# assafmu/wav2letter_pytorch

Measured on AMD Instinct MI355X. Metric: audio-frames/sec/GPU (fwd+bwd+CTC), Wav2Letter 64-mel x 1000-frame bf16, higher is better.
Workload: dtype bf16

## Files before the change

### include/w2l_hip.h

```cpp
#ifndef W2L_HIP_H
#define W2L_HIP_H
#include <stdint.h>
#ifdef __cplusplus
extern "C" {
#endif

const char* w2l_last_error(void);
int w2l_abi_version(void);


int w2l_pack_weights(const float* w, int64_t s_co, int64_t s_ci, int64_t s_kw, int Cout, int Cin, int Kw,
                     int CoutP, int CinP, void* w_fwd_hi, void* w_fwd_lo, void* w_dgr_hi, void* w_dgr_lo,
                     void* stream);

int w2l_sgd_pack(float* p, float* g, float* m, int first_step, float lr, float momentum, float weight_decay,
                 int nesterov, int zero_grad, int Cout, int Cin, int Kw, void* w_fwd_hi, void* w_fwd_lo, void* w_dgr_hi,
                 void* w_dgr_lo, void* w_fwd_q, void* w_dgr_q, float q_scale, void* stream);

int w2l_nct_to_ntc(const float* x, int N, int C, int T, int CP, int pad_l, int pad_r, int pad_mode,
                   const int32_t* lens, void* out_hi, void* out_lo, void* stream);

int w2l_pad_cast(const float* g, int N, int T, int C, int CP, int halo, void* out_hi, void* out_lo, float* colsum,
                 void* stream);

int w2l_conv_stat_tiles(int N, int Tout);
int w2l_conv1d_igemm(const void* xp, int64_t x_bstride, int64_t x_rows_total, const void* w, void* y, int y_f32,
                     int accumulate, const float* bias, float* stats_partial, int N, int Cin, int Cout, int Tout,
                     int Kw, int stride, int dil, void* stream);

int w2l_conv1d_igemm_tune(const void* xp, int64_t x_bstride, int64_t x_rows_total, const void* w, void* y, int y_f32,
                          const float* bias, float* stats_partial, int N, int Cin, int Cout, int Tout, int Kw, int stride,
                          int dil, int reps, void* stream);

int w2l_conv1d_igemm_ws(const void* xp, int64_t x_bstride, int64_t x_rows_total, const void* w, void* y, int y_f32,
                        int accumulate, const float* bias, float* stats_partial, int N, int Cin, int Cout, int Tout, int Kw,
                        int stride, int dil, void* splitk_ws, int64_t splitk_ws_bytes, void* stream);
int w2l_conv1d_igemm_tune_ws(const void* xp, int64_t x_bstride, int64_t x_rows_total, const void* w, void* y, int y_f32,
                             const float* bias, float* stats_partial, int N, int Cin, int Cout, int Tout, int Kw, int stride,
                             int dil, int reps, void* splitk_ws, int64_t splitk_ws_bytes, void* stream);
int64_t w2l_conv_splitk_workspace_bytes(int N, int Cout, int Tout);
int w2l_conv_streamk_ranges(int idx, int N, int Cin, int Cout, int Tout, int Kw, int stride, int dil, int64_t ws_bytes);
int w2l_conv_streamk_pieces(int tiles, int steps, int G, int* out, int cap);

int w2l_conv1d_igemm_fp8(const void* xq, int64_t x_bstride, int64_t x_rows_total, const void* wq, void* y, int y_f32,
                         float descale, const float* descale_dev, const float* bias, float* stats_partial, int N, int Cin,
                         int Cout, int Tout, int Kw, int dil, void* stream);
int w2l_conv1d_igemm_fp8_tune(const void* xq, int64_t x_bstride, int64_t x_rows_total, const void* wq, void* y, int y_f32,
                              const float* bias, float* stats_partial, int N, int Cin, int Cout, int Tout, int Kw, int dil,
                              int reps, void* stream);

void w2l_conv_force_tile_config(int idx);
void w2l_conv_force_fp8_config(int idx);
int w2l_conv_plan(int N, int Cin, int Cout, int Tout, int Kw, int stride, int dil, int stats_flag, int64_t ws_bytes,
                  int forced_idx, int* out);
int w2l_conv_plan_fp8(int N, int Cin, int Cout, int Tout, int Kw, int dil, int stats_flag, int forced_idx, int* out);

int w2l_wgrad_needs_zero(int N, int Cin, int Cout, int Tout, int Kw);
int w2l_conv1d_wgrad(const void* dy, int64_t dy_bstride, const void* xp, int64_t x_bstride, int64_t x_rows_total,
                     float* dw, int N, int Cin, int Cout, int Tout, int Kw, int stride, int dil, int accumulate,
                     void* stream);

int w2l_conv1d_wgrad_ws(const void* dy, int64_t dy_bstride, const void* xp, int64_t x_bstride, int64_t x_rows_total, float* dw,
                        int N, int Cin, int Cout, int Tout, int Kw, int stride, int dil, int accumulate, void* ws,
                        int64_t ws_bytes, void* stream);
int w2l_conv1d_wgrad_tune_ws(const void* dy, int64_t dy_bstride, const void* xp, int64_t x_bstride, int64_t x_rows_total,
                             float* dw_scratch, int N, int Cin, int Cout, int Tout, int Kw, int stride, int dil, int reps,
                             void* ws, int64_t ws_bytes, void* stream);
int w2l_wgrad_needs_zero_ws(int N, int Cin, int Cout, int Tout, int Kw, int64_t ws_bytes);
int64_t w2l_wgrad_workspace_bytes(int Cin, int Cout, int Kw);

int64_t w2l_wgrad_dealt_workspace_bytes(int Cin, int Cout, int Kw);
int w2l_conv1d_wgrad_tune_x(const void* dy, int64_t dy_bstride, const void* xp, int64_t x_bstride, int64_t x_rows_total,
                            float* dw_scratch, int N, int Cin, int Cout, int Tout, int Kw, int stride, int dil, int reps,
                            void* ws, int64_t ws_bytes, int flags, void* stream);
int w2l_wgrad_needs_zero_x(int N, int Cin, int Cout, int Tout, int Kw, int stride, int dil, int64_t ws_bytes);
int w2l_wgrad_dealt_segments(int tiles, int steps, int ranges, int* out, int max_blocks);
int w2l_wgrad_plan(int N, int Cin, int Cout, int Tout, int Kw);

typedef struct {
    const void* dy;
    int64_t dy_bstride;
    const void* xp;
    int64_t x_bstride;
    int64_t x_rows_total;
    float* dw;
    int Cin, Cout, Kw, pad_;
} w2l_wgrad_item_t;
#define W2L_WGRAD_GROUP_MAX 8
int w2l_conv1d_wgrad_group(const w2l_wgrad_item_t* items, int nitems, int N, int Tout, int dil, int form, void* stream);
int w2l_wgrad_group_tiles(int Cin, int Cout, int Kw, int form);

void w2l_wgrad_force_plan(int splits, int order);
void w2l_wgrad_deterministic(int on);

int w2l_conv1d_wgrad_tune(const void* dy, int64_t dy_bstride, const void* xp, int64_t x_bstride, int64_t x_rows_total,
                          float* dw_scratch, int N, int Cin, int Cout, int Tout, int Kw, int stride, int dil, int reps,
                          void* stream);

int w2l_wgrad_fp8_needs_zero(int N, int Cin, int Cout, int Tout, int Kw);
int w2l_conv1d_wgrad_fp8(const void* dyq, int64_t dy_bstride, const void* xq, int64_t x_bstride, int64_t x_rows_total,
                         float* dw, int N, int Cin, int Cout, int Tout, int Kw, int dil, float descale,
                         const float* descale_dev, int accumulate, void* stream);
int w2l_conv1d_wgrad_fp8_tune(const void* dyq, int64_t dy_bstride, const void* xq, int64_t x_bstride, int64_t x_rows_total,
                              float* dw_scratch, int N, int Cin, int Cout, int Tout, int Kw, int dil, int reps, void* stream);

int w2l_tune_save(const char* path);
int w2l_tune_load(const char* path);

int w2l_dwconv_fwd(const void* x_hi, const void* x_lo, int x_rows, const float* w, void* y_hi, void* y_lo, int N, int Tout,
                   int C, int K, int stride, int dil, const int32_t* lens, void* stream);
int w2l_dwconv_dgrad(const void* dy, int dy_f32, int dy_rows, const float* w, void* dxp, int dxp_f32, int N, int Tp, int Tout,
                     int C, int K, int dil, const int32_t* lens, void* stream);
int w2l_dwconv_wgrad(const void* dy, int dy_f32, int dy_rows, const void* x_hi, const void* x_lo, int x_rows, float* dw, int N,
                     int Tout, int C, int K, int stride, int dil, const int32_t* lens, void* stream);


int w2l_bn_finalize(const float* partial, int ntiles, int C, int64_t count, const float* gamma, const float* beta,
                    float eps, float momentum, float* running_mean, float* running_var, float* mean, float* invstd,
                    float* scale, float* shift, void* stream);

typedef struct {
    int32_t N, T, C;
    const void* y;
    int32_t y_f32;
    const float* scale;
    const float* shift;
    const float* mean;
    const float* invstd;
    const void* y2;
    const float* scale2;
    const float* shift2;
    const float* mean2;
    const float* invstd2;
    int32_t act;
    float drop_p;
    uint64_t seed, offset;
    uint8_t* mask;
    const int32_t* lens;
    const uint64_t* offset_dev;
    uint64_t* q_clipped;
} w2l_bnact_t;

int w2l_bn_act_fwd(const w2l_bnact_t* d, void* out_hi, void* out_lo, int out_rows, int pad_l, int pad_r,
                   int pad_mode, void* stream);
int w2l_bn_act_fwd_q(const w2l_bnact_t* d, void* out_hi, void* out_lo, void* out_q, float q_scale, int out_rows,
                     int pad_l, int pad_r, int pad_mode, void* stream);
typedef struct {
    const float* partial;
    int32_t rows;
    int64_t count;
    const float* gamma;
    const float* beta;
    float eps, momentum;
    float* running_mean;
    float* running_var;
    float* mean;
    float* invstd;
    float* scale;
    float* shift;
} w2l_bnfin_t;
int w2l_bn_act_fwd_fin(const w2l_bnact_t* d, const w2l_bnfin_t* f1, const w2l_bnfin_t* f2, void* out_hi, void* out_q,
                       float q_scale, int out_rows, int pad_l, int pad_r, int pad_mode, void* stream);
void w2l_conv_stats_mode(int slots);

int w2l_quantize_e4m3(const void* src, int src_f32, int64_t n, float scale, void* dst, void* stream);

typedef struct {
    const void* dxp;
    int32_t f32;
    int32_t pad_l, pad_r, pad_mode;
    int32_t rows;
} w2l_gradsrc_t;

int w2l_bn_bwd_blocks(int N, int T, int C);
int w2l_bn_act_bwd_reduce(const w2l_bnact_t* d, const w2l_gradsrc_t* g1, const w2l_gradsrc_t* g2, float* partial,
                          void* stream);
int w2l_bn_bwd_finalize(const float* partial, int nblocks, int C, int ncomp, float* sums, void* stream);
int w2l_bn_act_bwd_apply(const w2l_bnact_t* d, const w2l_gradsrc_t* g1, const w2l_gradsrc_t* g2, const float* sums,
                         void* dy_hi, void* dy_lo, int halo, void* dy2_hi, void* dy2_lo, int halo2, void* stream);
int w2l_bn_act_bwd_apply_fin(const w2l_bnact_t* d, const w2l_gradsrc_t* g1, const w2l_gradsrc_t* g2, const float* partial,
                             int nblocks, float* sums, void* dy_hi, void* dy_lo, int halo, void* dy2_hi, void* dy2_lo,
                             int halo2, float* amax, void* stream);
int w2l_bn_bwd_fast_ok(const w2l_bnact_t* d, const w2l_gradsrc_t* g1, const w2l_gradsrc_t* g2);
int w2l_bn_act_bwd_reduce_slots(const w2l_bnact_t* d, const w2l_gradsrc_t* g1, float* partial, int slots, void* stream);
int w2l_bn_act_bwd_apply_slots(const w2l_bnact_t* d, const w2l_gradsrc_t* g1, const float* partial, int nrows, float* sums,
                               void* dy_hi, int halo, float* amax, void* stream);
#define W2L_AMAX_SLOTS 64
int w2l_bn_act_bwd_apply_amax(const w2l_bnact_t* d, const w2l_gradsrc_t* g1, const w2l_gradsrc_t* g2, const float* sums,
                              void* dy_hi, void* dy_lo, int halo, void* dy2_hi, void* dy2_lo, int halo2, float* amax,
                              void* stream);
int w2l_quantize_e4m3_dyn(const void* src_bf16, int64_t n, const float* amax, void* dst, float* inv_scale, void* stream);

int w2l_conv1d_dgrad_bnreduce_ws(const void* dy, int64_t dy_rows_total, const void* w_dgr, void* dxp, float* partial,
                                 const w2l_bnact_t* d, int pad_l, int pad_r, int pad_mode, int per, int Cconv_out,
                                 int flat_rows, int Kw, int dil, void* splitk_ws, int64_t splitk_ws_bytes, void* stream);
int w2l_conv1d_dgrad_bnreduce_tune_ws(const void* dy, int64_t dy_rows_total, const void* w_dgr, void* dxp, float* partial,
                                      const w2l_bnact_t* d, int pad_l, int pad_r, int pad_mode, int per, int Cconv_out,
                                      int flat_rows, int Kw, int dil, int reps, void* splitk_ws, int64_t splitk_ws_bytes,
                                      void* stream);

typedef struct {
    const float* scale;
    const float* shift;
    const void* res;
    const void* res_lo;
    int32_t act;
    const int32_t* lens;
    void* out_hi;
    void* out_lo;
    int32_t out_rows, pad_l, pad_r, pad_mode;
} w2l_bnact_epi_t;
int w2l_conv1d_igemm_bnact(const void* xp, int64_t x_bstride, int64_t x_rows_total, const void* w, const float* acc_in,
                           const float* bias, const w2l_bnact_epi_t* e, int N, int Cin, int Cout, int Tout, int Kw, int stride,
                           int dil, void* stream);
int w2l_conv1d_igemm_bnact_ws(const void* xp, int64_t x_bstride, int64_t x_rows_total, const void* w, const float* acc_in,
                              const float* bias, const w2l_bnact_epi_t* e, int N, int Cin, int Cout, int Tout, int Kw,
                              int stride, int dil, void* splitk_ws, int64_t splitk_ws_bytes, void* stream);
int w2l_conv1d_igemm_bnact_tune_ws(const void* xp, int64_t x_bstride, int64_t x_rows_total, const void* w, const float* bias,
                                   const w2l_bnact_epi_t* e, int N, int Cin, int Cout, int Tout, int Kw, int stride, int dil,
                                   int reps, void* splitk_ws, int64_t splitk_ws_bytes, void* stream);

int w2l_conv1d_igemm_bnact_fp8(const void* xq, int64_t x_bstride, int64_t x_rows_total, const void* wq, float descale,
                               const float* bias, const w2l_bnact_epi_t* e, void* out_q, float q_scale, int64_t* q_clipped,
                               int N, int Cin, int Cout, int Tout, int Kw, int dil, void* stream);
int w2l_conv1d_igemm_bnact_fp8_tune(const void* xq, int64_t x_bstride, int64_t x_rows_total, const void* wq, const float* bias,
                                    const w2l_bnact_epi_t* e, void* out_q, float q_scale, int N, int Cin, int Cout, int Tout,
                                    int Kw, int dil, int reps, void* stream);

int w2l_log_softmax_fwd(const float* logits, int N, int T, int C, int CP, int mode, float* out, void* stream);
int w2l_log_softmax_bwd(const float* gout, const float* out, int N, int T, int C, int mode, float* glogits,
                        void* stream);
int64_t w2l_ctc_workspace_bytes(int N, int T, int Smax);
int w2l_ctc_loss(const float* log_probs, const int32_t* targets, const int32_t* input_lengths,
                 const int32_t* target_lengths, int N, int T, int C, int Smax, int blank, int zero_infinity,
                 float* nll, float* loss, float* grad, void* workspace, void* stream);

int64_t w2l_ctc_align_workspace_bytes(int N, int T, int Smax);
int w2l_ctc_align(const float* x, const int32_t* input_lengths, const int32_t* targets, int64_t target_stride,
                  const int32_t* target_lengths, int64_t length_stride, int N, int T, int A, int Smax, int blank,
                  int log_probs, void* workspace, int64_t workspace_bytes, float* score, int32_t* status, int32_t* path,
                  int32_t* starts, int32_t* ends, void* stream);

int64_t w2l_asg_workspace_bytes(int N, int T, int A, int Smax);
int w2l_asg_loss(const float* x, const float* transitions, const int32_t* targets, const int32_t* input_lengths,
                 const int32_t* target_lengths, int N, int T, int A, int Smax, int repeat_index, int reduction, float* nll,
                 float* loss, float* grad_x, float* grad_trans, int32_t* status, void* workspace, int64_t workspace_bytes,
                 void* stream);
int64_t w2l_asg_viterbi_workspace_bytes(int N, int T, int A);
int w2l_asg_viterbi(const float* x, const float* transitions, const int32_t* input_lengths, int N, int T, int A,
                    void* workspace, int64_t workspace_bytes, int32_t* path, float* score, void* stream);

int w2l_argmax(const float* probs, int64_t rows, int C, int32_t* idx, void* stream);
typedef struct {
    const float* prob;
    const float* bo;
    const uint64_t* ngram_keys;
    const int32_t* ngram_vals;
    int64_t ngram_cap;
    const uint64_t* trie_keys;
    const int32_t* trie_vals;
    int64_t trie_cap;
    const int32_t* trie_word;
    int32_t n_entries;
    int32_t n_words;
    int32_t n_trie_nodes;
} w2l_ngram_lm_t;
int w2l_ngram_lm_build(const uint64_t* keys, const int32_t* vals, int64_t n, uint64_t* table_keys, int32_t* table_vals,
                       int64_t cap, int32_t* dups, void* stream);
typedef struct {
    const uint64_t* trie_keys;
    const int32_t* trie_vals;
    int64_t trie_cap;
    const int32_t* trie_word;
    int32_t n_trie_nodes;
} w2l_lexicon_t;
int64_t w2l_ctc_beam_search_workspace_bytes(int N, int T, int k, int order);
int w2l_ctc_beam_search(const float* probs, const int32_t* sizes, int N, int T, int A, const int32_t* label_info_host,
                        int blank, int end_index, int space_index, int k, double alpha, double beta, double prune,
                        int log_probs, const w2l_ngram_lm_t* lm, int order, const w2l_lexicon_t* lexicon,
                        int complete_only, const w2l_lexicon_t* hotwords, double hotword_weight, void* workspace,
                        int64_t workspace_bytes, void* out, void* stream);
int64_t w2l_asg_beam_search_workspace_bytes(int N, int T, int A, int k, int order);
int w2l_asg_beam_search(const float* x, const float* transitions, const int32_t* sizes, int N, int T, int A,
                        const int32_t* label_info_host, int repeat_index, int space_index, int k, double alpha, double beta,
                        double prune, const w2l_ngram_lm_t* lm, int order, void* workspace, int64_t workspace_bytes, void* out,
                        void* stream);
int w2l_asg_beam_search_tables(const float* x, const float* transitions, const int32_t* sizes, int N, int T, int A,
                               const int32_t* label_info_host, int repeat_index, int space_index, int k, double alpha,
                               double beta, double prune, const w2l_ngram_lm_t* lm, int order, const w2l_lexicon_t* lexicon,
                               int complete_only, const w2l_lexicon_t* hotwords, double hotword_weight, void* workspace,
                               int64_t workspace_bytes, void* out, void* stream);
int64_t w2l_asg_align_workspace_bytes(int N, int T, int A, int Smax);
int w2l_asg_align(const float* x, const float* transitions, const int32_t* input_lengths, const int32_t* targets,
                  int64_t target_stride, const int32_t* target_lengths, int64_t length_stride, int N, int T, int A, int Smax,
                  int repeat_index, int encoded, void* workspace, int64_t workspace_bytes, float* score, int32_t* status,
                  int32_t* path, int32_t* starts, int32_t* ends, void* stream);
int w2l_levenshtein_host(const int32_t* a_host, int na, const int32_t* b_host, int nb);
int w2l_greedy_score_host(const int32_t* idx_host, int N, int T, const int32_t* sizes_host, int blank, const int32_t* lut,
                          int n_labels, const int32_t* ref_cp, const int64_t* ref_off, int64_t* totals, int32_t* hyp_cp,
                          int64_t* hyp_off);

int w2l_novograd_pack(float* p, const float* g, float* exp_avg, float* exp_avg_sq, float* max_exp_avg_sq, float* scratch,
                      int scratch_floats, float lr, float beta1, float beta2, float eps, float weight_decay, int grad_averaging,
                      int Cout, int Cin, int Kw, void* w_fwd_hi, void* w_fwd_lo, void* w_dgr_hi, void* w_dgr_lo, void* stream);

int w2l_logmel(const float* audio, const int32_t* n_samples, const float* noise, float dither, float preemph, int N,
               int64_t audio_stride, const float* window, int win_length, int n_fft, int hop, const float* fbT,
               const int32_t* fb_range, int n_mels, int take_log, float log_guard, float* logmel, int Tmax, void* stream);
int w2l_feature_normalize(const float* logmel, const int32_t* n_samples, int hop, int N, int Tmax, int n_mels, float eps,
                          float* mean_ws, float* std_ws, float* out_nct, void* stream);
int w2l_zero_rects(float* x, int N, int C, int T, const int32_t* rects, int R, void* stream);

#define W2L_RESAMPLE_TILE 512
#define W2L_RESAMPLE_MAX_K 512
#define W2L_RESAMPLE_MAX_SPAN 8192
int w2l_resample(const float* x, int64_t in_stride, float* out, int64_t out_stride, int N, const int32_t* rows_host,
                 const int32_t* rows_dev, const int32_t* banks_host, const int32_t* banks_dev, int n_banks, const float* taps,
                 int64_t n_taps, void* stream);

#define W2L_REVERB_TILE 1024
#define W2L_REVERB_CHUNK 512
#define W2L_REVERB_MAX_TAPS 16384
int w2l_reverb(const float* x, int64_t in_stride, float* out, int64_t out_stride, int N, const int32_t* rows_host,
               const int32_t* rows_dev, const int32_t* banks_host, const int32_t* banks_dev, int n_banks, const float* taps,
               int64_t n_taps, void* stream);
#define W2L_MIX_TILE 2048
int64_t w2l_mix_noise_slab_doubles(int N, int64_t out_stride);
int w2l_mix_noise(const float* x, int64_t x_stride, const float* z, int64_t z_stride, float* out, int64_t out_stride, int N,
                  const int32_t* rows_host, const int32_t* rows_dev, const float* snr_db, double* slab, int64_t slab_doubles,
                  void* stream);

int w2l_stream_probe(void* stream_a, void* stream_b, void* stamps_dev, int rounds, int spin_us);

#define W2L_RCCL_ID_BYTES 128
int w2l_rccl_available(void);
const char* w2l_rccl_library(void);
int w2l_rccl_unique_id(void* id_host);
int w2l_rccl_init(const void* id_host, int rank, int world, void** comm_out);
int w2l_rccl_world(void* comm, int* world_out);
int w2l_rccl_all_reduce(void* comm, void* buf, int64_t count, int dtype, int average, void* stream);
int w2l_rccl_broadcast(void* comm, void* buf, int64_t bytes, int root, void* stream);
int w2l_rccl_destroy(void* comm);

typedef union { void* p; int64_t i; double d; } w2l_slot_t;
#define W2L_REPLAY_MAX_ARGS 24
typedef struct { int32_t op; int32_t nargs; w2l_slot_t a[W2L_REPLAY_MAX_ARGS]; } w2l_call_t;
int w2l_replay_op(const char* entry_point_name);
int w2l_replay_arity(int op);
int w2l_replay(const w2l_call_t* calls, int n, int* failed_at);

int w2l_event_create(void** event_out);
int w2l_event_destroy(void* event);
int w2l_event_record(void* event, void* stream);
int w2l_stream_wait_event(void* stream, void* event);
int w2l_event_query(void* event);
int w2l_event_synchronize(void* event);
int w2l_stream_wait_stream(void* waiter, void* signaler);

int w2l_fill_zero(void* p, int64_t bytes, void* stream);
int w2l_pad_vec_f32(const float* src, int n, float* dst, int cp, float fill, void* stream);
int w2l_counter_add(void* counter_i64, int64_t delta, void* stream);
int w2l_add_i64_multi(void* table_dev, int n, int64_t delta, void* stream);
typedef struct { float* p; const float* g; float* m; int32_t n; int32_t pad_; } w2l_sgd_small_t;
int w2l_sgd_small_multi(const w2l_sgd_small_t* items_dev, int nitems, int max_n , float lr,
                        float momentum, float weight_decay, int nesterov, void* stream);

#define W2L_CLIP_NORM 0
#define W2L_CLIP_COEF 1
#define W2L_CLIP_BOUND 2
#define W2L_GNORM_CHUNK 8192
#define W2L_GNORM_BLOCKS 2048
typedef struct { const float* g; int64_t n; int64_t chunk0; } w2l_gnorm_item_t;
int w2l_grad_sqnorm_multi(const w2l_gnorm_item_t* items_dev, int nitems, int64_t nchunks, int inf_norm, double* partials,
                          float max_norm, float* clip, float* norm_out, void* stream);
int w2l_grad_clip_value(float* clip, float clip_value, void* stream);
int w2l_sgd_pack_clip(float* p, float* g, float* m, int first_step, float lr, float momentum, float weight_decay,
                      int nesterov, int zero_grad, int Cout, int Cin, int Kw, void* w_fwd_hi, void* w_fwd_lo, void* w_dgr_hi,
                      void* w_dgr_lo, void* w_fwd_q, void* w_dgr_q, float q_scale, const float* clip, void* stream);
int w2l_sgd_small_multi_clip(const w2l_sgd_small_t* items_dev, int nitems, int max_n, float lr, float momentum,
                             float weight_decay, int nesterov, const float* clip, void* stream);

typedef struct { int64_t step; double pow1; double pow2; } w2l_adam_state_t;
typedef struct { float* p; const float* g; float* m; float* v; int32_t n; int32_t pad_; } w2l_adam_small_t;
int w2l_adam_tick(w2l_adam_state_t* state_dev, float* dyn_dev, double lr, double beta1, double beta2, void* stream);
int w2l_adam_pack(float* p, float* g, float* m, float* v, const float* dyn, float beta1, float beta2, float eps,
                  float weight_decay, int decoupled, int zero_grad, int Cout, int Cin, int Kw, void* w_fwd_hi, void* w_fwd_lo,
                  void* w_dgr_hi, void* w_dgr_lo, void* w_fwd_q, void* w_dgr_q, float q_scale, const float* clip ,
                  void* stream);
// ... 9 lines not shown
```

### wav2letter_pytorch_amd/_lib.py

```python
from __future__ import annotations

import ctypes as C
import os

os.environ.setdefault('GPU_MAX_HW_QUEUES', '8')

import torch

_HERE = os.path.dirname(os.path.abspath(__file__))
LIB_PATH = os.environ.get('W2L_LIB') or os.path.join(_HERE, 'libw2l_hip.so')

c_p = C.c_void_p
c_i = C.c_int
c_i64 = C.c_int64
c_u64 = C.c_uint64
c_f = C.c_float


class BnActDesc(C.Structure):
    _fields_ = [
        ('N', C.c_int32), ('T', C.c_int32), ('C', C.c_int32),
        ('y', c_p), ('y_f32', C.c_int32),
        ('scale', c_p), ('shift', c_p), ('mean', c_p), ('invstd', c_p),
        ('y2', c_p), ('scale2', c_p), ('shift2', c_p), ('mean2', c_p), ('invstd2', c_p),
        ('act', C.c_int32), ('drop_p', c_f), ('seed', c_u64), ('offset', c_u64),
        ('mask', c_p), ('lens', c_p), ('offset_dev', c_p), ('q_clipped', c_p),
    ]


class WgradItem(C.Structure):
    _fields_ = [('dy', c_p), ('dy_bstride', C.c_int64), ('xp', c_p), ('x_bstride', C.c_int64), ('x_rows_total', C.c_int64),
                ('dw', c_p), ('Cin', C.c_int32), ('Cout', C.c_int32), ('Kw', C.c_int32), ('pad_', C.c_int32)]


class BnFin(C.Structure):
    _fields_ = [('partial', c_p), ('rows', C.c_int32), ('count', C.c_int64), ('gamma', c_p), ('beta', c_p), ('eps', c_f),
                ('momentum', c_f), ('running_mean', c_p), ('running_var', c_p), ('mean', c_p), ('invstd', c_p), ('scale', c_p),
                ('shift', c_p)]


class LmTables(C.Structure):
    _fields_ = [('prob', c_p), ('bo', c_p), ('ngram_keys', c_p), ('ngram_vals', c_p), ('ngram_cap', C.c_int64),
                ('trie_keys', c_p), ('trie_vals', c_p), ('trie_cap', C.c_int64), ('trie_word', c_p), ('n_entries', C.c_int32),
                ('n_words', C.c_int32), ('n_trie_nodes', C.c_int32)]


class LexTables(C.Structure):
    _fields_ = [('trie_keys', c_p), ('trie_vals', c_p), ('trie_cap', C.c_int64), ('trie_word', c_p),
                ('n_trie_nodes', C.c_int32)]


class BnActEpi(C.Structure):
    _fields_ = [('scale', c_p), ('shift', c_p), ('res', c_p), ('res_lo', c_p), ('act', C.c_int32), ('lens', c_p),
                ('out_hi', c_p), ('out_lo', c_p), ('out_rows', C.c_int32), ('pad_l', C.c_int32), ('pad_r', C.c_int32),
                ('pad_mode', C.c_int32)]


class GradSrc(C.Structure):
    _fields_ = [('dxp', c_p), ('f32', C.c_int32), ('pad_l', C.c_int32), ('pad_r', C.c_int32),
                ('pad_mode', C.c_int32), ('rows', C.c_int32)]


_SIGNATURES = {
    'w2l_last_error': (C.c_char_p, []),
    'w2l_abi_version': (c_i, []),
    'w2l_tune_save': (c_i, [C.c_char_p]),
    'w2l_tune_load': (c_i, [C.c_char_p]),
    'w2l_pack_weights': (c_i, [c_p, c_i64, c_i64, c_i64, c_i, c_i, c_i, c_i, c_i, c_p, c_p, c_p, c_p, c_p]),
    'w2l_sgd_pack': (c_i, [c_p, c_p, c_p, c_i, c_f, c_f, c_f, c_i, c_i, c_i, c_i, c_i, c_p, c_p, c_p, c_p, c_p, c_p, c_f, c_p]),
    'w2l_novograd_pack': (c_i, [c_p, c_p, c_p, c_p, c_p, c_p, c_i, c_f, c_f, c_f, c_f, c_f, c_i, c_i, c_i, c_i, c_p, c_p, c_p, c_p,
                                c_p]),
    'w2l_nct_to_ntc': (c_i, [c_p, c_i, c_i, c_i, c_i, c_i, c_i, c_i, c_p, c_p, c_p, c_p]),
    'w2l_pad_cast': (c_i, [c_p, c_i, c_i, c_i, c_i, c_i, c_p, c_p, c_p, c_p]),
    'w2l_conv_stat_tiles': (c_i, [c_i, c_i]),
    'w2l_conv1d_igemm': (c_i, [c_p, c_i64, c_i64, c_p, c_p, c_i, c_i, c_p, c_p, c_i, c_i, c_i, c_i, c_i, c_i, c_i, c_p]),
    'w2l_conv1d_igemm_tune': (c_i, [c_p, c_i64, c_i64, c_p, c_p, c_i, c_p, c_p, c_i, c_i, c_i, c_i, c_i, c_i, c_i, c_i, c_p]),
    'w2l_conv1d_igemm_ws': (c_i, [c_p, c_i64, c_i64, c_p, c_p, c_i, c_i, c_p, c_p, c_i, c_i, c_i, c_i, c_i, c_i, c_i, c_p, c_i64, c_p]),
    'w2l_conv1d_igemm_tune_ws': (c_i, [c_p, c_i64, c_i64, c_p, c_p, c_i, c_p, c_p, c_i, c_i, c_i, c_i, c_i, c_i, c_i, c_i, c_p,
                                       c_i64, c_p]),
    'w2l_conv1d_igemm_bnact': (c_i, [c_p, c_i64, c_i64, c_p, c_p, c_p, C.POINTER(BnActEpi), c_i, c_i, c_i, c_i, c_i, c_i, c_i, c_p]),
    'w2l_conv1d_igemm_bnact_ws': (c_i, [c_p, c_i64, c_i64, c_p, c_p, c_p, C.POINTER(BnActEpi), c_i, c_i, c_i, c_i, c_i, c_i, c_i,
                                        c_p, c_i64, c_p]),
    'w2l_conv1d_igemm_bnact_tune_ws': (c_i, [c_p, c_i64, c_i64, c_p, c_p, C.POINTER(BnActEpi), c_i, c_i, c_i, c_i, c_i, c_i, c_i,
                                             c_i, c_p, c_i64, c_p]),
    'w2l_conv_splitk_workspace_bytes': (c_i64, [c_i, c_i, c_i]),
    'w2l_conv_streamk_ranges': (c_i, [c_i] * 8 + [c_i64]),
    'w2l_conv_streamk_pieces': (c_i, [c_i, c_i, c_i, c_p, c_i]),
    'w2l_conv_force_tile_config': (None, [c_i]),
    'w2l_conv_force_fp8_config': (None, [c_i]),
    'w2l_conv_plan': (c_i, [c_i] * 8 + [c_i64, c_i, c_p]),
    'w2l_conv_plan_fp8': (c_i, [c_i] * 8 + [c_p]),
    'w2l_wgrad_force_plan': (None, [c_i, c_i]),
    'w2l_wgrad_deterministic': (None, [c_i]),
    'w2l_wgrad_needs_zero': (c_i, [c_i, c_i, c_i, c_i, c_i]),
    'w2l_conv1d_wgrad': (c_i, [c_p, c_i64, c_p, c_i64, c_i64, c_p, c_i, c_i, c_i, c_i, c_i, c_i, c_i, c_i, c_p]),
    'w2l_conv1d_wgrad_ws': (c_i, [c_p, c_i64, c_p, c_i64, c_i64, c_p, c_i, c_i, c_i, c_i, c_i, c_i, c_i, c_i, c_p, c_i64, c_p]),
    'w2l_conv1d_wgrad_tune_ws': (c_i, [c_p, c_i64, c_p, c_i64, c_i64, c_p, c_i, c_i, c_i, c_i, c_i, c_i, c_i, c_i, c_p, c_i64, c_p]),
    'w2l_wgrad_needs_zero_ws': (c_i, [c_i, c_i, c_i, c_i, c_i, c_i64]),
    'w2l_wgrad_workspace_bytes': (c_i64, [c_i, c_i, c_i]),
    'w2l_wgrad_dealt_workspace_bytes': (c_i64, [c_i, c_i, c_i]),
    'w2l_conv1d_wgrad_tune_x': (c_i, [c_p, c_i64, c_p, c_i64, c_i64, c_p, c_i, c_i, c_i, c_i, c_i, c_i, c_i, c_i, c_p, c_i64, c_i, c_p]),
    'w2l_wgrad_needs_zero_x': (c_i, [c_i, c_i, c_i, c_i, c_i, c_i, c_i, c_i64]),
    'w2l_wgrad_dealt_segments': (c_i, [c_i, c_i, c_i, c_p, c_i]),
    'w2l_wgrad_plan': (c_i, [c_i, c_i, c_i, c_i, c_i]),
    'w2l_conv1d_wgrad_group': (c_i, [c_p, c_i, c_i, c_i, c_i, c_i, c_p]),
    'w2l_wgrad_group_tiles': (c_i, [c_i, c_i, c_i, c_i]),
    'w2l_conv1d_wgrad_tune': (c_i, [c_p, c_i64, c_p, c_i64, c_i64, c_p, c_i, c_i, c_i, c_i, c_i, c_i, c_i, c_i, c_p]),
    'w2l_dwconv_fwd': (c_i, [c_p, c_p, c_i, c_p, c_p, c_p, c_i, c_i, c_i, c_i, c_i, c_i, c_p, c_p]),
    'w2l_dwconv_dgrad': (c_i, [c_p, c_i, c_i, c_p, c_p, c_i, c_i, c_i, c_i, c_i, c_i, c_i, c_p, c_p]),
    'w2l_dwconv_wgrad': (c_i, [c_p, c_i, c_i, c_p, c_p, c_i, c_p, c_i, c_i, c_i, c_i, c_i, c_i, c_p, c_p]),
    'w2l_bn_finalize': (c_i, [c_p, c_i, c_i, c_i64, c_p, c_p, c_f, c_f, c_p, c_p, c_p, c_p, c_p, c_p, c_p]),
    'w2l_bn_act_fwd': (c_i, [C.POINTER(BnActDesc), c_p, c_p, c_i, c_i, c_i, c_i, c_p]),
    'w2l_bn_act_fwd_q': (c_i, [C.POINTER(BnActDesc), c_p, c_p, c_p, c_f, c_i, c_i, c_i, c_i, c_p]),
    'w2l_bn_bwd_fast_ok': (c_i, [C.POINTER(BnActDesc), C.POINTER(GradSrc), C.POINTER(GradSrc)]),
    'w2l_bn_act_bwd_reduce_slots': (c_i, [C.POINTER(BnActDesc), C.POINTER(GradSrc), c_p, c_i, c_p]),
    'w2l_bn_act_bwd_apply_slots': (c_i, [C.POINTER(BnActDesc), C.POINTER(GradSrc), c_p, c_i, c_p, c_p, c_i, c_p, c_p]),
    'w2l_bn_act_fwd_fin': (c_i, [C.POINTER(BnActDesc), C.POINTER(BnFin), C.POINTER(BnFin), c_p, c_p, c_f, c_i, c_i, c_i, c_i, c_p]),
    'w2l_conv_stats_mode': (None, [c_i]),
    'w2l_quantize_e4m3': (c_i, [c_p, c_i, c_i64, c_f, c_p, c_p]),
    'w2l_quantize_e4m3_dyn': (c_i, [c_p, c_i64, c_p, c_p, c_p, c_p]),
    'w2l_bn_act_bwd_apply_amax': (c_i, [C.POINTER(BnActDesc), C.POINTER(GradSrc), C.POINTER(GradSrc), c_p, c_p, c_p, c_i,
                                        c_p, c_p, c_i, c_p, c_p]),
    'w2l_conv1d_igemm_fp8': (c_i, [c_p, c_i64, c_i64, c_p, c_p, c_i, c_f, c_p, c_p, c_p, c_i, c_i, c_i, c_i, c_i, c_i, c_p]),
    'w2l_conv1d_igemm_bnact_fp8': (c_i, [c_p, c_i64, c_i64, c_p, c_f, c_p, C.POINTER(BnActEpi), c_p, c_f, c_p, c_i, c_i, c_i, c_i,
                                         c_i, c_i, c_p]),
    'w2l_conv1d_igemm_bnact_fp8_tune': (c_i, [c_p, c_i64, c_i64, c_p, c_p, C.POINTER(BnActEpi), c_p, c_f, c_i, c_i, c_i, c_i, c_i,
                                              c_i, c_i, c_p]),
    'w2l_conv1d_igemm_fp8_tune': (c_i, [c_p, c_i64, c_i64, c_p, c_p, c_i, c_p, c_p, c_i, c_i, c_i, c_i, c_i, c_i, c_i, c_p]),
    'w2l_bn_bwd_blocks': (c_i, [c_i, c_i, c_i]),
    'w2l_bn_act_bwd_reduce': (c_i, [C.POINTER(BnActDesc), C.POINTER(GradSrc), C.POINTER(GradSrc), c_p, c_p]),
    'w2l_bn_bwd_finalize': (c_i, [c_p, c_i, c_i, c_i, c_p, c_p]),
    'w2l_bn_act_bwd_apply': (c_i, [C.POINTER(BnActDesc), C.POINTER(GradSrc), C.POINTER(GradSrc), c_p, c_p, c_p, c_i,
                                   c_p, c_p, c_i, c_p]),
    'w2l_conv1d_dgrad_bnreduce_ws': (c_i, [c_p, c_i64, c_p, c_p, c_p, C.POINTER(BnActDesc), c_i, c_i, c_i, c_i, c_i, c_i, c_i, c_i,
                                           c_p, c_i64, c_p]),
    'w2l_conv1d_dgrad_bnreduce_tune_ws': (c_i, [c_p, c_i64, c_p, c_p, c_p, C.POINTER(BnActDesc), c_i, c_i, c_i, c_i, c_i, c_i, c_i,
                                                c_i, c_i, c_p, c_i64, c_p]),
    'w2l_bn_act_bwd_apply_fin': (c_i, [C.POINTER(BnActDesc), C.POINTER(GradSrc), C.POINTER(GradSrc), c_p, c_i, c_p, c_p, c_p, c_i,
                                       c_p, c_p, c_i, c_p, c_p]),
    'w2l_log_softmax_fwd': (c_i, [c_p, c_i, c_i, c_i, c_i, c_i, c_p, c_p]),
    'w2l_log_softmax_bwd': (c_i, [c_p, c_p, c_i, c_i, c_i, c_i, c_p, c_p]),
    'w2l_ctc_workspace_bytes': (c_i64, [c_i, c_i, c_i]),
    'w2l_ctc_loss': (c_i, [c_p, c_p, c_p, c_p, c_i, c_i, c_i, c_i, c_i, c_i, c_p, c_p, c_p, c_p, c_p]),
    'w2l_asg_workspace_bytes': (c_i64, [c_i, c_i, c_i, c_i]),
    'w2l_asg_loss': (c_i, [c_p, c_p, c_p, c_p, c_p, c_i, c_i, c_i, c_i, c_i, c_i, c_p, c_p, c_p, c_p, c_p, c_p, c_i64, c_p]),
    'w2l_asg_viterbi_workspace_bytes': (c_i64, [c_i, c_i, c_i]),
    'w2l_asg_viterbi': (c_i, [c_p, c_p, c_p, c_i, c_i, c_i, c_p, c_i64, c_p, c_p, c_p]),
    'w2l_argmax': (c_i, [c_p, c_i64, c_i, c_p, c_p]),
    'w2l_ctc_align_workspace_bytes': (c_i64, [c_i, c_i, c_i]),
    'w2l_ctc_align': (c_i, [c_p, c_p, c_p, c_i64, c_p, c_i64, c_i, c_i, c_i, c_i, c_i, c_i, c_p, c_i64, c_p, c_p, c_p, c_p, c_p,
                            c_p]),
    'w2l_ctc_beam_search_workspace_bytes': (c_i64, [c_i, c_i, c_i, c_i]),
    'w2l_ctc_beam_search': (c_i, [c_p, c_p, c_i, c_i, c_i, c_p, c_i, c_i, c_i, c_i, C.c_double, C.c_double, C.c_double, c_i,
                                  C.POINTER(LmTables), c_i, C.POINTER(LexTables), c_i, C.POINTER(LexTables), C.c_double,
                                  c_p, c_i64, c_p, c_p]),
    'w2l_ngram_lm_build': (c_i, [c_p, c_p, c_i64, c_p, c_p, c_i64, c_p, c_p]),
    'w2l_asg_beam_search_workspace_bytes': (c_i64, [c_i, c_i, c_i, c_i, c_i]),
    'w2l_asg_beam_search': (c_i, [c_p, c_p, c_p, c_i, c_i, c_i, c_p, c_i, c_i, c_i, C.c_double, C.c_double, C.c_double,
                                  C.POINTER(LmTables), c_i, c_p, c_i64, c_p, c_p]),
    'w2l_asg_beam_search_tables': (c_i, [c_p, c_p, c_p, c_i, c_i, c_i, c_p, c_i, c_i, c_i, C.c_double, C.c_double, C.c_double,
                                         C.POINTER(LmTables), c_i, C.POINTER(LexTables), c_i, C.POINTER(LexTables), C.c_double,
                                         c_p, c_i64, c_p, c_p]),
    'w2l_asg_align_workspace_bytes': (c_i64, [c_i, c_i, c_i, c_i]),
    'w2l_asg_align': (c_i, [c_p, c_p, c_p, c_p, c_i64, c_p, c_i64, c_i, c_i, c_i, c_i, c_i, c_i, c_p, c_i64, c_p, c_p, c_p, c_p,
                            c_p, c_p]),
    'w2l_logmel': (c_i, [c_p, c_p, c_p, c_f, c_f, c_i, c_i64, c_p, c_i, c_i, c_i, c_p, c_p, c_i, c_i, c_f, c_p, c_i, c_p]),
    'w2l_feature_normalize': (c_i, [c_p, c_p, c_i, c_i, c_i, c_i, c_f, c_p, c_p, c_p, c_p]),
    'w2l_zero_rects': (c_i, [c_p, c_i, c_i, c_i, c_p, c_i, c_p]),
    'w2l_resample': (c_i, [c_p, c_i64, c_p, c_i64, c_i, c_p, c_p, c_p, c_p, c_i, c_p, c_i64, c_p]),
    'w2l_reverb': (c_i, [c_p, c_i64, c_p, c_i64, c_i, c_p, c_p, c_p, c_p, c_i, c_p, c_i64, c_p]),
    'w2l_mix_noise_slab_doubles': (c_i64, [c_i, c_i64]),
    'w2l_mix_noise': (c_i, [c_p, c_i64, c_p, c_i64, c_p, c_i64, c_i, c_p, c_p, c_p, c_p, c_i64, c_p]),
    'w2l_levenshtein_host': (c_i, [c_p, c_i, c_p, c_i]),
    'w2l_greedy_score_host': (c_i, [c_p, c_i, c_i, c_p, c_i, c_p, c_i, c_p, c_p, c_p, c_p, c_p]),
    'w2l_wgrad_fp8_needs_zero': (c_i, [c_i, c_i, c_i, c_i, c_i]),
    'w2l_conv1d_wgrad_fp8': (c_i, [c_p, c_i64, c_p, c_i64, c_i64, c_p, c_i, c_i, c_i, c_i, c_i, c_i, c_f, c_p, c_i, c_p]),
    'w2l_conv1d_wgrad_fp8_tune': (c_i, [c_p, c_i64, c_p, c_i64, c_i64, c_p, c_i, c_i, c_i, c_i, c_i, c_i, c_i, c_p]),
    'w2l_stream_probe': (c_i, [c_p, c_p, c_p, c_i, c_i]),
    'w2l_rccl_available': (c_i, []),
    'w2l_rccl_library': (C.c_char_p, []),
    'w2l_rccl_unique_id': (c_i, [c_p]),
    'w2l_rccl_init': (c_i, [c_p, c_i, c_i, c_p]),
    'w2l_rccl_world': (c_i, [c_p, c_p]),
    'w2l_rccl_all_reduce': (c_i, [c_p, c_p, c_i64, c_i, c_i, c_p]),
    'w2l_rccl_broadcast': (c_i, [c_p, c_p, c_i64, c_i, c_p]),
    'w2l_rccl_destroy': (c_i, [c_p]),
    'w2l_replay_op': (c_i, [C.c_char_p]),
    'w2l_replay_arity': (c_i, [c_i]),
    'w2l_replay': (c_i, [c_p, c_i, c_p]),
    'w2l_event_create': (c_i, [c_p]),
    'w2l_event_destroy': (c_i, [c_p]),
    'w2l_event_record': (c_i, [c_p, c_p]),
    'w2l_stream_wait_event': (c_i, [c_p, c_p]),
    'w2l_event_query': (c_i, [c_p]),
    'w2l_event_synchronize': (c_i, [c_p]),
    'w2l_stream_wait_stream': (c_i, [c_p, c_p]),
    'w2l_fill_zero': (c_i, [c_p, c_i64, c_p]),
    'w2l_pad_vec_f32': (c_i, [c_p, c_i, c_p, c_i, c_f, c_p]),
    'w2l_counter_add': (c_i, [c_p, c_i64, c_p]),
    'w2l_add_i64_multi': (c_i, [c_p, c_i, c_i64, c_p]),
    'w2l_sgd_small_multi': (c_i, [c_p, c_i, c_i, c_f, c_f, c_f, c_i, c_p]),
    'w2l_sgd_small_multi_clip': (c_i, [c_p, c_i, c_i, c_f, c_f, c_f, c_i, c_p, c_p]),
    'w2l_sgd_pack_clip': (c_i, [c_p, c_p, c_p, c_i, c_f, c_f, c_f, c_i, c_i, c_i, c_i, c_i, c_p, c_p, c_p, c_p, c_p, c_p, c_f, c_p,
                                c_p]),
    'w2l_grad_sqnorm_multi': (c_i, [c_p, c_i, c_i64, c_i, c_p, c_f, c_p, c_p, c_p]),
    'w2l_grad_clip_value': (c_i, [c_p, c_f, c_p]),
    'w2l_adam_tick': (c_i, [c_p, c_p, C.c_double, C.c_double, C.c_double, c_p]),
    'w2l_adam_pack': (c_i, [c_p, c_p, c_p, c_p, c_p, c_f, c_f, c_f, c_f, c_i, c_i, c_i, c_i, c_i, c_p, c_p, c_p, c_p, c_p, c_p, c_f,
                            c_p, c_p]),
    'w2l_adam_small_multi': (c_i, [c_p, c_i, c_i, c_p, c_f, c_f, c_f, c_f, c_i, c_p, c_p]),
}

EXPORTED_SYMBOLS = tuple(_SIGNATURES)
GNORM_CHUNK = 8192
GNORM_BLOCKS = 2048
CLIP_NORM, CLIP_COEF, CLIP_BOUND = 0, 1, 2


class W2LError(RuntimeError):
    pass


def _load():
    if not os.path.exists(LIB_PATH):
        raise ImportError(
            f'{LIB_PATH} not found: build the HIP extension first '
            f'(python -c "import __graft_entry__ as g; g.build()" or make -C wav2letter_pytorch_amd/csrc). '
            f'There is no CPU fallback.')
    lib = C.CDLL(LIB_PATH)
    for name, (res, args) in _SIGNATURES.items():
        fn = getattr(lib, name)
        fn.restype = res
        fn.argtypes = args
    return lib


lib = _load()


def check(rc: int, what: str = ''):
    if rc != 0:
        msg = lib.w2l_last_error()
        raise W2LError(f'{what} failed (code {rc}): {msg.decode() if msg else "?"}')


def ptr(t):
    return None if t is None else C.c_void_p(t.data_ptr())


def stream_ptr():
    return C.c_void_p(torch._C._cuda_getCurrentRawStream(torch._C._cuda_getDevice()))


def require_device(*tensors):
    for t in tensors:
        if t is not None and not t.is_cuda:
            raise W2LError('wav2letter_pytorch_amd runs on MI355X only: got a CPU tensor '
                           '(there is no CPU fallback; move the model and batch to cuda)')


TRACE_NAMES = {
    'w2l_conv1d_igemm': 'conv_igemm_kernel', 'w2l_conv1d_igemm_ws': 'conv_igemm_kernel',
    'w2l_conv1d_dgrad_bnreduce_ws': 'conv_igemm_kernel/dgrad+bnreduce',
    'w2l_conv1d_igemm_bnact': 'conv_igemm_kernel/bnact', 'w2l_conv1d_igemm_bnact_ws': 'conv_igemm_kernel/bnact',
    'w2l_conv1d_igemm_fp8': 'conv_igemm_fp8_kernel', 'w2l_conv1d_igemm_bnact_fp8': 'conv_igemm_fp8_kernel/bnact',
    'w2l_conv1d_wgrad': 'conv_wgrad_kernel', 'w2l_conv1d_wgrad_ws': 'conv_wgrad_kernel', 'w2l_conv1d_wgrad_group': 'conv_wgrad_kernel', 'w2l_conv1d_wgrad_fp8': 'conv_wgrad_fp8_kernel',
    'w2l_bn_finalize': 'bn_finalize_kernel', 'w2l_bn_act_fwd': 'bn_act_fwd_kernel', 'w2l_bn_act_fwd_q': 'bn_act_fwd_kernel',
    'w2l_bn_act_fwd_fin': 'bn_act_fwd_kernel', 'w2l_bn_act_bwd_reduce': 'bn_act_bwd_reduce_kernel',
    'w2l_bn_act_bwd_reduce_slots': 'bn_act_bwd_reduce_kernel', 'w2l_bn_act_bwd_apply_slots': 'bn_act_bwd_apply_kernel', 'w2l_bn_bwd_finalize': 'bn_bwd_finalize_kernel',
    'w2l_bn_act_bwd_apply': 'bn_act_bwd_apply_kernel', 'w2l_bn_act_bwd_apply_amax': 'bn_act_bwd_apply_kernel',
    'w2l_bn_act_bwd_apply_fin': 'bn_act_bwd_apply_kernel', 'w2l_sgd_pack': 'sgd_pack_kernel', 'w2l_pack_weights': 'pack_weights_kernel',
    'w2l_sgd_pack_clip': 'sgd_pack_kernel', 'w2l_adam_pack': 'adam_pack_kernel', 'w2l_grad_sqnorm_multi': 'grad_norm_kernels',
    'w2l_asg_loss': 'asg_kernels', 'w2l_asg_viterbi': 'asg_viterbi_kernel',
    'w2l_ctc_loss': 'ctc_kernels', 'w2l_log_softmax_fwd': 'log_softmax_fwd', 'w2l_log_softmax_bwd': 'log_softmax_bwd',
    'w2l_nct_to_ntc': 'nct_to_ntc_kernel', 'w2l_pad_cast': 'pad_cast_kernel', 'w2l_quantize_e4m3': 'quantize_e4m3',
    'w2l_quantize_e4m3_dyn': 'quantize_e4m3_dyn', 'w2l_dwconv_fwd': 'dw_fwd_kernel', 'w2l_dwconv_dgrad': 'dw_dgrad_kernel',
    'w2l_dwconv_wgrad': 'dw_wgrad_kernel', 'w2l_argmax': 'argmax_kernel', 'w2l_novograd_pack': 'novograd_pack_kernel',
    'w2l_ctc_beam_search': 'ctc_beam_search_kernel', 'w2l_ngram_lm_build': 'ngram_insert_kernel', 'w2l_ctc_align': 'ctc_align_kernel',
    'w2l_asg_beam_search': 'asg_beam_search_kernel', 'w2l_asg_beam_search_tables': 'asg_beam_search_kernel',
    'w2l_asg_align': 'asg_align_kernel',
}
_trace = {'rows': None, 'saved': {}, 'pool': []}


def trace_launches(enable: bool, capacity: int = 4096):
    if enable and _trace['rows'] is None:
        _trace['rows'] = []
    if enable and not _trace['saved']:
        _trace['pool'] = [torch.cuda.Event(enable_timing=True) for _ in range(2 * capacity)]
        for name, label in TRACE_NAMES.items():
            fn = getattr(lib, name)
            _trace['saved'][name] = fn

            def wrapper(*args, _fn=fn, _label=label):
                pool = _trace['pool']
                s = pool.pop() if pool else torch.cuda.Event(enable_timing=True)
                e = pool.pop() if pool else torch.cuda.Event(enable_timing=True)
                s.record()
                rc = _fn(*args)
                e.record()
                _trace['rows'].append((_label, torch._C._cuda_getCurrentRawStream(torch._C._cuda_getDevice()), s, e))
                return rc

            setattr(lib, name, wrapper)
    elif not enable:
        for name, fn in _trace['saved'].items():
            setattr(lib, name, fn)
        _trace['saved'] = {}


def trace_dump(path: str) -> int:
    rows, _trace['rows'] = _trace['rows'] or [], None
    _trace['pool'] = []
    if not rows:
        return 0
    origin = rows[0][2]
    with open(path, 'w') as f:
        f.write('Kernel_Name,Queue_Id,Start_Timestamp,End_Timestamp\n')
        for label, stream, s, e in rows:
            t0 = origin.elapsed_time(s)
            f.write('%s,%d,%d,%d\n' % (label, stream, int(t0 * 1e6), int((t0 + s.elapsed_time(e)) * 1e6)))
    return len(rows)


def raw_stream(stream=None) -> int:
    if stream is None:
        return torch._C._cuda_getCurrentRawStream(torch._C._cuda_getDevice())
    return stream.cuda_stream


class Event:
    __slots__ = ('h', '__weakref__')
    _free: list = []

    def __init__(self):
        if Event._free:
            self.h = Event._free.pop()
        else:
            out = C.c_void_p()
            check(lib.w2l_event_create(C.byref(out)), 'w2l_event_create')
            self.h = out.value
        rec = _recorder[0]
        if rec is not None:
            rec.keep.append(self)

    def record(self, stream=None):
        check(lib.w2l_event_record(self.h, raw_stream(stream)), 'w2l_event_record')

    def wait(self, stream=None):
        check(lib.w2l_stream_wait_event(raw_stream(stream), self.h), 'w2l_stream_wait_event')

    def query(self) -> bool:
        rc = lib.w2l_event_query(self.h)
        if rc not in (0, 1):
            check(rc, 'w2l_event_query')
        return rc == 0

    def synchronize(self):
        check(lib.w2l_event_synchronize(self.h), 'w2l_event_synchronize')

    def __del__(self):
        try:
            Event._free.append(self.h)
        except Exception:
            pass


def stream_wait_stream(waiter, signaler):
    a = waiter if isinstance(waiter, int) else waiter.cuda_stream
    b = signaler if isinstance(signaler, int) else signaler.cuda_stream
    check(lib.w2l_stream_wait_stream(a, b), 'w2l_stream_wait_stream')


class Slot(C.Union):
    _fields_ = [('p', c_p), ('i', c_i64), ('d', C.c_double)]


REPLAY_MAX_ARGS = 24


class Call(C.Structure):
    _fields_ = [('op', C.c_int32), ('nargs', C.c_int32), ('a', Slot * REPLAY_MAX_ARGS)]


_recorder = [None]
AUDIT = False
_REPLAY_OPS = {}


def _replay_ops():
    if not _REPLAY_OPS:
        for name, (_, args) in _SIGNATURES.items():
            op = lib.w2l_replay_op(name.encode())
            if op < 0:
                continue
            kinds = []
            for a in args:
                if a in (c_i, c_i64, c_u64, C.c_int32):
                    kinds.append('i')
                elif a in (c_f, C.c_double):
                    kinds.append('d')
                else:
                    kinds.append('p')
            assert lib.w2l_replay_arity(op) == len(kinds) <= REPLAY_MAX_ARGS, name
            _REPLAY_OPS[name] = (op, tuple(kinds))
    return _REPLAY_OPS


class Phase:
    __slots__ = ('items', 'keep', 'n_calls', 'dev_ptrs')

    def __init__(self, items, keep, n_calls, dev_ptrs=None):
        self.items, self.keep, self.n_calls = items, keep, n_calls
        self.dev_ptrs = dev_ptrs

    def replay(self):
        failed = C.c_int(-1)
        for it in self.items:
            if it[0] == 'c':
                rc = lib.w2l_replay(it[1], it[2], C.byref(failed))
                if rc != 0:
                    msg = lib.w2l_last_error()
                    raise W2LError(f'w2l_replay failed at record {failed.value} of {it[2]} (code {rc}): {msg.decode() if msg else "?"}')
            else:
                _, fn, args, stream = it
                if stream is None:
                    fn(*args)
# ... 155 lines not shown
```

### wav2letter_pytorch_amd/csrc/ctc.hip

```cpp
#include "common.h"
#include <math.h>
#include <stdlib.h>

namespace {

constexpr float NEG_INF = -INFINITY;

__device__ __forceinline__ float lse2(float a, float b) {
    const float m = fmaxf(a, b);
    if (m == NEG_INF) return NEG_INF;
    return m + __logf(__expf(a - m) + __expf(b - m));
}
__device__ __forceinline__ float lse3(float a, float b, float c) {
    const float m = __builtin_fmaxf(__builtin_fmaxf(a, b), c);
    if (m == NEG_INF) return NEG_INF;
    const float lo = __builtin_fminf(__builtin_fminf(a, b), c);
    const float md = __builtin_amdgcn_fmed3f(a, b, c);
    return m + __logf(1.f + __expf(md - m) + __expf(lo - m));
}

__global__ __launch_bounds__(256) void log_softmax_fwd_kernel(const float* logits, int64_t rows, int C, int CP, int mode,
                                                               float* out) {
    const int lane = threadIdx.x & 63;
    const int64_t row = (int64_t)blockIdx.x * 4 + (threadIdx.x >> 6);
// ... 40 lines not shown
    float* nll;
};

template <int NT, int SPT, bool LP_LDS>
__global__ __launch_bounds__(NT) void ctc_alpha_beta_kernel(CtcParams p) {
    extern __shared__ float sh[];
    const int n = blockIdx.x;
    const bool is_beta = blockIdx.y == 1;
    const int tid = threadIdx.x;
    const int S = min(max(p.tg_len[n], 0), p.Smax);
    const int Tn = min(max(p.in_len[n], 0), p.T);
    const int L = 2 * S + 1;
    const int Lp = SPT * NT + 4;
    float* buf0 = sh + 2;
    float* buf1 = sh + Lp + 2;
    const float* lp = p.lp + (int64_t)n * p.T * p.C;
    if (LP_LDS) {
        float* lds_lp = sh + 2 * Lp;
        const int total = Tn * p.C;
        for (int i = tid; i < total; i += NT) lds_lp[i] = lp[i];
        lp = lds_lp;
        __syncthreads();
    }
    float* dst = (is_beta ? p.beta : p.alpha) + (int64_t)n * p.T * p.L;
    const int32_t* tg = p.targets + (int64_t)n * p.Smax;

    int lab[SPT];
    bool skip[SPT];
#pragma unroll
    for (int k = 0; k < SPT; ++k) {
        const int s = tid + k * NT;
        lab[k] = p.blank;
        skip[k] = false;
        if (s < L && (s & 1)) {
            lab[k] = tg[s >> 1];
            if (!is_beta) skip[k] = s >= 3 && tg[(s >> 1) - 1] != lab[k];
            else skip[k] = s + 2 < L && tg[(s >> 1) + 1] != lab[k];
        }
    }
    if (tid < 2) { buf0[-2 + tid] = NEG_INF; buf1[-2 + tid] = NEG_INF; }
    if (tid < 2) { buf0[Lp - 4 + tid] = NEG_INF; buf1[Lp - 4 + tid] = NEG_INF; }

    if (Tn == 0) {
        if (!is_beta && tid == 0) p.nll[n] = S == 0 ? 0.f : (p.zero_inf ? 0.f : INFINITY);
        return;
    }
    const int t_first = is_beta ? Tn - 1 : 0;
    float cur[SPT], nxt_lp[SPT];
#pragma unroll
    for (int k = 0; k < SPT; ++k) {
        const int s = tid + k * NT;
        float v = NEG_INF;
        if (s < L) {
            const bool init = is_beta ? (s >= L - 2) : (s <= 1);
            if (init) v = lp[(int64_t)t_first * p.C + lab[k]];
            dst[(int64_t)t_first * p.L + s] = v;
        }
        cur[k] = v;
        buf0[s] = v;
        nxt_lp[k] = 0.f;
    }
    const int dir = is_beta ? -1 : 1;
    if (Tn > 1) {
#pragma unroll
        for (int k = 0; k < SPT; ++k)
            if (tid + k * NT < L) nxt_lp[k] = lp[(int64_t)(t_first + dir) * p.C + lab[k]];
    }
    __syncthreads();
    float* prev = buf0;
    float* next = buf1;
    for (int i = 1; i < Tn; ++i) {
        const int t = t_first + dir * i;
        float e[SPT];
#pragma unroll
        for (int k = 0; k < SPT; ++k) e[k] = nxt_lp[k];
        if (i + 1 < Tn) {
#pragma unroll
            for (int k = 0; k < SPT; ++k)
                if (tid + k * NT < L) nxt_lp[k] = lp[(int64_t)(t + dir) * p.C + lab[k]];
        }
#pragma unroll
        for (int k = 0; k < SPT; ++k) {
            const int s = tid + k * NT;
            const float a0 = cur[k];
            const float a1 = prev[s - dir];
            const float a2 = skip[k] ? prev[s - 2 * dir] : NEG_INF;
            float v = lse3(a0, a1, a2) + e[k];
            if (s >= L) v = NEG_INF;
            cur[k] = v;
            next[s] = v;
            if (s < L) dst[(int64_t)t * p.L + s] = v;
        }
        asm volatile("s_waitcnt lgkmcnt(0)" ::: "memory");
        __builtin_amdgcn_s_barrier();
        asm volatile("" ::: "memory");
        float* tmp = prev; prev = next; next = tmp;
    }
    if (!is_beta && tid == 0) {
        const float a = prev[L - 1];
        const float b = L > 1 ? prev[L - 2] : NEG_INF;
        float nll = -lse2(a, b);
        p.nll[n] = nll;
    }
}

__global__ __launch_bounds__(256) void ctc_grad_kernel(CtcParams p, float* grad, float* nll_out) {
    __shared__ float acc_all[4][64];
    const int lane = threadIdx.x & 63, w = threadIdx.x >> 6;
    const int n = blockIdx.y;
    const int t = blockIdx.x * 4 + w;
    if (t >= p.T) return;
    float* acc = acc_all[w];
    const int S = min(max(p.tg_len[n], 0), p.Smax);
    const int Tn = min(max(p.in_len[n], 0), p.T);
    const int L = 2 * S + 1;
    const float nll = p.nll[n];
    const bool inf = !(nll < INFINITY);
    float* g = grad + ((int64_t)n * p.T + t) * p.C;
    if (t >= Tn || (inf && p.zero_inf)) {
        for (int c = lane; c < p.C; c += 64) g[c] = 0.f;
        return;
    }
    const float* lp = p.lp + ((int64_t)n * p.T + t) * p.C;
    const float* al = p.alpha + ((int64_t)n * p.T + t) * p.L;
    const float* be = p.beta + ((int64_t)n * p.T + t) * p.L;
    const int32_t* tg = p.targets + (int64_t)n * p.Smax;
    for (int c = lane; c < 64; c += 64) acc[c] = 0.f;
    float m = NEG_INF;
    for (int s = lane; s < L; s += 64) {
        const int c = (s & 1) ? tg[s >> 1] : p.blank;
        const float v = al[s] + be[s];
        if (v > NEG_INF) m = fmaxf(m, v - lp[c]);
    }
#pragma unroll
    for (int k = 32; k > 0; k >>= 1) m = fmaxf(m, __shfl_xor(m, k, 64));
    __builtin_amdgcn_wave_barrier();
    if (m > NEG_INF) {
        for (int s = lane; s < L; s += 64) {
            const int c = (s & 1) ? tg[s >> 1] : p.blank;
            const float v = al[s] + be[s];
            if (v > NEG_INF) atomicAdd(&acc[c], expf(v - lp[c] - m));
        }
    }
    __builtin_amdgcn_wave_barrier();
    const float gs = 1.f / ((float)p.N * (float)max(S, 1));
    const float post_scale = m > NEG_INF ? expf(m + nll) : 0.f;
    for (int c = lane; c < p.C; c += 64) {
        const float post = acc[c] * post_scale;
        g[c] = (expf(lp[c]) - post) * gs;
    }
    (void)nll_out;
}

__global__ void ctc_loss_reduce_kernel(float* nll, const int32_t* tg_len, int N, int Smax, int zero_inf, float* loss) {
    __shared__ float red[256];
    float s = 0.f;
    for (int n = threadIdx.x; n < N; n += 256) {
        float v = nll[n];
        if (zero_inf && !(v < INFINITY)) { v = 0.f; nll[n] = 0.f; }
        const int S = min(max(tg_len[n], 0), Smax);
        s += v / (float)max(S, 1);
    }
    red[threadIdx.x] = s;
    __syncthreads();
    for (int k = 128; k > 0; k >>= 1) {
        if (threadIdx.x < k) red[threadIdx.x] += red[threadIdx.x + k];
        __syncthreads();
    }
    if (threadIdx.x == 0) loss[0] = red[0] / (float)N;
}

__global__ __launch_bounds__(256) void argmax_kernel(const float* probs, int64_t rows, int C, int32_t* idx) {
    const int64_t row = (int64_t)blockIdx.x * 256 + threadIdx.x;
    if (row >= rows) return;
    const float* p = probs + row * C;
    float best = p[0];
    int bi = 0;
    bool nan_found = best != best;
    for (int c = 1; c < C && !nan_found; ++c) {
        const float v = p[c];
        if (v != v) { bi = c; nan_found = true; }
        else if (v > best) { best = v; bi = c; }
    }
    idx[row] = bi;
}

}

extern "C" int w2l_log_softmax_fwd(const float* logits, int N, int T, int C, int CP, int mode, float* out, void* stream) {
    W2L_CHECK_ARG(logits && out && N > 0 && T > 0 && C > 0 && CP >= C, "log_softmax_fwd: bad arguments");
    const int64_t rows = (int64_t)N * T;
    hipLaunchKernelGGL(log_softmax_fwd_kernel, dim3((unsigned)((rows + 3) / 4)), dim3(256), 0, (hipStream_t)stream,
                       logits, rows, C, CP, mode, out);
    W2L_CHECK_LAUNCH();
    return 0;
}

extern "C" int w2l_log_softmax_bwd(const float* gout, const float* out, int N, int T, int C, int mode, float* glogits,
                                   void* stream) {
    W2L_CHECK_ARG(gout && out && glogits && N > 0 && T > 0 && C > 0, "log_softmax_bwd: bad arguments");
    const int64_t rows = (int64_t)N * T;
    hipLaunchKernelGGL(log_softmax_bwd_kernel, dim3((unsigned)((rows + 3) / 4)), dim3(256), 0, (hipStream_t)stream, gout,
                       out, rows, C, mode, glogits);
    W2L_CHECK_LAUNCH();
    return 0;
}

extern "C" int64_t w2l_ctc_workspace_bytes(int N, int T, int Smax) {
    if (N <= 0 || T <= 0 || Smax < 0) return 0;
    return 2 * (int64_t)N * T * (2 * Smax + 1) * (int64_t)sizeof(float);
}

extern "C" int w2l_ctc_loss(const float* log_probs, const int32_t* targets, const int32_t* input_lengths,
                            const int32_t* target_lengths, int N, int T, int C, int Smax, int blank, int zero_infinity,
                            float* nll, float* loss, float* grad, void* workspace, void* stream) {
    W2L_CHECK_ARG(log_probs && input_lengths && target_lengths && nll && loss && workspace, "ctc_loss: null pointer");
    W2L_CHECK_ARG(targets || Smax == 0, "ctc_loss: null targets");
    W2L_CHECK_ARG(N > 0 && T > 0 && C > 0 && C <= 64 && Smax >= 0 && blank >= 0 && blank < C, "ctc_loss: bad sizes");
    const int L = 2 * Smax + 1;
    W2L_CHECK_ARG(L <= 8 * 1024, "ctc_loss: target length %d too long (max 4095)", Smax);
    CtcParams p;
    p.lp = log_probs; p.targets = targets; p.in_len = input_lengths; p.tg_len = target_lengths;
    p.N = N; p.T = T; p.C = C; p.Smax = Smax; p.L = L; p.blank = blank; p.zero_inf = zero_infinity;
    p.alpha = (float*)workspace;
    p.beta = p.alpha + (int64_t)N * T * L;
    p.nll = nll;
    static const int kWide[] = {64, 128, 192, 256, 320, 384, 448, 512, 640, 768, 896, 1024};
    int nt = 1024;
    for (int w : kWide)
        if (L <= w) { nt = w; break; }
    int spt = (L + nt - 1) / nt;
    if (spt > 1) spt = spt <= 4 ? spt : (spt <= 6 ? 6 : 8);
    dim3 grid(N, 2), block(nt);
    size_t lds = 2 * (size_t)(spt * nt + 4) * sizeof(float);
    const size_t lp_bytes = (size_t)T * C * sizeof(float);
    const bool lp_lds = lds + lp_bytes <= 150 * 1024;
    if (lp_lds) lds += lp_bytes;
#define W2L_CTC_LAUNCH(NT, SPT)                                                                              \
    do {                                                                                                     \
        if (lp_lds) {                                                                                        \
            W2L_CHECK_HIP(w2l_allow_big_lds((const void*)ctc_alpha_beta_kernel<NT, SPT, true>));             \
            hipLaunchKernelGGL((ctc_alpha_beta_kernel<NT, SPT, true>), grid, block, lds, (hipStream_t)stream, p);  \
        } else {                                                                                             \
            hipLaunchKernelGGL((ctc_alpha_beta_kernel<NT, SPT, false>), grid, block, lds, (hipStream_t)stream, p); \
        }                                                                                                    \
    } while (0)
    if (spt == 1) {
        switch (nt) {
            case 64: W2L_CTC_LAUNCH(64, 1); break;
            case 128: W2L_CTC_LAUNCH(128, 1); break;
            case 192: W2L_CTC_LAUNCH(192, 1); break;
            case 256: W2L_CTC_LAUNCH(256, 1); break;
            case 320: W2L_CTC_LAUNCH(320, 1); break;
            case 384: W2L_CTC_LAUNCH(384, 1); break;
            case 448: W2L_CTC_LAUNCH(448, 1); break;
            case 512: W2L_CTC_LAUNCH(512, 1); break;
            case 640: W2L_CTC_LAUNCH(640, 1); break;
            case 768: W2L_CTC_LAUNCH(768, 1); break;
            case 896: W2L_CTC_LAUNCH(896, 1); break;
            default: W2L_CTC_LAUNCH(1024, 1); break;
        }
    } else {
        switch (spt) {
            case 2: W2L_CTC_LAUNCH(1024, 2); break;
            case 3: W2L_CTC_LAUNCH(1024, 3); break;
            case 4: W2L_CTC_LAUNCH(1024, 4); break;
            case 6: W2L_CTC_LAUNCH(1024, 6); break;
            default: W2L_CTC_LAUNCH(1024, 8); break;
        }
    }
#undef W2L_CTC_LAUNCH
    W2L_CHECK_LAUNCH();
    if (grad) {
        hipLaunchKernelGGL(ctc_grad_kernel, dim3((T + 3) / 4, N), dim3(256), 0, (hipStream_t)stream, p, grad, nll);
        W2L_CHECK_LAUNCH();
    }
    hipLaunchKernelGGL(ctc_loss_reduce_kernel, dim3(1), dim3(256), 0, (hipStream_t)stream, nll, target_lengths, N,
                       p.Smax, zero_infinity, loss);
    W2L_CHECK_LAUNCH();
    return 0;
}

extern "C" int w2l_argmax(const float* probs, int64_t rows, int C, int32_t* idx, void* stream) {
    W2L_CHECK_ARG(probs && idx && rows > 0 && C > 0, "argmax: bad arguments");
    hipLaunchKernelGGL(argmax_kernel, dim3((unsigned)((rows + 255) / 256)), dim3(256), 0, (hipStream_t)stream, probs, rows,
                       C, idx);
    W2L_CHECK_LAUNCH();
    return 0;
}
```

### wav2letter_pytorch_amd/csrc/pack.hip

```cpp
#include "common.h"

namespace {

__device__ __forceinline__ void put_split(bf16_raw* hi, bf16_raw* lo, int64_t off, float v) {
    bf16_raw h, l;
    f32_split_bf16(v, h, l);
    hi[off] = h;
    if (lo) lo[off] = l;
}

__global__ void pack_weights_kernel(const float* w, int64_t s_co, int64_t s_ci, int64_t s_kw, int Cout, int Cin,
                                    int Kw, int CoutP, int CinP, bf16_raw* fwd_hi, bf16_raw* fwd_lo,
                                    bf16_raw* dgr_hi, bf16_raw* dgr_lo) {
    __shared__ float tile[32][33];
    const int tx = threadIdx.x, ty = threadIdx.y;
    const int ci0 = blockIdx.x * 32, co0 = blockIdx.y * 32, kw = blockIdx.z;
    const bool ci_fast = s_ci <= s_co;
    for (int j = ty; j < 32; j += 8) {
        const int co = ci_fast ? co0 + j : co0 + tx;
        const int ci = ci_fast ? ci0 + tx : ci0 + j;
        float v = 0.f;
        if (co < Cout && ci < Cin) v = w[co * s_co + ci * s_ci + kw * s_kw];
        if (ci_fast) tile[j][tx] = v; else tile[tx][j] = v;
    }
// ... 221 lines not shown
    for (int64_t i = (int64_t)blockIdx.x * blockDim.x + threadIdx.x; i < total; i += (int64_t)gridDim.x * blockDim.x) {
        const int c = (int)(i % CP);
        const int64_t q = i / CP - halo;
        float v = 0.f;
        if (q >= 0) {
            const int64_t n = q / P;
            const int t = (int)(q - n * P);
            if (t < T && c < C) v = g[(n * T + t) * C + c];
        }
        put_split(out_hi, out_lo, i, v);
    }
}

__global__ void colsum_kernel(const float* g, int64_t rows, int C, int CP, float* colsum) {
    const int c = blockIdx.x;
    float s = 0.f;
    if (c < C)
        for (int64_t r = threadIdx.x; r < rows; r += blockDim.x) s += g[r * C + c];
    __shared__ float red[256];
    red[threadIdx.x] = s;
    __syncthreads();
    for (int k = 128; k > 0; k >>= 1) {
        if (threadIdx.x < k) red[threadIdx.x] += red[threadIdx.x + k];
        __syncthreads();
    }
    if (threadIdx.x == 0) colsum[c] = red[0];
}

}

extern "C" int w2l_pack_weights(const float* w, int64_t s_co, int64_t s_ci, int64_t s_kw, int Cout, int Cin, int Kw,
                                int CoutP, int CinP, void* w_fwd_hi, void* w_fwd_lo, void* w_dgr_hi, void* w_dgr_lo,
                                void* stream) {
    W2L_CHECK_ARG(w && (w_fwd_hi || w_dgr_hi), "pack_weights: null pointer");
    W2L_CHECK_ARG(Cout > 0 && Cin > 0 && Kw > 0 && CoutP >= Cout && CinP >= Cin, "pack_weights: bad sizes");
    W2L_CHECK_ARG(!(w_fwd_lo && !w_fwd_hi) && !(w_dgr_lo && !w_dgr_hi), "pack_weights: lo without hi");
    dim3 grid((CinP + 31) / 32, (CoutP + 31) / 32, Kw), block(32, 8);
    hipLaunchKernelGGL(pack_weights_kernel, grid, block, 0, (hipStream_t)stream, w, s_co, s_ci, s_kw, Cout, Cin, Kw,
                       CoutP, CinP, (bf16_raw*)w_fwd_hi, (bf16_raw*)w_fwd_lo, (bf16_raw*)w_dgr_hi, (bf16_raw*)w_dgr_lo);
    W2L_CHECK_LAUNCH();
    return 0;
}

extern "C" int w2l_sgd_pack(float* p, float* g, float* m, int first_step, float lr, float momentum,
                            float weight_decay, int nesterov, int zero_grad, int Cout, int Cin, int Kw, void* w_fwd_hi,
                            void* w_fwd_lo, void* w_dgr_hi, void* w_dgr_lo, void* w_fwd_q, void* w_dgr_q, float q_scale,
                            void* stream) {
    W2L_CHECK_ARG((!w_fwd_q && !w_dgr_q) || (q_scale > 0.f && w_fwd_hi && w_dgr_hi), "sgd_pack: e4m3 operands need a scale");
    W2L_CHECK_ARG(p && g && m, "sgd_pack: null pointer");
    W2L_CHECK_ARG(Cout > 0 && Cin > 0 && Kw > 0, "sgd_pack: bad sizes");
    W2L_CHECK_ARG(!(w_fwd_lo && !w_fwd_hi) && !(w_dgr_lo && !w_dgr_hi), "sgd_pack: lo without hi");
    dim3 grid((Cin + 31) / 32, (Cout + 31) / 32, Kw), block(32, 8);
    hipLaunchKernelGGL(sgd_pack_kernel<false>, grid, block, 0, (hipStream_t)stream, p, g, m, first_step, lr, momentum,
                       weight_decay, nesterov, zero_grad, Cout, Cin, Kw, (bf16_raw*)w_fwd_hi, (bf16_raw*)w_fwd_lo,
                       (bf16_raw*)w_dgr_hi, (bf16_raw*)w_dgr_lo, (uint8_t*)w_fwd_q, (uint8_t*)w_dgr_q, q_scale, nullptr);
    W2L_CHECK_LAUNCH();
    return 0;
}

extern "C" int w2l_sgd_pack_clip(float* p, float* g, float* m, int first_step, float lr, float momentum,
                                 float weight_decay, int nesterov, int zero_grad, int Cout, int Cin, int Kw, void* w_fwd_hi,
                                 void* w_fwd_lo, void* w_dgr_hi, void* w_dgr_lo, void* w_fwd_q, void* w_dgr_q, float q_scale,
                                 const float* clip, void* stream) {
    W2L_CHECK_ARG((!w_fwd_q && !w_dgr_q) || (q_scale > 0.f && w_fwd_hi && w_dgr_hi), "sgd_pack_clip: e4m3 operands need a scale");
    W2L_CHECK_ARG(p && g && m && clip, "sgd_pack_clip: null pointer");
    W2L_CHECK_ARG(Cout > 0 && Cin > 0 && Kw > 0, "sgd_pack_clip: bad sizes");
    W2L_CHECK_ARG(!(w_fwd_lo && !w_fwd_hi) && !(w_dgr_lo && !w_dgr_hi), "sgd_pack_clip: lo without hi");
    dim3 grid((Cin + 31) / 32, (Cout + 31) / 32, Kw), block(32, 8);
    hipLaunchKernelGGL(sgd_pack_kernel<true>, grid, block, 0, (hipStream_t)stream, p, g, m, first_step, lr, momentum,
                       weight_decay, nesterov, zero_grad, Cout, Cin, Kw, (bf16_raw*)w_fwd_hi, (bf16_raw*)w_fwd_lo,
                       (bf16_raw*)w_dgr_hi, (bf16_raw*)w_dgr_lo, (uint8_t*)w_fwd_q, (uint8_t*)w_dgr_q, q_scale, clip);
    W2L_CHECK_LAUNCH();
    return 0;
}

extern "C" int w2l_adam_pack(float* p, float* g, float* m, float* v, const float* dyn, float beta1, float beta2, float eps,
                             float weight_decay, int decoupled, int zero_grad, int Cout, int Cin, int Kw, void* w_fwd_hi,
                             void* w_fwd_lo, void* w_dgr_hi, void* w_dgr_lo, void* w_fwd_q, void* w_dgr_q, float q_scale,
                             const float* clip, void* stream) {
    W2L_CHECK_ARG((!w_fwd_q && !w_dgr_q) || (q_scale > 0.f && w_fwd_hi && w_dgr_hi), "adam_pack: e4m3 operands need a scale");
    W2L_CHECK_ARG(p && g && m && v && dyn, "adam_pack: null pointer");
    W2L_CHECK_ARG(Cout > 0 && Cin > 0 && Kw > 0, "adam_pack: bad sizes");
    W2L_CHECK_ARG(!(w_fwd_lo && !w_fwd_hi) && !(w_dgr_lo && !w_dgr_hi), "adam_pack: lo without hi");
    W2L_CHECK_ARG(beta1 >= 0.f && beta1 < 1.f && beta2 >= 0.f && beta2 < 1.f && eps >= 0.f, "adam_pack: betas in [0, 1), eps >= 0");
    dim3 grid((Cin + 31) / 32, (Cout + 31) / 32, Kw), block(32, 8);
    if (clip == nullptr)
        hipLaunchKernelGGL(adam_pack_kernel<false>, grid, block, 0, (hipStream_t)stream, p, g, m, v, dyn, beta1, beta2, eps,
                           weight_decay, decoupled, zero_grad, Cout, Cin, Kw, (bf16_raw*)w_fwd_hi, (bf16_raw*)w_fwd_lo,
                           (bf16_raw*)w_dgr_hi, (bf16_raw*)w_dgr_lo, (uint8_t*)w_fwd_q, (uint8_t*)w_dgr_q, q_scale, nullptr);
    else
        hipLaunchKernelGGL(adam_pack_kernel<true>, grid, block, 0, (hipStream_t)stream, p, g, m, v, dyn, beta1, beta2, eps,
                           weight_decay, decoupled, zero_grad, Cout, Cin, Kw, (bf16_raw*)w_fwd_hi, (bf16_raw*)w_fwd_lo,
                           (bf16_raw*)w_dgr_hi, (bf16_raw*)w_dgr_lo, (uint8_t*)w_fwd_q, (uint8_t*)w_dgr_q, q_scale, clip);
    W2L_CHECK_LAUNCH();
    return 0;
}

extern "C" int w2l_novograd_pack(float* p, const float* g, float* exp_avg, float* exp_avg_sq, float* max_exp_avg_sq,
                                 float* scratch, int scratch_floats, float lr, float beta1, float beta2, float eps,
                                 float weight_decay, int grad_averaging, int Cout, int Cin, int Kw, void* w_fwd_hi,
                                 void* w_fwd_lo, void* w_dgr_hi, void* w_dgr_lo, void* stream) {
    W2L_CHECK_ARG(p && g && exp_avg && exp_avg_sq && scratch, "novograd_pack: null pointer");
    W2L_CHECK_ARG(Cout > 0 && Cin > 0 && Kw > 0 && scratch_floats >= 2, "novograd_pack: bad sizes");
    W2L_CHECK_ARG(!(w_fwd_lo && !w_fwd_hi) && !(w_dgr_lo && !w_dgr_hi), "novograd_pack: lo without hi");
    const int64_t n = (int64_t)Cout * Cin * Kw;
    int nblocks = (int)((n + 256 * 16 - 1) / (256 * 16));
    if (nblocks > scratch_floats - 1) nblocks = scratch_floats - 1;
    if (nblocks > 1024) nblocks = 1024;
    if (nblocks < 1) nblocks = 1;
    hipStream_t st = (hipStream_t)stream;
    float* denom = scratch;
    float* partial = scratch + 1;
    hipLaunchKernelGGL(sqnorm_partial_kernel, dim3(nblocks), dim3(256), 0, st, g, n, partial);
    W2L_CHECK_LAUNCH();
    hipLaunchKernelGGL(novograd_finalize_kernel, dim3(1), dim3(256), 0, st, partial, nblocks, beta2, eps, exp_avg_sq,
                       max_exp_avg_sq, denom);
    W2L_CHECK_LAUNCH();
    dim3 grid((Cin + 31) / 32, (Cout + 31) / 32, Kw), block(32, 8);
    hipLaunchKernelGGL(novograd_pack_kernel, grid, block, 0, st, p, g, exp_avg, denom, lr, beta1, weight_decay, grad_averaging,
                       Cout, Cin, Kw, (bf16_raw*)w_fwd_hi, (bf16_raw*)w_fwd_lo, (bf16_raw*)w_dgr_hi, (bf16_raw*)w_dgr_lo);
    W2L_CHECK_LAUNCH();
    return 0;
}

extern "C" int w2l_nct_to_ntc(const float* x, int N, int C, int T, int CP, int pad_l, int pad_r, int pad_mode,
                              const int32_t* lens, void* out_hi, void* out_lo, void* stream) {
    W2L_CHECK_ARG(x && out_hi, "nct_to_ntc: null pointer");
    W2L_CHECK_ARG(N > 0 && C > 0 && T > 0 && CP >= C && pad_l >= 0 && pad_r >= 0, "nct_to_ntc: bad sizes");
    W2L_CHECK_ARG(pad_mode != 1 || (pad_l < T && pad_r < T), "nct_to_ntc: reflect padding (%d,%d) needs pad < T=%d",
                  pad_l, pad_r, T);
    const int R = pad_l + T + pad_r;
    dim3 grid((R + 31) / 32, (CP + 31) / 32, N), block(32, 8);
    hipLaunchKernelGGL(nct_to_ntc_kernel, grid, block, 0, (hipStream_t)stream, x, C, T, CP, R, pad_l, pad_r, pad_mode,
                       lens, (bf16_raw*)out_hi, (bf16_raw*)out_lo);
    W2L_CHECK_LAUNCH();
    return 0;
}

extern "C" int w2l_pad_cast(const float* g, int N, int T, int C, int CP, int halo, void* out_hi, void* out_lo,
                            float* colsum, void* stream) {
    W2L_CHECK_ARG(g && out_hi, "pad_cast: null pointer");
    W2L_CHECK_ARG(N > 0 && T > 0 && C > 0 && CP >= C && halo >= 0, "pad_cast: bad sizes");
    const int64_t total = ((int64_t)halo + (int64_t)N * (T + halo)) * CP;
    const int blocks = (int)((total + 255) / 256 < 4096 ? (total + 255) / 256 : 4096);
    hipLaunchKernelGGL(pad_cast_kernel, dim3(blocks), dim3(256), 0, (hipStream_t)stream, g, T, C, CP, halo,
                       (bf16_raw*)out_hi, (bf16_raw*)out_lo, total);
    W2L_CHECK_LAUNCH();
    if (colsum) {
        hipLaunchKernelGGL(colsum_kernel, dim3(CP), dim3(256), 0, (hipStream_t)stream, g, (int64_t)N * T, C, CP, colsum);
        W2L_CHECK_LAUNCH();
    }
    return 0;
}
```

### wav2letter_pytorch_amd/csrc/replay.hip

```cpp
#include "common.h"
#include "../../include/w2l_hip.h"
#include <string.h>
#include <mutex>
#include <type_traits>
#include <utility>
#include <vector>

extern "C" int w2l_event_create(void** ev) {
    W2L_CHECK_ARG(ev != nullptr, "event_create: null pointer");
    hipEvent_t e;
    W2L_CHECK_HIP(hipEventCreateWithFlags(&e, hipEventDisableTiming));
    *ev = (void*)e;
    return 0;
}
extern "C" int w2l_event_destroy(void* ev) {
    if (ev != nullptr) W2L_CHECK_HIP(hipEventDestroy((hipEvent_t)ev));
    return 0;
}
extern "C" int w2l_event_record(void* ev, void* stream) {
    W2L_CHECK_ARG(ev != nullptr, "event_record: null event");
    W2L_CHECK_HIP(hipEventRecord((hipEvent_t)ev, (hipStream_t)stream));
    return 0;
}
extern "C" int w2l_stream_wait_event(void* stream, void* ev) {
// ... 74 lines not shown
    }
}
template <bool CLIP>
__global__ __launch_bounds__(256) void adam_small_multi_kernel(const w2l_adam_small_t* items, const float* dyn, float beta1, float beta2,
                                                               float eps, float wd, int decoupled, const float* clip) {
    const w2l_adam_small_t it = items[blockIdx.x];
    const int lo = blockIdx.y * SGD_SMALL_CHUNK, hi = min(it.n, lo + SGD_SMALL_CHUNK);
    const adam_scalars s = adam_load_scalars(dyn, beta1, beta2, eps, wd, decoupled);
    float coef = 1.f, bound = 0.f;
    if constexpr (CLIP) {
        coef = clip[W2L_CLIP_COEF];
        bound = clip[W2L_CLIP_BOUND];
    }
    for (int i = lo + threadIdx.x; i < hi; i += 256) {
        float gv = it.g[i];
        if constexpr (CLIP) gv = clip_grad_read(gv, coef, bound);
        float mv = it.m[i], vv = it.v[i];
        const float pv = adam_update(s, it.p[i], gv, mv, vv);
        it.m[i] = mv;
        it.v[i] = vv;
        it.p[i] = pv;
    }
}
__global__ void adam_tick_kernel(w2l_adam_state_t* st, float* dyn, double lr, double beta1, double beta2) {
    if (threadIdx.x != 0 || blockIdx.x != 0) return;
    const double p1 = st->pow1 * beta1, p2 = st->pow2 * beta2;
    st->step += 1;
    st->pow1 = p1;
    st->pow2 = p2;
    dyn[W2L_ADAM_LR] = (float)lr;
    dyn[W2L_ADAM_STEP_SIZE] = (float)(lr / (1.0 - p1));
    dyn[W2L_ADAM_BC2_SQRT] = (float)sqrt(1.0 - p2);
    dyn[3] = 0.f;
}
}

extern "C" int w2l_pad_vec_f32(const float* src, int n, float* dst, int cp, float fill, void* stream) {
    W2L_CHECK_ARG(src != nullptr && dst != nullptr && n >= 0 && cp >= n, "pad_vec_f32: bad arguments");
    if (cp == 0) return 0;
    hipLaunchKernelGGL(pad_vec_kernel, dim3((cp + 255) / 256), dim3(256), 0, (hipStream_t)stream, src, n, dst, cp, fill);
    W2L_CHECK_LAUNCH();
    return 0;
}
extern "C" int w2l_counter_add(void* counter_i64, int64_t delta, void* stream) {
    W2L_CHECK_ARG(counter_i64 != nullptr, "counter_add: null pointer");
    hipLaunchKernelGGL(counter_add_kernel, dim3(1), dim3(64), 0, (hipStream_t)stream, (long long*)counter_i64, (long long)delta);
    W2L_CHECK_LAUNCH();
    return 0;
}
extern "C" int w2l_add_i64_multi(void* table_dev, int n, int64_t delta, void* stream) {
    W2L_CHECK_ARG(table_dev != nullptr || n == 0, "add_i64_multi: null table");
    if (n <= 0) return 0;
    hipLaunchKernelGGL(add_i64_multi_kernel, dim3((n + 63) / 64), dim3(64), 0, (hipStream_t)stream, (long long* const*)table_dev, n,
                       (long long)delta);
    W2L_CHECK_LAUNCH();
    return 0;
}
extern "C" int w2l_sgd_small_multi(const w2l_sgd_small_t* items_dev, int nitems, int max_n, float lr, float momentum,
                                   float weight_decay, int nesterov, void* stream) {
    W2L_CHECK_ARG(items_dev != nullptr || nitems == 0, "sgd_small_multi: null table");
    W2L_CHECK_ARG(max_n >= 0 && max_n <= (1 << 26), "sgd_small_multi: max_n (the largest item's element count) out of range");
    if (nitems <= 0 || max_n == 0) return 0;
    const int chunks = (max_n + SGD_SMALL_CHUNK - 1) / SGD_SMALL_CHUNK;
    hipLaunchKernelGGL(sgd_small_multi_kernel<false>, dim3(nitems, chunks), dim3(256), 0, (hipStream_t)stream, items_dev, lr,
                       momentum, weight_decay, nesterov, nullptr);
    W2L_CHECK_LAUNCH();
    return 0;
}
extern "C" int w2l_sgd_small_multi_clip(const w2l_sgd_small_t* items_dev, int nitems, int max_n, float lr, float momentum,
                                        float weight_decay, int nesterov, const float* clip, void* stream) {
    W2L_CHECK_ARG(items_dev != nullptr || nitems == 0, "sgd_small_multi_clip: null table");
    W2L_CHECK_ARG(clip != nullptr, "sgd_small_multi_clip: null clip buffer");
    W2L_CHECK_ARG(max_n >= 0 && max_n <= (1 << 26), "sgd_small_multi_clip: max_n (the largest item's element count) out of range");
    if (nitems <= 0 || max_n == 0) return 0;
    const int chunks = (max_n + SGD_SMALL_CHUNK - 1) / SGD_SMALL_CHUNK;
    hipLaunchKernelGGL(sgd_small_multi_kernel<true>, dim3(nitems, chunks), dim3(256), 0, (hipStream_t)stream, items_dev, lr,
                       momentum, weight_decay, nesterov, clip);
    W2L_CHECK_LAUNCH();
    return 0;
}

extern "C" int w2l_adam_small_multi(const w2l_adam_small_t* items_dev, int nitems, int max_n, const float* dyn, float beta1,
                                    float beta2, float eps, float weight_decay, int decoupled, const float* clip, void* stream) {
    W2L_CHECK_ARG(items_dev != nullptr || nitems == 0, "adam_small_multi: null table");
    W2L_CHECK_ARG(dyn != nullptr, "adam_small_multi: null dyn buffer");
    W2L_CHECK_ARG(max_n >= 0 && max_n <= (1 << 26), "adam_small_multi: max_n (the largest item's element count) out of range");
    W2L_CHECK_ARG(beta1 >= 0.f && beta1 < 1.f && beta2 >= 0.f && beta2 < 1.f && eps >= 0.f, "adam_small_multi: betas in [0, 1), eps >= 0");
    if (nitems <= 0 || max_n == 0) return 0;
    const int chunks = (max_n + SGD_SMALL_CHUNK - 1) / SGD_SMALL_CHUNK;
    if (clip == nullptr)
        hipLaunchKernelGGL(adam_small_multi_kernel<false>, dim3(nitems, chunks), dim3(256), 0, (hipStream_t)stream, items_dev, dyn,
                           beta1, beta2, eps, weight_decay, decoupled, nullptr);
    else
        hipLaunchKernelGGL(adam_small_multi_kernel<true>, dim3(nitems, chunks), dim3(256), 0, (hipStream_t)stream, items_dev, dyn,
                           beta1, beta2, eps, weight_decay, decoupled, clip);
    W2L_CHECK_LAUNCH();
    return 0;
}
extern "C" int w2l_adam_tick(w2l_adam_state_t* state_dev, float* dyn_dev, double lr, double beta1, double beta2, void* stream) {
    W2L_CHECK_ARG(state_dev != nullptr && dyn_dev != nullptr, "adam_tick: null pointer");
    W2L_CHECK_ARG(beta1 >= 0.0 && beta1 < 1.0 && beta2 >= 0.0 && beta2 < 1.0, "adam_tick: betas in [0, 1)");
    hipLaunchKernelGGL(adam_tick_kernel, dim3(1), dim3(64), 0, (hipStream_t)stream, state_dev, dyn_dev, lr, beta1, beta2);
    W2L_CHECK_LAUNCH();
    return 0;
}

namespace {
template <class T>
inline T slot_get(const w2l_slot_t& s) {
    if constexpr (std::is_pointer_v<T>) return (T)s.p;
    else if constexpr (std::is_floating_point_v<T>) return (T)s.d;
    else return (T)s.i;
}
template <class F>
struct Sig;
template <class R, class... A>
struct Sig<R (*)(A...)> {
    static constexpr int arity = (int)sizeof...(A);
    template <R (*Fn)(A...), size_t... I>
    static int call(const w2l_slot_t* a, std::index_sequence<I...>) {
        if constexpr (std::is_void_v<R>) {
            Fn(slot_get<A>(a[I])...);
            return 0;
        } else {
            return (int)Fn(slot_get<A>(a[I])...);
        }
    }
};
template <auto Fn>
int thunk(const w2l_slot_t* a) {
    using S = Sig<decltype(Fn)>;
    return S::template call<Fn>(a, std::make_index_sequence<(size_t)S::arity>{});
}
struct Entry {
    const char* name;
    int (*fn)(const w2l_slot_t*);
    int arity;
};
#define W2L_E(f) {#f, &thunk<&f>, Sig<decltype(&f)>::arity}
const Entry kEntries[] = {
    W2L_E(w2l_event_record), W2L_E(w2l_stream_wait_event), W2L_E(w2l_stream_wait_stream), W2L_E(w2l_fill_zero),
    W2L_E(w2l_pad_vec_f32), W2L_E(w2l_counter_add), W2L_E(w2l_add_i64_multi), W2L_E(w2l_sgd_small_multi),
    W2L_E(w2l_sgd_small_multi_clip), W2L_E(w2l_sgd_pack_clip), W2L_E(w2l_grad_sqnorm_multi), W2L_E(w2l_grad_clip_value),
    W2L_E(w2l_conv_stats_mode), W2L_E(w2l_wgrad_deterministic),
    W2L_E(w2l_pack_weights), W2L_E(w2l_sgd_pack), W2L_E(w2l_novograd_pack), W2L_E(w2l_adam_pack), W2L_E(w2l_adam_small_multi), W2L_E(w2l_nct_to_ntc), W2L_E(w2l_pad_cast),
    W2L_E(w2l_conv1d_igemm), W2L_E(w2l_conv1d_igemm_ws), W2L_E(w2l_conv1d_igemm_fp8), W2L_E(w2l_conv1d_dgrad_bnreduce_ws),
    W2L_E(w2l_conv1d_wgrad), W2L_E(w2l_conv1d_wgrad_ws), W2L_E(w2l_conv1d_wgrad_group), W2L_E(w2l_conv1d_wgrad_fp8),
    W2L_E(w2l_dwconv_fwd), W2L_E(w2l_dwconv_dgrad), W2L_E(w2l_dwconv_wgrad),
    W2L_E(w2l_bn_finalize), W2L_E(w2l_bn_act_fwd), W2L_E(w2l_bn_act_fwd_q), W2L_E(w2l_bn_act_fwd_fin),
    W2L_E(w2l_bn_act_bwd_reduce), W2L_E(w2l_bn_act_bwd_reduce_slots), W2L_E(w2l_bn_bwd_finalize), W2L_E(w2l_bn_act_bwd_apply),
    W2L_E(w2l_bn_act_bwd_apply_amax), W2L_E(w2l_bn_act_bwd_apply_fin), W2L_E(w2l_bn_act_bwd_apply_slots),
    W2L_E(w2l_quantize_e4m3), W2L_E(w2l_quantize_e4m3_dyn),
    W2L_E(w2l_log_softmax_fwd), W2L_E(w2l_log_softmax_bwd), W2L_E(w2l_ctc_loss), W2L_E(w2l_asg_loss), W2L_E(w2l_argmax),
    W2L_E(w2l_rccl_all_reduce),
};
constexpr int kNumEntries = (int)(sizeof(kEntries) / sizeof(kEntries[0]));
}

extern "C" int w2l_replay_op(const char* name) {
    if (name == nullptr) return -1;
    for (int i = 0; i < kNumEntries; ++i)
        if (strcmp(kEntries[i].name, name) == 0) return i;
    return -1;
}
extern "C" int w2l_replay_arity(int op) { return op >= 0 && op < kNumEntries ? kEntries[op].arity : -1; }

extern "C" int w2l_replay(const w2l_call_t* calls, int n, int* failed_at) {
    W2L_CHECK_ARG(calls != nullptr || n == 0, "replay: null list");
    for (int i = 0; i < n; ++i) {
        const w2l_call_t& c = calls[i];
        if (c.op < 0 || c.op >= kNumEntries || c.nargs != kEntries[c.op].arity) {
            if (failed_at) *failed_at = i;
            w2l_set_error("replay: record %d names entry point %d with %d arguments", i, c.op, c.nargs);
            return 1;
        }
        const int rc = kEntries[c.op].fn(c.a);
        if (rc != 0) {
            if (failed_at) *failed_at = i;
            return rc;
        }
    }
    return 0;
}
```

### wav2letter_pytorch_amd/ctc_loss.py

```python
from __future__ import annotations

import torch
import torch.nn as nn

from . import _lib
from ._lib import check, lib, ptr, stream_ptr


class _CTCFn(torch.autograd.Function):
    @staticmethod
    def forward(ctx, log_probs, targets, input_lengths, target_lengths, blank, zero_infinity):
        _lib.require_device(log_probs)
        lp = log_probs.detach().transpose(0, 1)
        if not lp.is_contiguous() or lp.dtype != torch.float32:
            lp = lp.contiguous().float()
        n, t, c = lp.shape
        dev = lp.device
        if targets.dim() != 2:
            raise NotImplementedError('CTCLoss: targets must be 2-D [N, S_max] (padded), as the collator produces')
        tg = targets.to(device=dev, dtype=torch.int32).contiguous()
        il = torch.as_tensor(input_lengths).to(device=dev, dtype=torch.int32).contiguous()
        tl = torch.as_tensor(target_lengths).to(device=dev, dtype=torch.int32).contiguous()
        smax = tg.shape[1]
        ws = torch.empty(max(int(lib.w2l_ctc_workspace_bytes(n, t, smax)), 4), dtype=torch.uint8, device=dev)
        nll = torch.empty(n, dtype=torch.float32, device=dev)
        loss = torch.empty(1, dtype=torch.float32, device=dev)
        grad = torch.empty(n, t, c, dtype=torch.float32, device=dev)
        check(lib.w2l_ctc_loss(ptr(lp), ptr(tg), ptr(il), ptr(tl), n, t, c, smax, int(blank), int(zero_infinity),
                               ptr(nll), ptr(loss), ptr(grad), ptr(ws), stream_ptr()), 'w2l_ctc_loss')
        ctx.grad = grad
        ctx.nll = nll
        return loss[0]

    @staticmethod
    def backward(ctx, g):
        grad = ctx.grad * g
        return grad.transpose(0, 1), None, None, None, None, None


class CTCLoss(nn.Module):

    def __init__(self, blank=0, reduction='mean', zero_infinity=False):
        super().__init__()
        if reduction != 'mean':
            raise NotImplementedError("only reduction='mean' is implemented (base_asr_models.py:23)")
        self.blank = blank
        self.reduction = reduction
        self.zero_infinity = zero_infinity

    def forward(self, log_probs, targets, input_lengths, target_lengths):
        return _CTCFn.apply(log_probs, targets, input_lengths, target_lengths, self.blank, self.zero_infinity)
```

### wav2letter_pytorch_amd/engine.py

```python
from __future__ import annotations

import atexit
import ctypes as C
import math
import os
from dataclasses import dataclass, field
from typing import Callable, List, NamedTuple, Optional, Sequence, Tuple

import torch

from . import _lib
from . import wgrad_groups as WG
from ._lib import BnActDesc, BnActEpi, GradSrc, check, lib, ptr, stream_ptr

ACT_NONE, ACT_CLAMP20, ACT_RELU = 0, 1, 2
PAD_ZERO, PAD_REFLECT = 0, 1


def _none():
    return None


class _Volatile(dict):

# ... 322 lines not shown
                fused.wait()
            if not recording or fused is not None:
                return hit
        cout, cin, kw = w.shape
        s_co, s_ci, s_kw = _phys_strides(w)
        check(lib.w2l_pack_weights(ptr(w), s_co, s_ci, s_kw, cout, cin, kw, hit.coutp, hit.cinp, ptr(hit.fwd_hi), ptr(hit.fwd_lo),
                                   ptr(hit.dgr_hi), ptr(hit.dgr_lo), stream_ptr()), 'w2l_pack_weights')
        hit.version, hit.ready = w._version, None
        return hit
    cout, cin, kw = w.shape
    coutp, cinp = padded_channels(cout), padded_channels(cin)
    dev = w.device
    if recording:
        _lib.poison('operand pack buffers created')
    fwd_hi = torch.empty(kw, coutp, cinp, dtype=torch.bfloat16, device=dev)
    dgr_hi = torch.empty(kw, cinp, coutp, dtype=torch.bfloat16, device=dev)
    fwd_lo = torch.empty_like(fwd_hi) if precise else None
    dgr_lo = torch.empty_like(dgr_hi) if precise else None
    s_co, s_ci, s_kw = _phys_strides(w)
    check(lib.w2l_pack_weights(ptr(w), s_co, s_ci, s_kw, cout, cin, kw, coutp, cinp, ptr(fwd_hi), ptr(fwd_lo),
                               ptr(dgr_hi), ptr(dgr_lo), stream_ptr()), 'w2l_pack_weights')
    pk = _PackedW(w._version, fwd_hi, fwd_lo, dgr_hi, dgr_lo, cinp, coutp, w.data_ptr())
    cache[precise] = pk
    return pk


def weight_event(w) -> '_lib.Event':
    ev = w.__dict__.get('_w2l_ready_ev')
    if ev is None:
        ev = w.__dict__['_w2l_ready_ev'] = _lib.Event()
        _wev_epoch[0] += 1
    return ev


_wev_epoch = [0]
_in_forward = [False]


FUSED_INFER = os.environ.get('W2L_FUSED_INFER', '1') != '0'
_infer_epoch = [0]


def infer_copies(units: Sequence['UnitSpec'], has_head: bool, fp8: bool, cp0: int) -> List[Tuple[bool, bool]]:
    out = []
    for ai in range(len(units) + 1):
        cp = cp0 if ai == 0 else padded_channels(units[ai - 1].main.cout)
        dense1 = [u.dw is None and u.main.stride == 1 for u in units if u.src == ai]
        dense1 += [u.res.stride == 1 for u in units if u.res is not None and u.res_src == ai]
        q = bool(fp8 and ai > 0 and cp % 128 == 0 and any(dense1))
        hi = (has_head and ai == len(units)) or any(not (q and d) for d in dense1)
        out.append((bool(hi or not q), q))
    return out


def bnact_rows(t: int, T: int, pad_l: int, pad_r: int, reflect: bool) -> List[int]:
    rows = [pad_l + t]
    if reflect:
        if 1 <= t <= pad_l:
            rows.append(pad_l - t)
        j = T - 1 - t
        if 1 <= j <= pad_r:
            rows.append(pad_l + T - 1 + j)
    return rows


def bnact_zero_rows(T: int, pad_l: int, pad_r: int) -> List[int]:
    return list(range(pad_l)) + [pad_l + T + j for j in range(pad_r)]


def fold_bn(gamma, beta, running_mean, running_var, eps: float):
    istd = 1.0 / torch.sqrt(running_var.float() + eps)
    scale = gamma.float() * istd
    return scale, beta.float() - running_mean.float() * gamma.float() * istd


def drop_infer_state():
    _infer_epoch[0] += 1


def invalidate_packed(params) -> int:
    if isinstance(params, torch.nn.Module):
        params = params.parameters()
    drop_infer_state()
    n = 0
    for p in params:
        cache = getattr(p, '_w2l_pack', None)
        if cache:
            for pk in cache.values():
                pk.version = -1
            n += 1
    return n


def _padded_vec(v: Optional[torch.Tensor], cp: int, fill: float) -> Optional[torch.Tensor]:
    if v is None:
        return None
    v = v.detach()
    if v.dtype != torch.float32:
        _lib.poison('a per-channel vector that is not fp32')
        v = v.float()
    if v.numel() == cp and v.is_contiguous():
        return v
    if v.is_cuda and v.is_contiguous():
        out = torch.empty(cp, dtype=torch.float32, device=v.device)
        check(lib.w2l_pad_vec_f32(ptr(v), v.numel(), ptr(out), cp, float(fill), stream_ptr()), 'w2l_pad_vec_f32')
        return out
    out = torch.full((cp,), fill, dtype=torch.float32, device=v.device)
    out[: v.numel()] = v
    return out


SPLITK_WS_CAP = 1 << 30
_splitk_ws = {}


def _splitk_workspace(dev, n, cout, tout):
    need = min(int(lib.w2l_conv_splitk_workspace_bytes(n, cout, tout)), SPLITK_WS_CAP)
    ws = _splitk_ws.get(dev.index)
    if ws is None or ws.numel() < need:
        if ws is not None:
            _retired_ws.append(ws)
        _lib.poison('split-K workspace grown')
        ws = torch.zeros(need, dtype=torch.uint8, device=dev)
        _splitk_ws[dev.index] = ws
    return ws


_side_streams = {}


def _side_stream(dev, main=None) -> 'torch.cuda.Stream':
    st = _side_streams.get(dev.index)
    if st is None:
        from .streams import concurrent_stream
        _lib.poison('side stream created')
        st = concurrent_stream(dev, 'wgrad', main=main)
        _side_streams[dev.index] = st
    return st


WGROUP_MAX = int(os.environ.get('W2L_WGRAD_GROUP_MAX', '3'))
_wgrad_ws = {}
_retired_ws = []
DETERMINISTIC_WGRAD = os.environ.get('W2L_DETERMINISTIC', '0') == '1'
lib.w2l_wgrad_deterministic(int(DETERMINISTIC_WGRAD))
DEALT_WGRAD = os.environ.get('W2L_DEALT_WGRAD', '1') == '1'
DEFER_SPREAD = os.environ.get('W2L_DEFER_SPREAD', 'start')
WGRAD_AFTER_DGRAD = os.environ.get('W2L_WGRAD_AFTER_DGRAD', '0') == '1'
FUSED_BN_REDUCE = os.environ.get('W2L_FUSED_BN_REDUCE', '0')
FUSED_BN_REDUCE_MAX_ROWS = 12288
FOLD_BN_FINALIZE = os.environ.get('W2L_FOLD_BN_FINALIZE', '0') == '1'
FOLD_BN_FWD = os.environ.get('W2L_FOLD_BN_FWD', 'auto')
FOLD_BN_FWD_MAX_ROWS = 12288
FAST_BN_BWD = os.environ.get('W2L_FAST_BN_BWD', '1') == '1'
STAT_SLOTS = int(os.environ.get('W2L_STAT_SLOTS', '8'))


def _wgrad_workspace(dev, cin, cout, kw):
    if DETERMINISTIC_WGRAD:
        need = min(int(lib.w2l_wgrad_workspace_bytes(cin, cout, kw)), SPLITK_WS_CAP)
    else:
        need = min(int(lib.w2l_wgrad_dealt_workspace_bytes(cin, cout, kw)), SPLITK_WS_CAP)
        if need == 0:
            return None
    ws = _wgrad_ws.get(dev.index)
    if ws is None or ws.numel() < need:
        if ws is not None:
            _retired_ws.append(ws)
        _lib.poison('weight-gradient workspace grown')
        ws = torch.zeros(need, dtype=torch.uint8, device=dev)
        _wgrad_ws[dev.index] = ws
    return ws


def _igemm(x: Act, row_off: int, w_hi, w_lo, y, bias, stats, Cin, Cout, Tout, Kw, stride, dil, precise, alg_flops=0.0):
    n = x.N
    bstride = x.rows * x.CP
    rows_total = n * x.rows - row_off
    esz = 2

    def xptr(t):
        return C.c_void_p(t.data_ptr() + row_off * x.CP * esz)

    st = stream_ptr()
    if not precise:
        ws = _splitk_workspace(x.hi.device, n, Cout, Tout)
        if AUTOTUNE:
            key = (n, Cin, Cout, Tout, Kw, stride, dil, stats is not None, x.hi.device.index)
            if _tune_once(key, 'measuring launches'):
                check(lib.w2l_conv1d_igemm_tune_ws(xptr(x.hi), bstride, rows_total, ptr(w_hi), ptr(y),
                                                   int(y.dtype == torch.float32), ptr(bias), ptr(stats), n, Cin, Cout, Tout,
                                                   Kw, stride, dil, TUNE_REPS, ptr(ws), ws.numel(), st), 'w2l_conv1d_igemm_tune_ws')
                if stats is not None and stats.shape[0] <= 64:
                    stats.zero_()
        with _timed('conv_igemm_kernel', alg_flops):
            check(lib.w2l_conv1d_igemm_ws(xptr(x.hi), bstride, rows_total, ptr(w_hi), ptr(y), int(y.dtype == torch.float32),
                                          0, ptr(bias), ptr(stats), n, Cin, Cout, Tout, Kw, stride, dil, ptr(ws), ws.numel(),
                                          st), 'w2l_conv1d_igemm_ws')
        return
    assert y.dtype == torch.float32
    check(lib.w2l_conv1d_igemm(xptr(x.hi), bstride, rows_total, ptr(w_hi), ptr(y), 1, 0, ptr(bias), None, n, Cin, Cout,
                               Tout, Kw, stride, dil, st), 'w2l_conv1d_igemm')
    check(lib.w2l_conv1d_igemm(xptr(x.hi), bstride, rows_total, ptr(w_lo), ptr(y), 1, 1, None, None, n, Cin, Cout, Tout,
                               Kw, stride, dil, st), 'w2l_conv1d_igemm')
    check(lib.w2l_conv1d_igemm(xptr(x.lo), bstride, rows_total, ptr(w_hi), ptr(y), 1, 1, None, ptr(stats), n, Cin, Cout,
                               Tout, Kw, stride, dil, st), 'w2l_conv1d_igemm')


FP8_ACT_SCALE = {ACT_CLAMP20: 16.0, ACT_RELU: 8.0, ACT_NONE: 8.0}
FP8_WEIGHT_RESCALE = 256
FP8_RESCALE_LAG = 8
AMAX_SLOTS = 64
FP8_DGRAD = os.environ.get('W2L_FP8_DGRAD', 'auto')
FP8_DGRAD_MIN_ROWS = 3072
FP8_WGRAD = os.environ.get('W2L_FP8_WGRAD', 'auto')
JOIN_EVENTS = None


_fp8_epoch = [0]


def _pow2_scale(amax: float) -> float:
    return 2.0 ** math.floor(math.log2(448.0 / max(float(amax), 1e-30)))


def _fp8_weights(conv: ConvSpec, pk: '_PackedW', dgrad: bool = False):
    w = conv.weight
    st = w.__dict__.get('_w2l_fp8')
    if st is None or st['q'].shape != pk.fwd_hi.shape or st['q'].device != pk.fwd_hi.device:
        _lib.poison('fp8 weight scale: first use')
        mn, mx = torch.aminmax(pk.fwd_hi)
        scale = _pow2_scale(max(-float(mn), float(mx)))
        dev = pk.fwd_hi.device
        st = _Volatile({'q': torch.empty(pk.fwd_hi.shape, dtype=torch.uint8, device=dev),
                        'qd': torch.empty(pk.dgr_hi.shape, dtype=torch.uint8, device=dev), 'scale': scale, 'age': 0,
                        'version': None, 'version_d': None, 'req': None})
        w.__dict__['_w2l_fp8'] = st
    elif not dgrad and not torch.cuda.is_current_stream_capturing():
        req = st.get('req')
        if req is not None and st['age'] >= FP8_RESCALE_LAG:
            ev, host = req
            ev.synchronize()
            _lib.poison('fp8 weight scale: adoption point')
            st['req'] = None
            scale = _pow2_scale(max(-float(host[0]), float(host[1])))
            if scale != st['scale']:
                st['scale'] = scale
                _fp8_epoch[0] += 1
                st['version'] = st['version_d'] = None
        elif req is None and st['age'] >= FP8_WEIGHT_RESCALE:
            _lib.poison('fp8 weight scale: amax request')
            host = torch.empty(2, dtype=torch.float32, pin_memory=True)
            host.copy_(torch.stack(torch.aminmax(pk.fwd_hi)).float(), non_blocking=True)
            ev = torch.cuda.Event()
            ev.record()
            st['req'] = (ev, host)
            st['age'] = 0
    key, vkey, src = ('qd', 'version_d', pk.dgr_hi) if dgrad else ('q', 'version', pk.fwd_hi)
    if st[vkey] != pk.version:
        check(lib.w2l_quantize_e4m3(ptr(src), 0, src.numel(), st['scale'], ptr(st[key]), stream_ptr()), 'w2l_quantize_e4m3')
        st[vkey] = pk.version
        if not dgrad:
            st['age'] += 1
    return st[key], st['scale']


class StackEngine:

    def __init__(self, units: Sequence[UnitSpec], head: Optional[ConvSpec], n_labels: int, precise: bool = False,
                 fp8: bool = False):
        if fp8 and precise:
            raise ValueError('fp8 operands and the fp32 parity mode exclude each other')
        self.fp8 = fp8
        """``head`` = the classifier conv followed by (log_)softmax; ``None`` runs an OPEN stack whose result is the last
        unit's activation as fp32 [N, C, T'] (stand-alone Conv1dBlock / MaskedConv1d / JasperBlock modules)."""
        self.units = list(units)
        self.head = head
        self.n_labels = n_labels
        self.precise = precise
        self.grad_ready: Optional[Callable] = None
        self.flat_ready: Optional[Callable] = None
        self.backward_done: Optional[Callable[[], None]] = None
        self.overlap_wgrad = True
        self._side = None
        self._main_stream = None
        self._side_used = False
        self._held: list = []
        self._dyq: dict = {}
        self._nbt_pending: list = []
        self._zero_pool = None
        self.dropout_counter: Optional[torch.Tensor] = None
        self._q_clipped: Optional[torch.Tensor] = None
        self.defer_wgrad = 0
        self.deferred = None
        self.grad_reduce_start: Optional[Callable] = None
        self._deferred: list = []
        self._wg_of: dict = {}
        self._wg_pending: dict = {}

    def parameters(self) -> List[torch.Tensor]:
        out = []
        for u in self.units:
            if u.dw is not None:
                out += u.dw.params()
            out += u.main.params()
            if u.res is not None:
                out += u.res.params()
        if self.head is not None:
            out += self.head.params()
        return out

    def _in_pad_for(self, act_index: int):
        pl = pr = 0
        mode = PAD_ZERO
        convs = []
        for u in self.units:
            if u.src == act_index:
                convs.append(u.dw if u.dw is not None else u.main)
            if u.res is not None and u.res_src == act_index:
                convs.append(u.res)
        if act_index == len(self.units) and self.head is not None:
            convs.append(self.head)
        for c in convs:
            if c.pad_l > pl or c.pad_r > pr:
                pl, pr = max(pl, c.pad_l), max(pr, c.pad_r)
            if c.pad_l or c.pad_r:
                mode = c.pad_mode
        return pl, pr, mode

    def forward(self, x: torch.Tensor, lens: Optional[torch.Tensor], training: bool, softmax_mode: int = 0,
                want_input_grad: bool = False):
        _in_forward[0] = True
        try:
            return self._forward(x, lens, training, softmax_mode, want_input_grad)
        finally:
            _in_forward[0] = False
            lib.w2l_conv_stats_mode(0)
            self._stat_pool = None

    def _forward(self, x, lens, training, softmax_mode, want_input_grad):
        _lib.require_device(x)
        global _dropout_calls
        if training:
            _infer_epoch[0] += 1
        if self._deferred:
            self.flush_deferred(pos=0)
        precise = self.precise
        N, C0, T0 = x.shape
        fold = training and not precise and x.is_cuda and not DETERMINISTIC_WGRAD and (
            FOLD_BN_FWD in ('1', True) or (FOLD_BN_FWD == 'auto' and self.units and
                                           N * T0 // max(1, self.units[0].main.stride) < FOLD_BN_FWD_MAX_ROWS))
        self._stat_pool = None
        self._after_apply = []
        if fold:
            need = 0
            for u in self.units:
                for c in (u.main, u.res):
                    if c is not None and c.has_bn:
                        need += STAT_SLOTS * 2 * padded_channels(c.cout)
            fold = need > 0
            if fold:
                self._stat_pool = [zeros(need, torch.float32, x.device), 0]
        lib.w2l_conv_stats_mode(STAT_SLOTS if fold else 0)
        x = x.contiguous().float()
        dev = x.device
        st = stream_ptr
        ctx = {'units': [], 'acts': [], 'training': training, 'x_shape': (N, C0, T0), 'want_dx': bool(want_input_grad)}
        lens_dev, mid_lens, out_lens, lens_final = self._plan_lens(lens, dev)
        pl, pr, mode = self._in_pad_for(0)
        cp0 = padded_channels(C0)
        a_hi = torch.empty(N, pl + T0 + pr, cp0, dtype=torch.bfloat16, device=dev)
        a_lo = torch.empty_like(a_hi) if precise else None
        if lens_dev is not None and not any((u.src == 0 and u.update_lens) for u in self.units):
            in_mask = None
        else:
            in_mask = lens_dev
        check(lib.w2l_nct_to_ntc(ptr(x), N, C0, T0, cp0, pl, pr, mode, ptr(in_mask), ptr(a_hi), ptr(a_lo), st()),
              'w2l_nct_to_ntc')
        acts: List[Act] = [Act(a_hi, a_lo, N, T0, C0, cp0, pl, pr, mode, in_mask)]
        if self.fp8 and self.head is None and self.units and cp0 % 128 == 0 and self._fp8_consumers(0):
            a0 = acts[0]
            a0.q = torch.empty(a_hi.shape, dtype=torch.uint8, device=dev)
            a0.q_scale = FP8_ACT_SCALE[self.units[0].act]
            check(lib.w2l_quantize_e4m3(ptr(a_hi), 0, a_hi.numel(), a0.q_scale, ptr(a0.q), st()), 'w2l_quantize_e4m3')

        for ui, u in enumerate(self.units):
            if ui and self._deferred:
                self.flush_deferred(pos=ui)
            uc = _UnitCtx(unit=u)
            src = acts[u.src]
            conv = u.main
            if u.dw is not None:
                dwc = u.dw
                src = self._dw_forward(dwc, src, mid_lens[ui])
                uc.mid = src
            y, stats, Tout = self._conv_forward(conv, src, need_stats=conv.has_bn and training)
            uc.y, uc.Tout = y, Tout
            coutp = y.shape[2]
            fins = [None, None]
            if conv.has_bn:
                if fold:
                    fins[0], (uc.scale, uc.shift, uc.mean, uc.invstd) = self._bn_fin_record(conv, stats, N * Tout, coutp)
                else:
                    uc.scale, uc.shift, uc.mean, uc.invstd = self._bn_finalize(conv, stats, N * Tout, coutp, training)
            if u.res is not None:
                rsrc = acts[u.res_src]
                y2, stats2, Tout2 = self._conv_forward(u.res, rsrc, need_stats=u.res.has_bn and training)
                if Tout2 != Tout or y2.shape != y.shape:
                    raise ValueError('residual branch shape mismatch')
                uc.y2 = y2
                if u.res.has_bn:
                    if fold:
                        fins[1], (uc.scale2, uc.shift2, uc.mean2, uc.invstd2) = self._bn_fin_record(u.res, stats2, N * Tout, coutp)
                    else:
                        uc.scale2, uc.shift2, uc.mean2, uc.invstd2 = self._bn_finalize(u.res, stats2, N * Tout, coutp, training)
            uc.lens_out = out_lens[ui]
            opl, opr, omode = self._in_pad_for(ui + 1)
            out_hi = torch.empty(N, opl + Tout + opr, coutp, dtype=torch.bfloat16, device=dev)
            out_lo = torch.empty_like(out_hi) if precise else None
            p = u.drop_p if training else 0.0
            if p > 0.0:
                uc.mask = torch.empty(N * Tout * (coutp // 8), dtype=torch.uint8, device=dev)
                uc.seed = torch.initial_seed() & 0xFFFFFFFFFFFFFFFF
                if self.dropout_counter is not None:
                    uc.offset = ui + 1
                else:
                    _dropout_calls += 1
                    uc.offset = _dropout_calls
            d = self._desc(uc, N, Tout, coutp, p, uc.lens_out)
            out_q, q_scale = None, 1.0
            if self.fp8 and coutp % 128 == 0 and self._fp8_consumers(ui + 1):
                out_q = torch.empty(N, opl + Tout + opr, coutp, dtype=torch.uint8, device=dev)
                q_scale = FP8_ACT_SCALE[u.act]
                if self._q_clipped is None or self._q_clipped.device != dev:
                    _lib.poison('fp8 saturation counter created')
                    self._q_clipped = torch.zeros(1, dtype=torch.int64, device=dev)
                d.q_clipped = self._q_clipped.data_ptr()
# ... 358 lines not shown
        xq = C.c_void_p(src.q.data_ptr() + row_off * src.CP)
        bstride, rows_total = src.rows * src.CP, N * src.rows - row_off
        y_f32 = int(y.dtype == torch.float32)
        st = stream_ptr()
        if AUTOTUNE:
            key = ('fp8', N, cin, cout, Tout, conv.kernel, conv.dilation, stats is not None, src.q.device.index)
            if _tune_once(key):
                check(lib.w2l_conv1d_igemm_fp8_tune(xq, bstride, rows_total, ptr(wq), ptr(y), y_f32, ptr(bias), ptr(stats), N,
                                                    cin, cout, Tout, conv.kernel, conv.dilation, TUNE_REPS, st),
                      'w2l_conv1d_igemm_fp8_tune')
                if stats is not None and getattr(self, '_stat_pool', None) is not None:
                    stats.zero_()
        with _timed('conv_igemm_fp8_kernel', flops):
            check(lib.w2l_conv1d_igemm_fp8(xq, bstride, rows_total, ptr(wq), ptr(y), y_f32, 1.0 / (src.q_scale * w_scale), None,
                                           ptr(bias), ptr(stats), N, cin, cout, Tout, conv.kernel, conv.dilation, st),
                  'w2l_conv1d_igemm_fp8')

    @staticmethod
    def _dw_weight(dwc: ConvSpec, cp: int) -> torch.Tensor:
        w = dwc.weight.detach()
        c, _, k = w.shape
        km = w.permute(2, 0, 1).reshape(k, c)
        if cp == c and km.is_contiguous():
            return km
        _lib.poison('depthwise weight of a padded channel count')
        out = torch.zeros(k, cp, dtype=torch.float32, device=w.device)
        out[:, :c] = km
        return out

    def _dw_forward(self, dwc: ConvSpec, src: Act, lens_mid, out=None) -> Act:
        if src.pad_l < dwc.pad_l or src.pad_r < dwc.pad_r:
            raise ValueError('activation buffer is not padded enough for its depthwise consumer')
        N, cp = src.N, src.CP
        Tmid = dwc.out_len(src.T)
        dev = src.hi.device
        if out is not None:
            mid_hi, mid_lo = out
        else:
            mid_hi = torch.empty(N, Tmid, cp, dtype=torch.bfloat16, device=dev)
            mid_lo = torch.empty_like(mid_hi) if self.precise else None
        row_off = src.pad_l - dwc.pad_l
        off = row_off * cp * 2
        w = self._dw_weight(dwc, cp)
        check(lib.w2l_dwconv_fwd(C.c_void_p(src.hi.data_ptr() + off),
                                 C.c_void_p(src.lo.data_ptr() + off) if src.lo is not None else None, src.rows, ptr(w),
                                 ptr(mid_hi), ptr(mid_lo), N, Tmid, cp, dwc.kernel, dwc.stride, dwc.dilation, ptr(lens_mid),
                                 stream_ptr()), 'w2l_dwconv_fwd')
        return Act(mid_hi, mid_lo, N, Tmid, dwc.cout, cp, 0, 0, PAD_ZERO, lens_mid)

    def _dw_backward(self, dwc: ConvSpec, dmid, src: Act, mid: Act, need_dx: bool, grads):
        g, per = dmid.buf, dmid.per
        N, cp = src.N, src.CP
        dev = g.device
        row_off = src.pad_l - dwc.pad_l
        k = dwc.kernel
        dwg = zeros((k, cp), torch.float32, dev)
        check(lib.w2l_dwconv_wgrad(ptr(g), int(g.dtype == torch.float32), per, _row_ptr(src.hi, row_off, cp, 2),
                                   _row_ptr(src.lo, row_off, cp, 2) if src.lo is not None else None, src.rows, ptr(dwg), N,
                                   mid.T, cp, k, dwc.stride, dwc.dilation, ptr(mid.lens), stream_ptr()), 'w2l_dwconv_wgrad')
        c = dwc.cout
        gw = dwg.view(k, cp, 1).permute(1, 2, 0)
        self._set(grads, dwc.weight, gw if cp == c else gw[:c], storage=dwg)
        if not need_dx:
            return None
        Tp = src.T + dwc.pad_l + dwc.pad_r
        tmid, lens_mid = mid.T, mid.lens
        if dwc.stride != 1:
            _lib.poison('strided depthwise data gradient')
            s_ = dwc.stride
            tup = (mid.T - 1) * s_ + 1
            up = torch.zeros(N, tup, cp, dtype=g.dtype, device=dev)
            up[:, 0:tup:s_] = g.view(N, per, cp)[:, :mid.T]
            g, per, tmid = up, tup, tup
            if lens_mid is not None:
                lens_mid = ((lens_mid - 1) * s_ + 1).clamp(min=0).to(torch.int32)
        dxp = torch.empty(N, Tp, cp, dtype=torch.float32 if self.precise else torch.bfloat16, device=dev)
        w = self._dw_weight(dwc, cp)
        check(lib.w2l_dwconv_dgrad(ptr(g), int(g.dtype == torch.float32), per, ptr(w), ptr(dxp),
                                   int(dxp.dtype == torch.float32), N, Tp, tmid, cp, k, dwc.dilation, ptr(lens_mid),
                                   stream_ptr()), 'w2l_dwconv_dgrad')
        return _GradSource(dxp, dwc.pad_l, dwc.pad_r, dwc.pad_mode, Tp)

    def _bn_finalize(self, conv: ConvSpec, stats, count, cp, training):
        dev = conv.weight.device
        scale, shift, mean, invstd = torch.empty(4, cp, dtype=torch.float32, device=dev).unbind(0)
        gamma = _padded_vec(conv.bn_weight, cp, 1.0)
        beta = _padded_vec(conv.bn_bias, cp, 0.0)
        rm, rv = conv.running_mean, conv.running_var
        padded_running = rm is not None and rm.numel() != cp
        if padded_running:
            rm_p, rv_p = _padded_vec(rm, cp, 0.0).clone(), _padded_vec(rv, cp, 1.0).clone()
        else:
            rm_p, rv_p = rm, rv
        if training:
            ntiles = stats.shape[0]
            check(lib.w2l_bn_finalize(ptr(stats), ntiles, cp, count, ptr(gamma), ptr(beta), conv.eps, conv.momentum,
                                      ptr(rm_p), ptr(rv_p), ptr(mean), ptr(invstd), ptr(scale), ptr(shift),
                                      stream_ptr()), 'w2l_bn_finalize')
            if padded_running:
                _lib.poison('running statistics of a padded channel count')
                rm.copy_(rm_p[: rm.numel()])
                rv.copy_(rv_p[: rv.numel()])
            if conv.num_batches_tracked is not None:
                self._nbt_pending.append(conv.num_batches_tracked)
        else:
            check(lib.w2l_bn_finalize(None, 0, cp, 1, ptr(gamma), ptr(beta), conv.eps, conv.momentum, ptr(rm_p),
                                      ptr(rv_p), ptr(mean), ptr(invstd), ptr(scale), ptr(shift), stream_ptr()),
                  'w2l_bn_finalize')
        return scale, shift, mean, invstd

    def _bn_fin_record(self, conv: ConvSpec, stats, count, cp):
        dev = conv.weight.device
        scale, shift, mean, invstd = torch.empty(4, cp, dtype=torch.float32, device=dev).unbind(0)
        gamma = _padded_vec(conv.bn_weight, cp, 1.0)
        beta = _padded_vec(conv.bn_bias, cp, 0.0)
        rm, rv = conv.running_mean, conv.running_var
        if rm is not None and rm.numel() != cp:
            rm_p, rv_p = _padded_vec(rm, cp, 0.0).clone(), _padded_vec(rv, cp, 1.0).clone()
            self._after_apply.append((rm, rv, rm_p, rv_p))
        else:
            rm_p, rv_p = rm, rv
        f = _lib.BnFin()
        f.partial, f.rows, f.count = stats.data_ptr(), stats.shape[0], count
        f.gamma, f.beta = gamma.data_ptr(), beta.data_ptr()
        f.eps, f.momentum = conv.eps, conv.momentum
        f.running_mean = rm_p.data_ptr() if rm_p is not None else None
        f.running_var = rv_p.data_ptr() if rv_p is not None else None
        f.mean, f.invstd, f.scale, f.shift = mean.data_ptr(), invstd.data_ptr(), scale.data_ptr(), shift.data_ptr()
        f._keep = (gamma, beta, rm_p, rv_p, stats)
        if conv.num_batches_tracked is not None:
            self._nbt_pending.append(conv.num_batches_tracked)
        return f, (scale, shift, mean, invstd)

    def _desc(self, uc: _UnitCtx, N, T, cp, p, lens, constant_stats: bool = False) -> BnActDesc:
        d = BnActDesc()
        d.N, d.T, d.C = N, T, cp
        d.y = uc.y.data_ptr()
        d.y_f32 = int(uc.y.dtype == torch.float32)
        for name in ('scale', 'shift', 'mean', 'invstd', 'scale2', 'shift2', 'mean2', 'invstd2'):
            t = getattr(uc, name)
            if constant_stats and name in ('mean', 'invstd', 'mean2', 'invstd2'):
                t = None
            setattr(d, name, t.data_ptr() if t is not None else None)
        d.y2 = uc.y2.data_ptr() if uc.y2 is not None else None
        d.act = uc.unit.act
        d.drop_p = float(p)
        d.seed, d.offset = uc.seed, uc.offset
        d.mask = uc.mask.data_ptr() if uc.mask is not None else None
        d.lens = lens.data_ptr() if lens is not None else None
        d.offset_dev = self.dropout_counter.data_ptr() if (self.dropout_counter is not None and p > 0.0) else None
        uc.keep.append(lens)
        return d

    def backward(self, ctx, g_out: torch.Tensor):
        try:
            return self._backward(ctx, g_out)
        finally:
            lib.w2l_conv_stats_mode(0)
            self._slot_pool = None

    def _backward(self, ctx, g_out: torch.Tensor):
        acts: List[Act] = ctx['acts']
        out = ctx['out']
        N = out.shape[0]
        dev = out.device
        grads = {}
        batch_stats = bool(ctx['training'])
        self._main_stream = torch.cuda.current_stream(dev) if dev.type == 'cuda' else None
        pool_elems = roundup(self.head.cout, 64) if self.head is not None else 0
        for uc in ctx['units']:
            if uc.unit.main.has_bn or (uc.unit.res is not None and uc.unit.res.has_bn):
                pool_elems += 4 * acts[uc.out_index].CP
        slot_need = 0
        if FAST_BN_BWD and not DETERMINISTIC_WGRAD and batch_stats and not self.precise and dev.type == 'cuda':
            slot_need = sum(STAT_SLOTS * 2 * acts[uc.out_index].CP for uc in ctx['units'] if uc.unit.main.has_bn and uc.unit.res is None)
        bias_need = 0
        if batch_stats:
            for u in self.units:
                for c in (u.main, u.res):
                    if c is not None and c.bias is not None and c.has_bn:
                        bias_need += roundup(c.cout, 64)
        zbuf = zeros(pool_elems + slot_need + bias_need, torch.float32, dev)
        small_pool = zbuf[:pool_elems]
        pool_off = 0
        self._slot_pool = [zbuf[pool_elems: pool_elems + slot_need], 0, {}] if slot_need else None
        self._zero_pool = [zbuf[pool_elems + slot_need:], 0] if bias_need else None
        lib.w2l_conv_stats_mode(STAT_SLOTS if self._slot_pool is not None else 0)
        lib.w2l_wgrad_deterministic(int(DETERMINISTIC_WGRAD))
        act_grads: List[List[_GradSource]] = [[] for _ in acts]
        if self.head is None:
            last = acts[-1]
            _lib.poison('open stack')
            gp = torch.zeros(N, last.T, last.CP, dtype=torch.float32, device=dev)
            gp[:, :, :last.C] = g_out.float().transpose(1, 2)
            act_grads[len(acts) - 1].append(_GradSource(gp, 0, 0, PAD_ZERO, last.T))
        else:
            self._plan_wgrad_groups(ctx)
            pool_off = self._head_backward(ctx, g_out, small_pool, grads, act_grads)
        self._units_backward(ctx, act_grads, small_pool, pool_off, grads, batch_stats)
        for recs in list(self._wg_pending.values()):
            for r in recs:
                self._wgrad_single(r, grads)
        self._wg_pending.clear()
        self._wg_of = {}
        ctx['input_grad'] = self.input_grad(ctx, act_grads[0]) if ctx.get('want_dx') and act_grads[0] else None
        if self.flat_ready is not None:
            _py(self.flat_ready, small_pool)
        elif self.grad_ready is not None:
            _py(self.grad_ready, None, small_pool, small_pool)
        if self._side_used:
            if JOIN_EVENTS is not None:
                em, es = torch.cuda.Event(enable_timing=True), torch.cuda.Event(enable_timing=True)
                em.record(self._main_stream)
                es.record(self._side)
                JOIN_EVENTS.append((em, es))
            _lib.stream_wait_stream(self._main_stream, self._side)
            self._side_used = False
        self._main_stream = None
        self._held.clear()
        self._dyq.clear()
        self._zero_pool = None
        self._slot_pool = None
        lib.w2l_conv_stats_mode(0)
        _flush_tune_cache()
        if self.backward_done is not None:
            _py(self.backward_done)
        return [grads.get(id(p)) for p in self.parameters()]

    def _head_backward(self, ctx, g_out, small_pool, grads, act_grads) -> int:
        precise = self.precise
        acts: List[Act] = ctx['acts']
        out = ctx['out']
        N, Th, L = out.shape
        dev = out.device
        st = stream_ptr
        pool_off = 0
        g_out = g_out.contiguous().float()
        glog = torch.empty_like(out)
        check(lib.w2l_log_softmax_bwd(ptr(g_out), ptr(out), N, Th, L, ctx['softmax_mode'], ptr(glog), st()),
              'w2l_log_softmax_bwd')
        head = self.head
        pk = pack_weights(head, precise)
        hh = roundup(Th, 64) - Th
        dy_hi = torch.empty(hh + N * (Th + hh), pk.coutp, dtype=torch.bfloat16, device=dev)
        dy_lo = torch.empty_like(dy_hi) if precise else None
        colsum = small_pool[pool_off: pool_off + pk.coutp]
        pool_off += roundup(head.cout, 64)
        check(lib.w2l_pad_cast(ptr(glog), N, Th, L, pk.coutp, hh, ptr(dy_hi), ptr(dy_lo), ptr(colsum), st()),
              'w2l_pad_cast')
        last = acts[-1]
        self._wgrad(head, pk, dy_hi, dy_lo, hh, Th, last, grads)
        if head.bias is not None:
            grads[id(head.bias)] = colsum[: head.cout]
        act_grads[len(acts) - 1].append(self._dgrad(head, pk, dy_hi, dy_lo, hh, Th, last, self._producer(ctx, len(acts) - 1)))
        return pool_off

    def _producer(self, ctx, act_index: int):
        mode = FUSED_BN_REDUCE
        if mode in (False, '0') or self.precise or act_index < 1:
            return None
        uc = ctx['units'][act_index - 1]
        u = uc.unit
        if u.res is not None or not u.main.has_bn or uc.y is None or uc.y.dtype != torch.bfloat16:
            return None
        if mode == 'auto' and uc.y.shape[0] * uc.y.shape[1] >= FUSED_BN_REDUCE_MAX_ROWS:
            return None
        return (uc, ctx['training'])

    def _units_backward(self, ctx, act_grads, small_pool, pool_off, grads, batch_stats: bool):
        precise = self.precise
        acts: List[Act] = ctx['acts']
        N = ctx['out'].shape[0]
        dev = ctx['out'].device
        amax_pool = (zeros((len(acts) + 1, 2, AMAX_SLOTS), torch.float32, dev)
                     if self.fp8 else None)
        for uc in reversed(ctx['units']):
            u = uc.unit
            oi = uc.out_index
            srcs = act_grads[oi]
            if not srcs:
                raise RuntimeError('activation without a gradient source')
            if len(srcs) > 2:
                raise NotImplementedError('more than two consumers of one activation')
            a_out = acts[oi]
            Tout, coutp = uc.Tout, a_out.CP
            p = u.drop_p if (ctx['training'] and uc.mask is not None) else 0.0
            d = self._desc(uc, N, Tout, coutp, p, uc.lens_out)
            g1 = self._gsrc(srcs[0])
            g2 = self._gsrc(srcs[1]) if len(srcs) > 1 else None
            chain, partial, nb, sums, pool_off = self._bn_bwd_reduce(uc, d, g1, g2, srcs, N, coutp, small_pool, pool_off, batch_stats)
            main, res = u.main, u.res
            need_dx_main = self._needs_grad(u.src, ctx)
            tail = roundup(Tout, 128 if self.fp8 else 64) - Tout
            h1 = max((main.kernel - 1) * main.dilation, tail)
            dy_hi = torch.empty(h1 + N * (Tout + h1), coutp, dtype=torch.bfloat16, device=dev)
            dy_lo = torch.empty_like(dy_hi) if precise else None
            dy2_hi = dy2_lo = None
            h2 = 0
            if res is not None:
                h2 = max((res.kernel - 1) * res.dilation, tail)
                dy2_hi = torch.empty(h2 + N * (Tout + h2), coutp, dtype=torch.bfloat16, device=dev)
                dy2_lo = torch.empty_like(dy2_hi) if precise else None
            if not batch_stats:
                d = self._desc(uc, N, Tout, coutp, p, uc.lens_out, constant_stats=True)
            fp8_dgrad = self.fp8 and coutp % 128 == 0 and (FP8_DGRAD == '1' or (FP8_DGRAD == 'auto' and
                                                                                  N * Tout >= FP8_DGRAD_MIN_ROWS))
            fp8_wgrad = self.fp8 and coutp % 128 == 0 and (FP8_WGRAD == '1' or (FP8_WGRAD == 'auto' and
                                                                                  N * Tout >= FP8_DGRAD_MIN_ROWS))
            amax = amax_pool[oi] if fp8_dgrad or fp8_wgrad else None
            amax_w = amax if fp8_wgrad else None
            amax_d = amax if fp8_dgrad else None
            self._bn_bwd_apply(chain, d, g1, g2, partial, nb, sums, dy_hi, dy_lo, h1, dy2_hi, dy2_lo, h2, amax)
            act_grads[oi] = []
            if main.has_bn:
                grads[id(main.bn_bias)] = sums[0, : main.cout]
                grads[id(main.bn_weight)] = sums[1, : main.cout]
            if res is not None and res.has_bn:
                grads[id(res.bn_bias)] = sums[2, : res.cout]
                grads[id(res.bn_weight)] = sums[3, : res.cout]
            pkm = pack_weights(main, precise)
            src = acts[u.src] if u.dw is None else uc.mid
            late = WGRAD_AFTER_DGRAD and u.dw is None and need_dx_main
            if not late:
                self._wgrad(main, pkm, dy_hi, dy_lo, h1, Tout, src, grads, amax=None if amax_w is None else amax_w[0],
                            defer=self._defer_ok(ctx, uc, main))
            if main.bias is not None:
                if main.has_bn and batch_stats:
                    grads[id(main.bias)] = self._zeros(main.cout, dev)
                else:
                    self._set(grads, main.bias, self._dy_colsum(dy_hi, dy_lo, h1, N, Tout, coutp, main.cout))
            if u.dw is not None:
                dmid = self._dgrad(main, pkm, dy_hi, dy_lo, h1, Tout, src,
                                   amax=None if amax_d is None else amax_d[0])
                gsrc = self._dw_backward(u.dw, dmid, acts[u.src], uc.mid, need_dx_main, grads)
                if gsrc is not None:
                    act_grads[u.src].append(gsrc)
            elif need_dx_main:
                act_grads[u.src].append(self._dgrad(main, pkm, dy_hi, dy_lo, h1, Tout, src, self._producer(ctx, u.src),
                                                    amax=None if amax_d is None else amax_d[0]))
            if late:
                self._wgrad(main, pkm, dy_hi, dy_lo, h1, Tout, src, grads, amax=None if amax_w is None else amax_w[0],
                            defer=self._defer_ok(ctx, uc, main))
            if res is not None:
                pkr = pack_weights(res, precise)
                rsrc = acts[u.res_src]
                self._wgrad(res, pkr, dy2_hi, dy2_lo, h2, Tout, rsrc, grads, amax=None if amax_w is None else amax_w[1],
                            defer=self._defer_ok(ctx, uc, res))
                if res.bias is not None:
                    if res.has_bn and batch_stats:
                        grads[id(res.bias)] = self._zeros(res.cout, dev)
                    else:
                        self._set(grads, res.bias, self._dy_colsum(dy2_hi, dy2_lo, h2, N, Tout, coutp, res.cout))
                if self._needs_grad(u.res_src, ctx):
                    act_grads[u.res_src].append(self._dgrad(res, pkr, dy2_hi, dy2_lo, h2, Tout, rsrc,
                                                            self._producer(ctx, u.res_src),
                                                            amax=None if amax_d is None else amax_d[1]))

    def _bn_bwd_reduce(self, uc, d, g1, g2, srcs, N, coutp, small_pool, pool_off, batch_stats):
        u, slot_pool = uc.unit, self._slot_pool
        if not (u.main.has_bn or (u.res is not None and u.res.has_bn)):
            return 'plain', None, 0, None, pool_off
        pd, pg1, pg2, st = C.byref(d), C.byref(g1), None if g2 is None else C.byref(g2), stream_ptr()
        ncomp = 4 if u.res is not None else 2
        def slots_ok():
            return bool(g2 is None and slot_pool is not None and lib.w2l_bn_bwd_fast_ok(pd, pg1, None))
        chain = 'fold' if FOLD_BN_FINALIZE and batch_stats else 'three'
        fused = [s_.partial for s_ in srcs if s_.partial is not None]
        if len(fused) == len(srcs) and ncomp == 2:
            fused = list({id(t): t for t in fused}.values())
            partial = fused[0] if len(fused) == 1 else torch.cat(fused, 0)
            if slot_pool is not None and len(fused) == 1 and slot_pool[2].get(id(uc)) is not None and slots_ok():
                chain = 'slots'
        elif FAST_BN_BWD and batch_stats and not self.precise and ncomp == 2 and slots_ok():
            chain, partial = 'slots', slot_pool[0][slot_pool[1]: slot_pool[1] + STAT_SLOTS * 2 * coutp].view(STAT_SLOTS, 2, coutp)
            slot_pool[1] += partial.numel()
            check(lib.w2l_bn_act_bwd_reduce_slots(pd, pg1, ptr(partial), STAT_SLOTS, st), 'w2l_bn_act_bwd_reduce_slots')
        else:
            partial = torch.empty(lib.w2l_bn_bwd_blocks(N, uc.Tout, coutp), ncomp, coutp, dtype=torch.float32, device=small_pool.device)
            check(lib.w2l_bn_act_bwd_reduce(pd, pg1, pg2, ptr(partial), st), 'w2l_bn_act_bwd_reduce')
        nb, sums = partial.shape[0], small_pool[pool_off: pool_off + 4 * coutp].view(4, coutp)
        if chain == 'three':
            check(lib.w2l_bn_bwd_finalize(ptr(partial), nb, coutp, ncomp, ptr(sums), st), 'w2l_bn_bwd_finalize')
        uc.keep.append((partial, sums))
        return chain, partial, nb, sums, pool_off + 4 * coutp

    def _bn_bwd_apply(self, chain, d, g1, g2, partial, nb, sums, dy_hi, dy_lo, h1, dy2_hi, dy2_lo, h2, amax):
        pd, pg1, pg2, st = C.byref(d), C.byref(g1), None if g2 is None else C.byref(g2), stream_ptr()
        if chain == 'slots':
            check(lib.w2l_bn_act_bwd_apply_slots(pd, pg1, ptr(partial), nb, ptr(sums), ptr(dy_hi), h1, ptr(amax), st), 'w2l_bn_act_bwd_apply_slots')
        elif chain == 'fold':
            check(lib.w2l_bn_act_bwd_apply_fin(pd, pg1, pg2, ptr(partial), nb, ptr(sums), ptr(dy_hi), ptr(dy_lo), h1, ptr(dy2_hi),
                                               ptr(dy2_lo), h2, ptr(amax), st), 'w2l_bn_act_bwd_apply_fin')
        else:
            check(lib.w2l_bn_act_bwd_apply_amax(pd, pg1, pg2, ptr(sums), ptr(dy_hi), ptr(dy_lo), h1, ptr(dy2_hi), ptr(dy2_lo), h2,
                                                ptr(amax), st), 'w2l_bn_act_bwd_apply')

    def _needs_grad(self, act_index: int, ctx=None) -> bool:
        return act_index != 0 or bool(ctx and ctx.get('want_dx'))

    def input_grad(self, ctx, srcs) -> torch.Tensor:
        N, C0, T0 = ctx['x_shape']
        a0 = ctx['acts'][0]
# ... 476 lines not shown
```

### wav2letter_pytorch_amd/layers.py

```python
from __future__ import annotations

import math
import os
from itertools import chain
from typing import Callable, Optional

import torch
import torch.nn as nn

from .engine import ACT_NONE, PAD_ZERO, ConvSpec, StackEngine, UnitSpec, _GradSource


def default_precision(cfg=None) -> str:
    p = None
    if cfg is not None:
        try:
            p = cfg.get('precision', None)
        except Exception:
            p = None
    p = p or os.environ.get('W2L_PRECISION', 'bf16')
    if p not in ('bf16', 'fp32', 'fp8'):
        raise ValueError(f"precision must be 'bf16', 'fp32' or 'fp8', got {p!r}")
    return p


class Conv1d(nn.Module):

    def __init__(self, in_channels, out_channels, kernel_size, stride=1, padding=0, dilation=1, groups=1, bias=True,
                 init='torch_default'):
        super().__init__()
        k = kernel_size[0] if isinstance(kernel_size, (tuple, list)) else kernel_size
        self.in_channels, self.out_channels = in_channels, out_channels
        self.kernel_size = (k,)
        self.stride = (stride,)
        self.padding = (padding,)
        self.dilation = (dilation,)
        self.groups = groups
        phys = torch.empty(k, out_channels, in_channels // groups)
        self.weight = nn.Parameter(phys.permute(1, 2, 0))
        self.bias = nn.Parameter(torch.empty(out_channels)) if bias else None
        self.reset_parameters(init)

    def reset_parameters(self, init='torch_default'):
        tmp = torch.empty(self.weight.shape)
        if init == 'xavier_uniform':
            nn.init.xavier_uniform_(tmp, gain=1.0)
        else:
            nn.init.kaiming_uniform_(tmp, a=math.sqrt(5))
        with torch.no_grad():
            self.weight.copy_(tmp)
            if self.bias is not None:
                fan_in = self.weight.shape[1] * self.weight.shape[2]
                bound = 1 / math.sqrt(fan_in) if fan_in > 0 else 0
                self.bias.copy_(torch.empty(self.bias.shape).uniform_(-bound, bound))

    def extra_repr(self):
        return (f'{self.in_channels}, {self.out_channels}, kernel_size={self.kernel_size}, stride={self.stride}, '
                f'padding={self.padding}, dilation={self.dilation}, bias={self.bias is not None}')

    def forward(self, x):
        if self.groups != 1:
            return depthwise_forward(self, x, None)
        pad = self.padding[0]
        eng = solo_engine(self, lambda: [UnitSpec(main=conv_spec(self, None, pad, pad, PAD_ZERO, 'conv'), src=0, act=ACT_NONE)])
        out, _ = run_stack(eng, x, None, self.training)
        return out


class BatchNorm1d(nn.Module):

    def __init__(self, num_features, eps=1e-5, momentum=0.1):
        super().__init__()
        self.num_features, self.eps, self.momentum = num_features, eps, momentum
        self.affine = True
        self.track_running_stats = True
        self.weight = nn.Parameter(torch.ones(num_features))
        self.bias = nn.Parameter(torch.zeros(num_features))
        self.register_buffer('running_mean', torch.zeros(num_features))
        self.register_buffer('running_var', torch.ones(num_features))
        self.register_buffer('num_batches_tracked', torch.tensor(0, dtype=torch.long))

    def extra_repr(self):
        return f'{self.num_features}, eps={self.eps}, momentum={self.momentum}'

    def forward(self, x):
        raise RuntimeError('BatchNorm1d holds parameters and running statistics only: the kernels normalise the output of '
                           'the convolution in front of it (Conv1dBlock / JasperBlock), there is no conv-less BatchNorm pass')


class _DepthwiseFn(torch.autograd.Function):

    @staticmethod
    def forward(ctx, x, conv, lens, weight, bias):
        import ctypes as C
        from . import _lib
        from ._lib import check, lib, ptr, stream_ptr
        from .engine import Act, padded_channels
        _lib.require_device(x)
        prec = getattr(conv, 'precision', None) or default_precision()
        eng = StackEngine([], None, 0, precise=prec == 'fp32')
        pad = conv.padding[0]
        spec = conv_spec(conv, None, pad, pad, PAD_ZERO, 'depthwise', depthwise=True)
        x = x.contiguous().float()
        n, c, t = x.shape
        cp = padded_channels(c)
        dev = x.device
        lens_dev = None if lens is None else lens.to(device=dev, dtype=torch.int32)
        a_hi = torch.empty(n, t + 2 * pad, cp, dtype=torch.bfloat16, device=dev)
        a_lo = torch.empty_like(a_hi) if eng.precise else None
        check(lib.w2l_nct_to_ntc(ptr(x), n, c, t, cp, pad, pad, PAD_ZERO, ptr(lens_dev), ptr(a_hi), ptr(a_lo), stream_ptr()),
              'w2l_nct_to_ntc')
        src = Act(a_hi, a_lo, n, t, c, cp, pad, pad, PAD_ZERO, lens_dev)
        mid = eng._dw_forward(spec, src, None)
        out = mid.hi[:, :, :c].float()
        if mid.lo is not None:
            out = out + mid.lo[:, :, :c].float()
        out = out.transpose(1, 2).contiguous()
        if bias is not None:
            out = out + bias.detach()[None, :, None]
        ctx.state = (eng, spec, src, mid, bias is not None)
        return out

    @staticmethod
    def backward(ctx, g):
        eng, spec, src, mid, has_bias = ctx.state
        n, c, t, cp = src.N, src.C, src.T, src.CP
        gp = torch.zeros(n, mid.T, cp, dtype=torch.float32, device=g.device)
        gp[:, :, :c] = g.float().transpose(1, 2)
        grads = {}
        gsrc = eng._dw_backward(spec, _GradSource(gp, 0, 0, PAD_ZERO, mid.T), src, mid, True, grads)
        dxp, pl, per = gsrc.buf, gsrc.pad_l, gsrc.per
        dx = dxp.view(n, per, cp)[:, pl:pl + t, :c].float()
        if src.lens is not None:
            dx = dx * (torch.arange(t, device=dx.device)[None, :, None] < src.lens.long()[:, None, None])
        ctx.state = None
        return dx.transpose(1, 2).contiguous(), None, None, grads[id(spec.weight)], (g.sum((0, 2)) if has_bias else None)


def depthwise_forward(conv: 'Conv1d', x, lens):
    if conv.groups != conv.in_channels or conv.in_channels != conv.out_channels:
        raise NotImplementedError('grouped convolution with 1 < groups < channels is not built (not reachable from the '
                                  'config: jasper.py:440-449 never passes groups)')
    return _DepthwiseFn.apply(x, conv, lens, conv.weight, conv.bias)


def conv_spec(conv: Conv1d, bn: Optional[BatchNorm1d], pad_l: int, pad_r: int, pad_mode: int, name: str = '',
              depthwise: bool = False) -> ConvSpec:
    if depthwise:
        if conv.groups != conv.in_channels or conv.in_channels != conv.out_channels:
            raise NotImplementedError('only depthwise (groups == channels) grouped convolutions are built')
    elif conv.groups != 1:
        raise NotImplementedError('grouped convolution (1 < groups < channels) is not reachable from the config')
    spec = ConvSpec(weight=conv.weight, bias=conv.bias, kernel=conv.kernel_size[0], stride=conv.stride[0],
                    dilation=conv.dilation[0], pad_l=pad_l, pad_r=pad_r, pad_mode=pad_mode, name=name)
    if bn is not None:
        spec.bn_weight, spec.bn_bias = bn.weight, bn.bias
        spec.running_mean, spec.running_var = bn.running_mean, bn.running_var
        spec.num_batches_tracked = bn.num_batches_tracked
        spec.eps, spec.momentum = bn.eps, bn.momentum
    return spec


class _StackFn(torch.autograd.Function):

    @staticmethod
    def forward(ctx, x, engine: StackEngine, lens, training: bool, softmax_mode: int, holder: dict, *params):
        want_dx = bool(x.requires_grad)
        out, ectx = engine.forward(x, lens, training, softmax_mode, want_input_grad=want_dx)
        ctx.engine, ctx.ectx = engine, ectx
        if holder.get('keep_ctx'):
            holder['ctx'] = ectx
        holder['lens_out'] = ectx['lens_out']
        return out

    @staticmethod
    def backward(ctx, g):
        from . import replay
        rp = ctx.engine.__dict__.get('_replayer')
        if rp is not None:
            rp.before_eager()
            rp.pending = None
        replay._last_backward[0] = None
        grads = ctx.engine.backward(ctx.ectx, g)
        dx = ctx.ectx.get('input_grad')
        ctx.ectx = None
        return (dx, None, None, None, None, None, *grads)


def run_stack(engine: StackEngine, x, lens, training: bool, softmax_mode: int = 0, keep_ctx: bool = False):
    from . import replay
    holder = {'keep_ctx': keep_ctx}
    rp = replay.replayer_for(engine) if x.is_cuda else None
    if rp is not None:
        plan = rp.plan_forward(x, lens, training, softmax_mode, keep_ctx)
        if plan is not None:
            out = replay._ReplayFn.apply(x, engine, lens, softmax_mode, holder, plan[0], plan[1], *engine.parameters())
            return out, holder.get('lens_out')
        rp.before_eager()
        rp.flush_pending()
    out = _StackFn.apply(x, engine, lens, training, softmax_mode, holder, *engine.parameters())
    if keep_ctx:
        return out, holder.get('lens_out'), holder.get('ctx')
    return out, holder.get('lens_out')


def run_infer(engine: StackEngine, x, lens, softmax_mode: int = 0):
    from . import replay
    rp = replay.replayer_for(engine) if x.is_cuda else None
    if rp is not None:
        rp.before_eager()
        rp.flush_pending()
    return engine.infer(x, lens, softmax_mode)


def solo_engine(owner: nn.Module, units_fn: Callable[[], list]) -> StackEngine:
    prec = getattr(owner, 'precision', None) or default_precision()
    key = tuple((id(t), t.device) for t in chain(owner.parameters(), owner.buffers())) + (prec,)
    hit = owner.__dict__.get('_solo_engine')
    if hit is None or hit[0] != key:
        from .base_asr_models import EngineSlot
        hit = EngineSlot((key, StackEngine(units_fn(), None, 0, precise=prec == 'fp32', fp8=prec == 'fp8')))
        owner.__dict__['_solo_engine'] = hit
    return hit[1]
```

### wav2letter_pytorch_amd/replay.py

```python
from __future__ import annotations

import os
import weakref
from typing import Optional

import numpy as np
import torch

from . import _lib
from ._lib import check, lib, ptr

ENABLED = os.environ.get('W2L_REPLAY', '1') != '0'
WARM_STEPS = int(os.environ.get('W2L_REPLAY_WARM', '2'))
MAX_GROUPS = int(os.environ.get('W2L_REPLAY_MAX_SHAPES', '8'))
MAX_FAILURES = 3
FP8_EAGER_EVERY = 256
FP8_EAGER_STEPS = 10
VERBOSE = os.environ.get('W2L_REPLAY_VERBOSE', '0') == '1'
LENS_RING = 4
TRANSIENT = ('fp8 weight scale', 'kernel plans were measured', 'measuring launches', 'workspace grown', 'created', 'table built',
             'momentum buffer')

_last_backward = [None]
STATS = {'recorded': 0, 'recorded_O': 0, 'replayed_F': 0, 'replayed_B': 0, 'replayed_O': 0, 'replayed_X': 0, 'poisoned': []}


def _say(msg):
    if VERBOSE:
        print('[w2l replay] ' + msg, flush=True)


_POOLS: list = []


class _Lease:
    __slots__ = ('__weakref__',)


def new_pool(lease):
    pool = torch.cuda.MemPool()
    _POOLS.append((pool, weakref.ref(lease)))
    return pool


def purge_pools():
    if _POOLS and any(ref() is None for _, ref in _POOLS):
        dead = [e for e in _POOLS if e[1]() is None]
        _POOLS[:] = [e for e in _POOLS if e[1]() is not None]
        del dead


class RecordSet:

    def __init__(self, group, index):
        self.group = weakref.ref(group)
        self.index = index
        self.reset()

    def reset(self):
        self.lease = _Lease()
        self.lease_O = _Lease()
        self.lease_X = _Lease()
        self.pool = self.pool_O = self.pool_X = None
        self.F = self.B = self.O = self.X = None
        self.O_sig = self.X_sig = None
        self.x_static = self.x_ref = None
        self.g_static = None
        self.out = None
        self.ectx = None
        self.lens_out = None
        self.lens_static = None
        self.grads = None
        self.deferred = []
        self.O_ptrs = None
        self.O_spare = None

    def ensure_pool(self):
        if self.pool is None:
            self.pool = new_pool(self.lease)
        return self.pool


class Group:
    def __init__(self, key):
        self.key = key
        self.sets = [RecordSet(self, 0), RecordSet(self, 1)]
        self.next = 0
        self.seen = 0
        self.failures = 0
        self.disabled = None
        self.fp8_epoch = None
        self.replays = 0
        self.eager_left = 0
        self.last_use = 0


def opt_signature(opt):
    own = getattr(opt, '_replay_signature', None)
    if own is not None:
        return own()
    clip = opt._clip_signature() if hasattr(opt, '_clip_signature') else None
    return tuple((g['lr'], g['momentum'], g['weight_decay'], g['nesterov'], g['dampening'], g.get('maximize', False))
                 for g in opt.param_groups) + (opt.__dict__.get('_w2l_state_epoch', 0), clip)


class StepReplayer:

    def __init__(self, engine):
        self.engine = weakref.ref(engine)
        self.groups = {}
        self.pending: Optional[RecordSet] = None
        self.counter = None
        self.counter_host = 0
        self.clock = 0
        self.after_replayed_O = False
        self.opt_stream = None
        self.first_seen = {}
        self._fused_ws = None

    def _mode_flags(self):
        from . import engine as E
        return (E.DETERMINISTIC_WGRAD, E.DEALT_WGRAD, E.DEFER_SPREAD, E.WGRAD_AFTER_DGRAD, E.FUSED_BN_REDUCE, E.FOLD_BN_FINALIZE,
                E.FOLD_BN_FWD, E.FAST_BN_BWD, E.STAT_SLOTS, E.FP8_DGRAD, E.FP8_WGRAD, E.WGROUP_MAX, E.AUTOTUNE,
                os.environ.get('W2L_WGRAD_GROUPS', 'auto'))

    def plan_forward(self, x, lens, training, softmax_mode, keep_ctx):
        from . import engine as E
        eng = self.engine()
        if (not ENABLED or eng is None or not training or keep_ctx or not x.is_cuda or x.requires_grad or not torch.is_grad_enabled()
                or eng.head is None or eng.precise or eng.grad_ready is not None or eng.flat_ready is not None
                or eng.backward_done is not None or eng.grad_reduce_start is not None or eng.dropout_counter is not None
                or E.KERNEL_TIMER is not None or E.JOIN_EVENTS is not None or _lib._trace['saved'] or _lib.recording() is not None
                or x.dtype != torch.float32 or not x.is_contiguous() or (lens is not None and lens.is_cuda)
                or E.DEFER_SPREAD != 'start' or torch.cuda.is_current_stream_capturing()):
            return None
        purge_pools()
        defer = eng.defer_wgrad if eng.deferred is not None else 0
        key = (tuple(x.shape), softmax_mode, lens is None, x.device.index, _lib.raw_stream(), self._mode_flags(),
               defer if isinstance(defer, int) else tuple(sorted(defer)), id(eng.deferred), bool(eng.overlap_wgrad),
               torch.initial_seed(), E._wev_epoch[0])
        self.clock += 1
        g = self.groups.get(key)
        if g is None:
            n = self.first_seen.get(key, 0) + 1
            if len(self.first_seen) > 4096:
                self.first_seen.clear()
            self.first_seen[key] = n
            if n <= WARM_STEPS:
                return None
            if len(self.groups) >= MAX_GROUPS:
                victim = min(self.groups.values(), key=lambda v: v.last_use)
                if (self.pending is not None and self.pending.group() is victim) or self.clock - victim.last_use < 4 * MAX_GROUPS:
                    return None
                del self.groups[victim.key]
            free, total = torch.cuda.mem_get_info(x.device)
            if free < 0.2 * total:
                return None
            g = self.groups[key] = Group(key)
            g.seen = WARM_STEPS
            g.fp8_epoch = E._fp8_epoch[0]
        g.last_use = self.clock
        if g.disabled is not None:
            return None
        if g.fp8_epoch != E._fp8_epoch[0]:
            g.fp8_epoch = E._fp8_epoch[0]
            self._drop(g)
        g.seen += 1
        if g.seen <= WARM_STEPS:
            return None
        if eng.fp8:
            if g.eager_left > 0:
                g.eager_left -= 1
                return None
            if g.replays >= FP8_EAGER_EVERY:
                g.replays = 0
                g.eager_left = FP8_EAGER_STEPS - 1
                self._age_fp8_weights(FP8_EAGER_EVERY)
                return None
        if self._weights_moved(eng):
            return None
        s = g.sets[g.next]
        if self.pending is s:
            return None
        g.next ^= 1
        return ('replay' if s.F is not None and s.B is not None else 'record'), s

    def _weights_moved(self, eng) -> bool:
        moved = False
        for w in self._conv_weights(eng):
            if '_w2l_ready_ev' not in w.__dict__:
                continue
            pk = (getattr(w, '_w2l_pack', None) or {}).get(False)
            if pk is None or pk.src_ptr != w.data_ptr():
                self.groups.clear()
                self.pending = None
                return True
            if pk.version != w._version:
                moved = True
        return moved

    def _conv_weights(self, eng):
        ws = self._fused_ws
        if ws is None or ws[0] is not eng.units:
            ws = self._fused_ws = (eng.units, [c.weight for u in eng.units for c in (u.main, u.res) if c is not None] +
                                   ([eng.head.weight] if eng.head is not None else []))
        return ws[1]

    def _age_fp8_weights(self, n):
        eng = self.engine()
        for u in eng.units:
            for c in (u.main, u.res):
                st = c.weight.__dict__.get('_w2l_fp8') if c is not None else None
                if st is not None:
                    st['age'] += n

    def _drop(self, g):
        for s in g.sets:
            if self.pending is s:
                continue
            s.reset()

    def fail(self, s: RecordSet, why: str):
        g = s.group()
        s.reset()
        if g is None:
            return
        STATS['poisoned'].append(why)
        _say(f'recording dropped: {why}')
        if any(t in why for t in TRANSIENT):
            g.seen = 0
            return
        g.failures += 1
        if g.failures >= MAX_FAILURES:
            g.disabled = why
            for t in g.sets:
                if self.pending is not t:
                    t.reset()

    def before_eager(self):
        if self.after_replayed_O and self.opt_stream is not None:
            _lib.stream_wait_stream(_lib.raw_stream(), self.opt_stream)
        self.after_replayed_O = False

    def flush_pending(self):
        eng = self.engine()
        s = self.pending
        if s is None or not eng._deferred:
            self.pending = None
            return
        opt = eng.deferred
        if opt is None or not all(eng._stepped(r) for r in eng._deferred) or s.B is None:
            self.pending = None
            return
        hp = opt._deferred_state()['hp']
        sig = tuple(hp[id(r.conv.weight)][2] for r in eng._deferred) + (opt.__dict__.get('_w2l_state_epoch', 0),)
        if s.X is not None and s.X_sig != sig:
            s.X = None
        if s.X is not None:
            s.X.replay()
            from . import engine as E
            for r in eng._deferred:
                w = r.conv.weight
                for pk in (getattr(w, '_w2l_pack', None) or {}).values():
                    pk.ready, pk.version = E.weight_event(w), w._version
            eng._deferred = []
            eng._side_used = True
            STATS['replayed_X'] += 1
            self.pending = None
            return
        s.lease_X = _Lease()
        s.pool_X = new_pool(s.lease_X)
        with torch.cuda.use_mem_pool(s.pool_X), _lib.Recorder() as rec:
            eng.flush_deferred(pos=0)
        ph = rec.finish()
        self.pending = None
        if ph is None or eng._deferred:
            s.pool_X = None
            g = s.group()
            if g is not None:
                g.failures += 1
                if g.failures >= MAX_FAILURES:
                    g.disabled = rec.poisoned or 'held-back weight gradients not launched in one piece'
            STATS['poisoned'].append(rec.poisoned or 'phase X incomplete')
            return
        s.X, s.X_sig = ph, sig

    def sync_counter(self, dev, advance):
        from . import engine as E
        if self.counter is None or self.counter.device != dev:
            self.counter = torch.zeros(1, dtype=torch.int64, device=dev)
            self.counter_host = 0
        if self.counter_host != E._dropout_calls:
            self.counter.fill_(E._dropout_calls)
            self.counter_host = E._dropout_calls
        E._dropout_calls += advance
        self.counter_host += advance
        return self.counter


def replayer_for(engine) -> Optional[StepReplayer]:
    if not ENABLED:
        return None
    rp = engine.__dict__.get('_replayer')
    if rp is None:
        rp = engine.__dict__['_replayer'] = StepReplayer(engine)
    return rp


def lens_rows_host(engine, lens):
    cur = lens.numpy().astype(np.int32)
    cur_f = cur.astype(np.float32)
    rows, mid_has, out_has = [cur], [], []
    one = np.float32(1.0)
    mids = []
    outs = []
    for u in engine.units:
        has_mid = False
        if u.dw is not None and u.update_lens:
            c = u.dw
            cur_f = (cur_f + np.float32(c.pad_l + c.pad_r) - np.float32(c.dilation * (c.kernel - 1)) - one) / np.float32(c.stride) + one
            cur = cur_f.astype(np.int32)
            mids.append(cur)
            has_mid = True
        mid_has.append(has_mid)
        if u.update_lens:
            c = u.main
            cur_f = (cur_f + np.float32(c.pad_l + c.pad_r) - np.float32(c.dilation * (c.kernel - 1)) - one) / np.float32(c.stride) + one
            cur = cur_f.astype(np.int32)
        out_has.append(bool(u.mask_out))
        if u.mask_out:
            outs.append(cur)
    return np.stack(rows + mids + outs), mid_has, out_has, torch.from_numpy(cur_f.copy())


class _ReplayFn(torch.autograd.Function):

    @staticmethod
    def forward(ctx, x, engine, lens, softmax_mode, holder, mode, rset, *params):
        rp = replayer_for(engine)
        ctx.engine, ctx.rset, ctx.mode, ctx.softmax_mode = engine, rset, mode, softmax_mode
        if mode == 'replay':
            out = _replay_forward(rp, engine, rset, x, lens)
        else:
            out = _record_forward(rp, engine, rset, x, lens, softmax_mode)
        holder['lens_out'] = rset.lens_out
        return out

    @staticmethod
    def backward(ctx, g):
        engine, rset = ctx.engine, ctx.rset
        rp = replayer_for(engine)
        n = len(engine.parameters())
        if any(p.grad is not None for p, _ in (rset.grads or [])) or (rset.grads is None and
                                                                      any(p.grad is not None for p in engine.parameters())):
            if rset.ectx is None:
                raise RuntimeError('replayed step: p.grad is already set (gradient accumulation) and the eager context of this '
                                   'record set is gone; call optimizer.zero_grad(set_to_none=True) before backward(), or set W2L_REPLAY=0')
            rp.before_eager()
            grads = engine.backward(rset.ectx, g)
            rp.pending = None
            _last_backward[0] = None
            return (None,) * 7 + tuple(grads)
        if ctx.mode == 'replay':
            _replay_backward(rp, engine, rset, g)
        else:
            _record_backward(rp, engine, rset, g)
        return (None,) * (7 + n)


def _upload_lens(rset, engine, lens):
    rows, mid_has, out_has, final = lens_rows_host(engine, lens)
    st = rset.lens_static
    if st is None or tuple(st['host'].shape) != rows.shape:
        return None, None
    ring = st.setdefault('ring', [(st['host'], st['event'])])
    if len(ring) < LENS_RING:
        ring.append((torch.empty(rows.shape, dtype=torch.int32, pin_memory=True), _lib.Event()))
        host, ev = ring[-1]
    else:
        st['turn'] = (st.get('turn', 0) + 1) % LENS_RING
        host, ev = ring[st['turn']]
        ev.synchronize()
    host.numpy()[...] = rows
    st['dev'].copy_(host, non_blocking=True)
    ev.record()
    return st, final


def _replay_forward(rp, engine, rset, x, lens):
    from . import engine as E
    if lens is not None:
        st, final = _upload_lens(rset, engine, lens)
        if st is None:
            raise RuntimeError('replayed step: the length table of this record set does not fit the batch')
        rset.lens_out = final
    rset.x_static.copy_(x, non_blocking=True)
    rp.flush_pending()
    if engine._deferred:
        rp.before_eager()
        engine.flush_deferred(pos=0)
    rp.sync_counter(x.device, len(engine.units) + 1)
    rset.F.replay()
    E.drop_infer_state()
    g = rset.group()
    if g is not None:
        g.replays += 1
    STATS['replayed_F'] += 1
    return rset.out.detach()


def _record_forward(rp, engine, rset, x, lens, softmax_mode):
    from . import engine as E
    rp.before_eager()
    rp.flush_pending()
    if engine._deferred:
        engine.flush_deferred(pos=0)
    rset.reset()
    pool = rset.ensure_pool()
    n_drop = len(engine.units) + 1
    counter = rp.sync_counter(x.device, n_drop)
    tune0 = (len(E._tuned_shapes), len(E._wgroup_forms))
    with torch.cuda.use_mem_pool(pool):
        rset.x_static = torch.empty_like(x)
        rset.x_static.copy_(x)
        rset.x_ref = None
        if lens is not None:
            rows, _, _, _ = lens_rows_host(engine, lens)
            rset.lens_static = {'host': torch.empty(rows.shape, dtype=torch.int32, pin_memory=True),
                                'dev': torch.empty(rows.shape, dtype=torch.int32, device=x.device), 'event': _lib.Event()}
        engine.dropout_counter = counter
        engine._lens_static = rset.lens_static
        try:
            with _lib.Recorder() as rec:
                out, ectx = engine.forward(rset.x_static, lens, True, softmax_mode, want_input_grad=False)
                check(lib.w2l_counter_add(ptr(counter), n_drop, _lib.raw_stream()), 'w2l_counter_add')
        finally:
            engine.dropout_counter = None
            engine._lens_static = None
    ph = rec.finish()
    rset.ectx, rset.out, rset.lens_out = ectx, out, ectx['lens_out']
    if ph is not None and tune0 != (len(E._tuned_shapes), len(E._wgroup_forms)):
        ph, rec.poisoned = None, 'kernel plans were measured during the step'
    if ph is None:
        why = rec.poisoned
        rset_out, rset_ctx = out, ectx
        rp.fail(rset, 'forward: ' + str(why))
        rset.ectx, rset.out, rset.lens_out = rset_ctx, rset_out, rset_ctx['lens_out']
        return out
    rset.F = ph
    return out


def _assign_grads(rset):
    for p, gbuf in rset.grads:
        if gbuf is not None:
            p.grad = gbuf.detach()


def _record_backward(rp, engine, rset, g):
    from . import engine as E
    pool = rset.ensure_pool()
    tune0 = (len(E._tuned_shapes), len(E._wgroup_forms))
    with torch.cuda.use_mem_pool(pool):
        rset.g_static = torch.empty(g.shape, dtype=torch.float32, device=g.device)
        rset.g_static.copy_(g)
        with _lib.Recorder() as rec:
            grads = engine.backward(rset.ectx, rset.g_static)
    ph = rec.finish() if rset.F is not None else None
    params = engine.parameters()
    why = rec.poisoned
    if ph is not None and tune0 != (len(E._tuned_shapes), len(E._wgroup_forms)):
        ph, why = None, 'kernel plans were measured during the step'
    fixed = []
    for p, gr in zip(params, grads):
        if gr is not None and (gr.shape != p.shape or any(a != b for n, a, b in zip(p.shape, gr.stride(), p.stride()) if n > 1)):
            gr = torch.empty_like(p).copy_(gr)
            ph, why = None, 'gradient of a padded channel count'
        fixed.append((p, gr))
    rset.grads = fixed
    _assign_grads(rset)
    rset.deferred = list(engine._deferred)
    if ph is None:
        if rset.F is not None:
            rp.fail(rset, 'backward: ' + str(why))
        rp.pending = None
        _last_backward[0] = None
        return
    rset.B = ph
    rp.pending = rset if rset.deferred else None
    _last_backward[0] = (weakref.ref(rp), rset)
    STATS['recorded'] += 1
    _say(f'recorded set {rset.index}: F {rset.F.n_calls} calls, B {rset.B.n_calls} calls, {len(rset.deferred)} held-back gradients')


def _replay_backward(rp, engine, rset, g):
    rset.g_static.copy_(g, non_blocking=True)
    rset.B.replay()
    engine._side_used = False
    if rset.deferred:
        opt = engine.deferred
        tok = opt.token() if opt is not None else 0
        for r in rset.deferred:
            r.token = tok
        engine._deferred = list(rset.deferred)
        rp.pending = rset
    else:
        rp.pending = None
    _assign_grads(rset)
    _last_backward[0] = (weakref.ref(rp), rset)
    STATS['replayed_B'] += 1


def optimizer_step(opt, eager_body) -> bool:
    hit = _last_backward[0]
    _last_backward[0] = None
    if hit is None or not ENABLED:
        return False
    rp, rset = hit[0](), hit[1]
    if rp is None or rset.B is None or rset.grads is None:
        return False
    engine = rp.engine()
    if engine is None:
        return False
    mine = opt.__dict__.get('_w2l_param_ids')
    if mine is None:
        mine = opt.__dict__['_w2l_param_ids'] = frozenset(id(p) for g in opt.param_groups for p in g['params'])
    if any(id(p) not in mine for p, _ in rset.grads):
        return False
    extra = opt.__dict__.get('_w2l_extra_params')
    if extra is None or extra[0]() is not engine:
        ids = frozenset(id(p) for p in engine.parameters())
        extra = opt.__dict__['_w2l_extra_params'] = (weakref.ref(engine), [p for g in opt.param_groups for p in g['params'] if id(p) not in ids])
    watched = [(p, None) for p in extra[1]]
    sig = (opt_signature(opt), bool(opt.overlap), _lib.raw_stream())
    if rset.O_sig != sig and rset.O_spare is not None and rset.O_spare[1] == sig:
        cur = (rset.O, rset.O_sig, rset.O_ptrs, rset.lease_O, rset.pool_O)
        rset.O, rset.O_sig, rset.O_ptrs, rset.lease_O, rset.pool_O = rset.O_spare
        rset.O_spare = cur if cur[0] is not None else None
    if rset.O is not None and rset.O_sig == sig:
        for (p, gbuf), want in zip(rset.grads + watched, rset.O_ptrs):
            have = p.grad.data_ptr() if p.grad is not None else 0
            if have != want:
                return False
        rset.O.replay()
        from .engine import drop_infer_state
        drop_infer_state()
        for w in rp._conv_weights(engine):
            if '_w2l_ready_ev' not in w.__dict__:
                torch.autograd.graph.increment_version(w)
        st, dst = opt._side_state(), opt._deferred_state()
        dst['seq'] += 1
        st['pending'] = True
        rp.after_replayed_O = True
        rp.opt_stream = st['stream']
        STATS['replayed_O'] += 1
        return True
    if rset.O is not None and rset.O_sig is not None and rset.O_sig[0][-1:] != sig[0][-1:]:
        rset.O_spare = (rset.O, rset.O_sig, rset.O_ptrs, rset.lease_O, rset.pool_O)
        rset.O = rset.O_sig = None
    rset.lease_O = _Lease()
    rset.pool_O = new_pool(rset.lease_O)
    with torch.cuda.use_mem_pool(rset.pool_O), _lib.Recorder() as rec:
        eager_body()
    ph = rec.finish()
    if ph is None:
        rset.pool_O = None
        g = rset.group()
        if g is not None:
            g.failures += 1
            if g.failures >= MAX_FAILURES:
                g.disabled = 'optimizer step: ' + str(rec.poisoned)
        STATS['poisoned'].append('optimizer step: ' + str(rec.poisoned))
        _say('optimizer phase dropped: ' + str(rec.poisoned))
        return True
    rset.O, rset.O_sig = ph, sig
    STATS['recorded_O'] += 1
    rset.O_ptrs = [p.grad.data_ptr() if p.grad is not None else 0 for p, _ in rset.grads + watched]
    rp.opt_stream = opt._side_state()['stream']
    return True


def audit(engine) -> list:
    rp = engine.__dict__.get('_replayer')
    if rp is None:
        return []
    sets = [s for g in rp.groups.values() for s in g.sets]
    if rp.pending is not None and not any(rp.pending is s for s in sets):
        sets.append(rp.pending)
    todo = []
    for s in sets:
        phases = [('F', s.F), ('B', s.B), ('O', s.O), ('X', s.X)] + ([('O_spare', s.O_spare[0])] if s.O_spare is not None else [])
        own = [p.id for p in (s.pool, s.pool_O, s.pool_X, s.O_spare[4] if s.O_spare is not None else None) if p is not None]
        for name, ph in phases:
            if ph is not None:
                todo.append(('set %d %s' % (s.index, name), ph, own))
    if not todo:
        return []
    snap = torch.cuda.memory._snapshot()
    out = []
    for label, ph, own in todo:
        if ph.dev_ptrs is None:
            out.append(label + ': recorded without _lib.AUDIT, its pointers are unknown')
            continue
        out += [label + ' ' + f for f in _lib.classify_pointers(ph.dev_ptrs, snap, own)]
    return out


def report(engine) -> dict:
    rp = engine.__dict__.get('_replayer')
    out = {'enabled': ENABLED, 'shapes': []}
    if rp is None:
        return out
    for g in rp.groups.values():
        out['shapes'].append({'input': list(g.key[0]), 'seen': g.seen, 'disabled': g.disabled, 'failures': g.failures,
                              'sets': [{'F': s.F.n_calls if s.F else None, 'B': s.B.n_calls if s.B else None,
                                        'O': s.O.n_calls if s.O else None, 'X': s.X.n_calls if s.X else None,
                                        'python_items': sum(1 for ph in (s.F, s.B, s.O, s.X) if ph for it in ph.items if it[0] == 'py')}
                                       for s in g.sets]})
    return out
```

Measured before the change: 2.550 million.

## Fuse CTC gradient, log-softmax backward and bf16 dy packing at the loss seam

Splits the CTC loss into an alpha/beta pass in forward and a fused backward kernel. In backward, that kernel computes the CTC gradient, applies the log-softmax backward and writes padded bf16 dy rows straight into the model's backward input layout. This removes the separate fp32 grad tensor round trip and the extra log-softmax-backward and pad/cast kernels between loss and model. It adds a colsum entry point and threads a 'seam' handle through eager, record and replay paths, patching replayed call arguments. The cost is considerable bookkeeping complexity and new fallback paths.

Measured after the change: 2.553 million (median of 6 runs). No clear change (+0.1%).

```diff
diff --git a/include/w2l_hip.h b/include/w2l_hip.h
--- a/include/w2l_hip.h
+++ b/include/w2l_hip.h
@@ -22,6 +22,7 @@
 
 int w2l_pad_cast(const float* g, int N, int T, int C, int CP, int halo, void* out_hi, void* out_lo, float* colsum,
                  void* stream);
+int w2l_colsum(const float* g, int64_t rows, int C, int CP, float* colsum, void* stream);
 
 int w2l_conv_stat_tiles(int N, int Tout);
 int w2l_conv1d_igemm(const void* xp, int64_t x_bstride, int64_t x_rows_total, const void* w, void* y, int y_f32,
@@ -234,6 +235,13 @@
 int w2l_ctc_loss(const float* log_probs, const int32_t* targets, const int32_t* input_lengths,
                  const int32_t* target_lengths, int N, int T, int C, int Smax, int blank, int zero_infinity,
                  float* nll, float* loss, float* grad, void* workspace, void* stream);
+int w2l_ctc_alpha_beta(const float* log_probs, const int32_t* targets, const int32_t* input_lengths,
+                       const int32_t* target_lengths, int N, int T, int C, int Smax, int blank, int zero_infinity,
+                       float* nll_raw, float* nll, float* loss, void* workspace, void* stream);
+int w2l_ctc_grad_dy(const float* log_probs, const int32_t* targets, const int32_t* input_lengths,
+                    const int32_t* target_lengths, int N, int T, int C, int Smax, int blank, int zero_infinity,
+                    const float* nll_raw, const void* workspace, const float* upstream, int CP, int halo, void* dy,
+                    float* glogits, float* grad, float* nll, float* loss, void* stream);
 
 int64_t w2l_ctc_align_workspace_bytes(int N, int T, int Smax);
 int w2l_ctc_align(const float* x, const int32_t* input_lengths, const int32_t* targets, int64_t target_stride,
diff --git a/wav2letter_pytorch_amd/_lib.py b/wav2letter_pytorch_amd/_lib.py
--- a/wav2letter_pytorch_amd/_lib.py
+++ b/wav2letter_pytorch_amd/_lib.py
@@ -72,6 +72,7 @@
                                 c_p]),
     'w2l_nct_to_ntc': (c_i, [c_p, c_i, c_i, c_i, c_i, c_i, c_i, c_i, c_p, c_p, c_p, c_p]),
     'w2l_pad_cast': (c_i, [c_p, c_i, c_i, c_i, c_i, c_i, c_p, c_p, c_p, c_p]),
+    'w2l_colsum': (c_i, [c_p, c_i64, c_i, c_i, c_p, c_p]),
     'w2l_conv_stat_tiles': (c_i, [c_i, c_i]),
     'w2l_conv1d_igemm': (c_i, [c_p, c_i64, c_i64, c_p, c_p, c_i, c_i, c_p, c_p, c_i, c_i, c_i, c_i, c_i, c_i, c_i, c_p]),
     'w2l_conv1d_igemm_tune': (c_i, [c_p, c_i64, c_i64, c_p, c_p, c_i, c_p, c_p, c_i, c_i, c_i, c_i, c_i, c_i, c_i, c_i, c_p]),
@@ -142,6 +143,9 @@
     'w2l_log_softmax_bwd': (c_i, [c_p, c_p, c_i, c_i, c_i, c_i, c_p, c_p]),
     'w2l_ctc_workspace_bytes': (c_i64, [c_i, c_i, c_i]),
     'w2l_ctc_loss': (c_i, [c_p, c_p, c_p, c_p, c_i, c_i, c_i, c_i, c_i, c_i, c_p, c_p, c_p, c_p, c_p]),
+    'w2l_ctc_alpha_beta': (c_i, [c_p, c_p, c_p, c_p, c_i, c_i, c_i, c_i, c_i, c_i, c_p, c_p, c_p, c_p, c_p]),
+    'w2l_ctc_grad_dy': (c_i, [c_p, c_p, c_p, c_p, c_i, c_i, c_i, c_i, c_i, c_i, c_p, c_p, c_p, c_i, c_i, c_p, c_p, c_p, c_p, c_p,
+                              c_p]),
     'w2l_asg_workspace_bytes': (c_i64, [c_i, c_i, c_i, c_i]),
     'w2l_asg_loss': (c_i, [c_p, c_p, c_p, c_p, c_p, c_i, c_i, c_i, c_i, c_i, c_i, c_p, c_p, c_p, c_p, c_p, c_p, c_i64, c_p]),
     'w2l_asg_viterbi_workspace_bytes': (c_i64, [c_i, c_i, c_i]),
@@ -272,7 +276,8 @@
     'w2l_bn_act_bwd_apply_fin': 'bn_act_bwd_apply_kernel', 'w2l_sgd_pack': 'sgd_pack_kernel', 'w2l_pack_weights': 'pack_weights_kernel',
     'w2l_sgd_pack_clip': 'sgd_pack_kernel', 'w2l_adam_pack': 'adam_pack_kernel', 'w2l_grad_sqnorm_multi': 'grad_norm_kernels',
     'w2l_asg_loss': 'asg_kernels', 'w2l_asg_viterbi': 'asg_viterbi_kernel',
-    'w2l_ctc_loss': 'ctc_kernels', 'w2l_log_softmax_fwd': 'log_softmax_fwd', 'w2l_log_softmax_bwd': 'log_softmax_bwd',
+    'w2l_ctc_loss': 'ctc_kernels', 'w2l_ctc_alpha_beta': 'ctc_kernels', 'w2l_ctc_grad_dy': 'ctc_grad_dy_kernel',
+    'w2l_colsum': 'colsum_kernel', 'w2l_log_softmax_fwd': 'log_softmax_fwd', 'w2l_log_softmax_bwd': 'log_softmax_bwd',
     'w2l_nct_to_ntc': 'nct_to_ntc_kernel', 'w2l_pad_cast': 'pad_cast_kernel', 'w2l_quantize_e4m3': 'quantize_e4m3',
     'w2l_quantize_e4m3_dyn': 'quantize_e4m3_dyn', 'w2l_dwconv_fwd': 'dw_fwd_kernel', 'w2l_dwconv_dgrad': 'dw_dgrad_kernel',
     'w2l_dwconv_wgrad': 'dw_wgrad_kernel', 'w2l_argmax': 'argmax_kernel', 'w2l_novograd_pack': 'novograd_pack_kernel',
diff --git a/wav2letter_pytorch_amd/csrc/ctc.hip b/wav2letter_pytorch_amd/csrc/ctc.hip
--- a/wav2letter_pytorch_amd/csrc/ctc.hip
+++ b/wav2letter_pytorch_amd/csrc/ctc.hip
@@ -216,12 +216,14 @@
     (void)nll_out;
 }
 
-__global__ void ctc_loss_reduce_kernel(float* nll, const int32_t* tg_len, int N, int Smax, int zero_inf, float* loss) {
-    __shared__ float red[256];
+__device__ __forceinline__ void ctc_loss_mean(const float* nll, float* nll_out, const int32_t* tg_len, int N, int Smax,
+                                              int zero_inf, float* loss, float* red) {
     float s = 0.f;
     for (int n = threadIdx.x; n < N; n += 256) {
         float v = nll[n];
-        if (zero_inf && !(v < INFINITY)) { v = 0.f; nll[n] = 0.f; }
+        const bool clean = zero_inf && !(v < INFINITY);
+        if (clean) v = 0.f;
+        if (nll_out && (clean || nll_out != nll)) nll_out[n] = v;
         const int S = min(max(tg_len[n], 0), Smax);
         s += v / (float)max(S, 1);
     }
@@ -232,6 +234,84 @@
         __syncthreads();
     }
     if (threadIdx.x == 0) loss[0] = red[0] / (float)N;
+}
+
+__global__ __launch_bounds__(256) void ctc_loss_reduce_kernel(const float* nll, float* nll_out, const int32_t* tg_len, int N,
+                                                               int Smax, int zero_inf, float* loss) {
+    __shared__ float red[256];
+    ctc_loss_mean(nll, nll_out, tg_len, N, Smax, zero_inf, loss, red);
+}
+
+__global__ __launch_bounds__(256) void ctc_grad_dy_kernel(CtcParams p, const float* upstream, int CP, int halo, int64_t rows,
+                                                           bf16_raw* dy, float* glog, float* grad, float* nll_out,
+                                                           float* loss) {
+#pragma clang fp contract(off)
+    __shared__ float acc_all[4][64];
+    __shared__ float red[256];
+    if (blockIdx.x == 0 && loss) ctc_loss_mean(p.nll, nll_out, p.tg_len, p.N, p.Smax, p.zero_inf, loss, red);
+    const int lane = threadIdx.x & 63, w = threadIdx.x >> 6;
+    const int64_t r = (int64_t)blockIdx.x * 4 + w;
+    if (r >= rows) return;
+    bf16_raw* out = dy + r * CP;
+    const int P = p.T + halo;
+    const int64_t q = r - halo;
+    const int n = q >= 0 ? (int)(q / P) : 0;
+    const int t = (int)(q - (int64_t)n * P);
+    if (q < 0 || t >= p.T) {
+        for (int c = lane; c < CP; c += 64) out[c] = 0;
+        return;
+    }
+    float* acc = acc_all[w];
+    const int S = min(max(p.tg_len[n], 0), p.Smax);
+    const int Tn = min(max(p.in_len[n], 0), p.T);
+    const int L = 2 * S + 1;
+    const float nll = p.nll[n];
+    const bool inf = !(nll < INFINITY);
+    const bool masked = t >= Tn || (inf && p.zero_inf);
+    const int64_t row = (int64_t)n * p.T + t;
+    const float* lp = p.lp + row * p.C;
+    const float up = upstream ? upstream[0] : 1.f;
+    acc[lane] = 0.f;
+    float m = NEG_INF;
+    float post_scale = 0.f;
+    if (!masked) {
+        const float* al = p.alpha + row * p.L;
+        const float* be = p.beta + row * p.L;
+        const int32_t* tg = p.targets + (int64_t)n * p.Smax;
+        for (int s = lane; s < L; s += 64) {
+            const int c = (s & 1) ? tg[s >> 1] : p.blank;
+            const float v = al[s] + be[s];
+            if (v > NEG_INF && (unsigned)c < (unsigned)p.C) m = fmaxf(m, v - lp[c]);
+        }
+#pragma unroll
+        for (int k = 32; k > 0; k >>= 1) m = fmaxf(m, __shfl_xor(m, k, 64));
+        __builtin_amdgcn_wave_barrier();
+        if (m > NEG_INF) {
+            for (int s = lane; s < L; s += 64) {
+                const int c = (s & 1) ? tg[s >> 1] : p.blank;
+                const float v = al[s] + be[s];
+                if (v > NEG_INF && (unsigned)c < (unsigned)p.C) atomicAdd(&acc[c], expf(v - lp[c] - m));
+            }
+        }
+        __builtin_amdgcn_wave_barrier();
+        post_scale = m > NEG_INF ? expf(m + nll) : 0.f;
+    }
+    const float gs = 1.f / ((float)p.N * (float)max(S, 1));
+    const int c = lane;
+    float e = 0.f, gu = 0.f;
+    if (c < p.C) {
+        e = expf(lp[c]);
+        const float g = masked ? 0.f : __builtin_fmaf(-acc[c], post_scale, e) * gs;
+        if (grad) grad[row * p.C + c] = g;
+        gu = g * up;
+    }
+    float s = 0.f;
+    s += gu;
+#pragma unroll
+    for (int k = 32; k > 0; k >>= 1) s += __shfl_xor(s, k, 64);
+    const float gl = __builtin_fmaf(-e, s, gu);
+    if (c < p.C && glog) glog[row * p.C + c] = gl;
+    for (int cc = lane; cc < CP; cc += 64) out[cc] = cc < p.C ? f32_to_bf16_bits(gl) : (bf16_raw)0;
 }
 
 __global__ __launch_bounds__(256) void argmax_kernel(const float* probs, int64_t rows, int C, int32_t* idx) {
@@ -275,20 +355,20 @@
     return 2 * (int64_t)N * T * (2 * Smax + 1) * (int64_t)sizeof(float);
 }
 
-extern "C" int w2l_ctc_loss(const float* log_probs, const int32_t* targets, const int32_t* input_lengths,
+static CtcParams ctc_params(const float* log_probs, const int32_t* targets, const int32_t* input_lengths,
                             const int32_t* target_lengths, int N, int T, int C, int Smax, int blank, int zero_infinity,
-                            float* nll, float* loss, float* grad, void* workspace, void* stream) {
-    W2L_CHECK_ARG(log_probs && input_lengths && target_lengths && nll && loss && workspace, "ctc_loss: null pointer");
-    W2L_CHECK_ARG(targets || Smax == 0, "ctc_loss: null targets");
-    W2L_CHECK_ARG(N > 0 && T > 0 && C > 0 && C <= 64 && Smax >= 0 && blank >= 0 && blank < C, "ctc_loss: bad sizes");
-    const int L = 2 * Smax + 1;
-    W2L_CHECK_ARG(L <= 8 * 1024, "ctc_loss: target length %d too long (max 4095)", Smax);
+                            float* nll, void* workspace) {
     CtcParams p;
     p.lp = log_probs; p.targets = targets; p.in_len = input_lengths; p.tg_len = target_lengths;
-    p.N = N; p.T = T; p.C = C; p.Smax = Smax; p.L = L; p.blank = blank; p.zero_inf = zero_infinity;
+    p.N = N; p.T = T; p.C = C; p.Smax = Smax; p.L = 2 * Smax + 1; p.blank = blank; p.zero_inf = zero_infinity;
     p.alpha = (float*)workspace;
-    p.beta = p.alpha + (int64_t)N * T * L;
+    p.beta = p.alpha + (int64_t)N * T * p.L;
     p.nll = nll;
+    return p;
+}
+
+static int ctc_launch_alpha_beta(const CtcParams& p, void* stream) {
+    const int N = p.N, T = p.T, C = p.C, L = p.L;
     static const int kWide[] = {64, 128, 192, 256, 320, 384, 448, 512, 640, 768, 896, 1024};
     int nt = 1024;
     for (int w : kWide)
@@ -335,12 +415,63 @@
     }
 #undef W2L_CTC_LAUNCH
     W2L_CHECK_LAUNCH();
+    return 0;
+}
+
+#define W2L_CTC_CHECK_ARGS(what)                                                                                      \
+    W2L_CHECK_ARG(targets || Smax == 0, what ": null targets");                                                       \
+    W2L_CHECK_ARG(N > 0 && T > 0 && C > 0 && C <= 64 && Smax >= 0 && blank >= 0 && blank < C, what ": bad sizes");    \
+    W2L_CHECK_ARG(2 * Smax + 1 <= 8 * 1024, what ": target length %d too long (max 4095)", Smax)
+
+extern "C" int w2l_ctc_loss(const float* log_probs, const int32_t* targets, const int32_t* input_lengths,
+                            const int32_t* target_lengths, int N, int T, int C, int Smax, int blank, int zero_infinity,
+                            float* nll, float* loss, float* grad, void* workspace, void* stream) {
+    W2L_CHECK_ARG(log_probs && input_lengths && target_lengths && nll && loss && workspace, "ctc_loss: null pointer");
+    W2L_CTC_CHECK_ARGS("ctc_loss");
+    const CtcParams p = ctc_params(log_probs, targets, input_lengths, target_lengths, N, T, C, Smax, blank, zero_infinity, nll,
+                                   workspace);
+    if (int rc = ctc_launch_alpha_beta(p, stream)) return rc;
     if (grad) {
         hipLaunchKernelGGL(ctc_grad_kernel, dim3((T + 3) / 4, N), dim3(256), 0, (hipStream_t)stream, p, grad, nll);
         W2L_CHECK_LAUNCH();
     }
-    hipLaunchKernelGGL(ctc_loss_reduce_kernel, dim3(1), dim3(256), 0, (hipStream_t)stream, nll, target_lengths, N,
-                       p.Smax, zero_infinity, loss);
+    hipLaunchKernelGGL(ctc_loss_reduce_kernel, dim3(1), dim3(256), 0, (hipStream_t)stream, (const float*)nll, nll,
+                       target_lengths, N, p.Smax, zero_infinity, loss);
+    W2L_CHECK_LAUNCH();
+    return 0;
+}
+
+extern "C" int w2l_ctc_alpha_beta(const float* log_probs, const int32_t* targets, const int32_t* input_lengths,
+                                  const int32_t* target_lengths, int N, int T, int C, int Smax, int blank, int zero_infinity,
+                                  float* nll_raw, float* nll, float* loss, void* workspace, void* stream) {
+    W2L_CHECK_ARG(log_probs && input_lengths && target_lengths && nll_raw && workspace, "ctc_alpha_beta: null pointer");
+    W2L_CHECK_ARG(nll != nll_raw, "ctc_alpha_beta: nll and nll_raw must be two buffers");
+    W2L_CTC_CHECK_ARGS("ctc_alpha_beta");
+    const CtcParams p = ctc_params(log_probs, targets, input_lengths, target_lengths, N, T, C, Smax, blank, zero_infinity,
+                                   nll_raw, workspace);
+    if (int rc = ctc_launch_alpha_beta(p, stream)) return rc;
+    if (loss) {
+        hipLaunchKernelGGL(ctc_loss_reduce_kernel, dim3(1), dim3(256), 0, (hipStream_t)stream, (const float*)nll_raw, nll,
+                           target_lengths, N, p.Smax, zero_infinity, loss);
+        W2L_CHECK_LAUNCH();
+    }
+    return 0;
+}
+
+extern "C" int w2l_ctc_grad_dy(const float* log_probs, const int32_t* targets, const int32_t* input_lengths,
+                               const int32_t* target_lengths, int N, int T, int C, int Smax, int blank, int zero_infinity,
+                               const float* nll_raw, const void* workspace, const float* upstream, int CP, int halo, void* dy,
+                               float* glogits, float* grad, float* nll, float* loss, void* stream) {
+    W2L_CHECK_ARG(log_probs && input_lengths && target_lengths && nll_raw && workspace && dy, "ctc_grad_dy: null pointer");
+    W2L_CHECK_ARG(nll != nll_raw, "ctc_grad_dy: nll and nll_raw must be two buffers");
+    W2L_CTC_CHECK_ARGS("ctc_grad_dy");
+    W2L_CHECK_ARG(CP >= C && halo >= 0, "ctc_grad_dy: bad dy layout (CP %d, halo %d)", CP, halo);
+    const CtcParams p = ctc_params(log_probs, targets, input_lengths, target_lengths, N, T, C, Smax, blank, zero_infinity,
+                                   (float*)nll_raw, (void*)workspace);
+    const int64_t rows = (int64_t)halo + (int64_t)N * (T + halo);
+    W2L_CHECK_ARG((rows + 3) / 4 <= 0x7fffffff, "ctc_grad_dy: %lld rows", (long long)rows);
+    hipLaunchKernelGGL(ctc_grad_dy_kernel, dim3((unsigned)((rows + 3) / 4)), dim3(256), 0, (hipStream_t)stream, p, upstream, CP,
+                       halo, rows, (bf16_raw*)dy, glogits, grad, nll, loss);
     W2L_CHECK_LAUNCH();
     return 0;
 }
diff --git a/wav2letter_pytorch_amd/csrc/pack.hip b/wav2letter_pytorch_amd/csrc/pack.hip
--- a/wav2letter_pytorch_amd/csrc/pack.hip
+++ b/wav2letter_pytorch_amd/csrc/pack.hip
@@ -397,3 +397,11 @@
     }
     return 0;
 }
+
+extern "C" int w2l_colsum(const float* g, int64_t rows, int C, int CP, float* colsum, void* stream) {
+    W2L_CHECK_ARG(g && colsum, "colsum: null pointer");
+    W2L_CHECK_ARG(rows > 0 && C > 0 && CP >= C, "colsum: bad sizes");
+    hipLaunchKernelGGL(colsum_kernel, dim3(CP), dim3(256), 0, (hipStream_t)stream, g, rows, C, CP, colsum);
+    W2L_CHECK_LAUNCH();
+    return 0;
+}
diff --git a/wav2letter_pytorch_amd/csrc/replay.hip b/wav2letter_pytorch_amd/csrc/replay.hip
--- a/wav2letter_pytorch_amd/csrc/replay.hip
+++ b/wav2letter_pytorch_amd/csrc/replay.hip
@@ -250,6 +250,7 @@
     W2L_E(w2l_bn_act_bwd_apply_amax), W2L_E(w2l_bn_act_bwd_apply_fin), W2L_E(w2l_bn_act_bwd_apply_slots),
     W2L_E(w2l_quantize_e4m3), W2L_E(w2l_quantize_e4m3_dyn),
     W2L_E(w2l_log_softmax_fwd), W2L_E(w2l_log_softmax_bwd), W2L_E(w2l_ctc_loss), W2L_E(w2l_asg_loss), W2L_E(w2l_argmax),
+    W2L_E(w2l_ctc_alpha_beta), W2L_E(w2l_ctc_grad_dy), W2L_E(w2l_colsum),
     W2L_E(w2l_rccl_all_reduce),
 };
 constexpr int kNumEntries = (int)(sizeof(kEntries) / sizeof(kEntries[0]));
diff --git a/wav2letter_pytorch_amd/ctc_loss.py b/wav2letter_pytorch_amd/ctc_loss.py
--- a/wav2letter_pytorch_amd/ctc_loss.py
+++ b/wav2letter_pytorch_amd/ctc_loss.py
@@ -5,6 +5,90 @@
 
 from . import _lib
 from ._lib import check, lib, ptr, stream_ptr
+
+_ZERO = {}
+_I32_CACHE = {}
+
+
+def _as_i32(role, t, dev):
+    t = torch.as_tensor(t)
+    if t.dtype == torch.int32 and t.device == dev and t.is_contiguous():
+        return t
+    if torch.cuda.is_current_stream_capturing():
+        return t.to(device=dev, dtype=torch.int32).contiguous()
+    key = (role, dev.index)
+    hit = _I32_CACHE.get(key)
+    if hit is not None and hit[3] is t and hit[0] == t.data_ptr() and hit[1] == t._version and hit[2] == t.shape:
+        return hit[4]
+    out = t.to(device=dev, dtype=torch.int32).contiguous()
+    _I32_CACHE[key] = (t.data_ptr(), t._version, t.shape, t, out)
+    return out
+
+
+class LossSeam:
+    __slots__ = ('node', 'lp', 'tg', 'il', 'tl', 'ws', 'nll_raw', 'smax', 'blank', 'zero_inf', 'up', 'zero', 'state', 'src')
+
+    def __init__(self):
+        self.node = None
+        self.up = None
+        self.state = 'new'
+        self.src = None
+
+    def tensors(self):
+        return [self.lp, self.tg, self.il, self.tl, self.ws, self.nll_raw, self.up, self.zero]
+
+    def launch(self, CP, halo, dy, glog):
+        n, t, c = self.lp.shape
+        check(lib.w2l_ctc_grad_dy(ptr(self.lp), ptr(self.tg), ptr(self.il), ptr(self.tl), n, t, c, self.smax, self.blank,
+                                  self.zero_inf, ptr(self.nll_raw), ptr(self.ws), ptr(self.up), CP, halo, ptr(dy), ptr(glog),
+                                  None, None, None, stream_ptr()), 'w2l_ctc_grad_dy')
+
+    def gradient(self):
+        n, t, c = self.lp.shape
+        dev = self.lp.device
+        ws = torch.empty(max(int(lib.w2l_ctc_workspace_bytes(n, t, self.smax)), 4), dtype=torch.uint8, device=dev)
+        nll = torch.empty(n, dtype=torch.float32, device=dev)
+        loss = torch.empty(1, dtype=torch.float32, device=dev)
+        grad = torch.empty(n, t, c, dtype=torch.float32, device=dev)
+        check(lib.w2l_ctc_loss(ptr(self.lp), ptr(self.tg), ptr(self.il), ptr(self.tl), n, t, c, self.smax, self.blank,
+                               self.zero_inf, ptr(nll), ptr(loss), ptr(grad), ptr(ws), stream_ptr()), 'w2l_ctc_loss')
+        return grad
+
+
+def _engine_node(log_probs):
+    fn = log_probs.grad_fn
+    if fn is None or fn.name() != 'TransposeBackward0' or {getattr(fn, '_saved_dim0', None), getattr(fn, '_saved_dim1', None)} != {0, 1}:
+        return None
+    node, index = fn.next_functions[0]
+    if index != 0 or not getattr(node, 'w2l_seam_ok', False):
+        return None
+    return node
+
+
+def _plan_seam(log_probs, lp):
+    from . import engine as E
+    if not E.FUSED_LOSS_SEAM or log_probs.dtype != torch.float32 or torch.cuda.is_current_stream_capturing():
+        return None
+    node = _engine_node(log_probs)
+    if node is None or lp.shape[2] > 64:
+        return None
+    if (lp.data_ptr(), tuple(lp.shape), tuple(lp.stride())) != node.w2l_seam_out:
+        return None
+    old = getattr(node, 'w2l_seam', None)
+    if old is not None:
+        old.state = 'cancelled'
+        return None
+    return node
+
+
+def claim(node, g):
+    h = getattr(node, 'w2l_seam', None)
+    if h is None or h.state != 'armed':
+        return None, g
+    h.state, h.node = 'used', None
+    if g.data_ptr() == h.zero.data_ptr() and not any(g.stride()) and g.shape == h.lp.shape:
+        return h, None
+    return None, g + h.gradient() * h.up
 
 
 class _CTCFn(torch.autograd.Function):
@@ -18,13 +102,25 @@
         dev = lp.device
         if targets.dim() != 2:
             raise NotImplementedError('CTCLoss: targets must be 2-D [N, S_max] (padded), as the collator produces')
-        tg = targets.to(device=dev, dtype=torch.int32).contiguous()
-        il = torch.as_tensor(input_lengths).to(device=dev, dtype=torch.int32).contiguous()
-        tl = torch.as_tensor(target_lengths).to(device=dev, dtype=torch.int32).contiguous()
-        smax = tg.shape[1]
-        ws = torch.empty(max(int(lib.w2l_ctc_workspace_bytes(n, t, smax)), 4), dtype=torch.uint8, device=dev)
+        smax = targets.shape[1]
+        ctx.seam = None
         nll = torch.empty(n, dtype=torch.float32, device=dev)
         loss = torch.empty(1, dtype=torch.float32, device=dev)
+        node = _plan_seam(log_probs, lp)
+        if node is not None:
+            h = node.w2l_seam_buffers(lp, targets, input_lengths, target_lengths, smax, int(blank), int(zero_infinity))
+            if h is not None:
+                check(lib.w2l_ctc_alpha_beta(ptr(h.lp), ptr(h.tg), ptr(h.il), ptr(h.tl), n, t, c, smax, h.blank, h.zero_inf,
+                                             ptr(h.nll_raw), ptr(nll), ptr(loss), ptr(h.ws), stream_ptr()), 'w2l_ctc_alpha_beta')
+                h.node, h.state, h.up = node, 'new', None
+                node.w2l_seam = h
+                ctx.seam = h
+                ctx.nll = nll
+                return loss[0]
+        tg = _as_i32('tg', targets, dev)
+        il = _as_i32('il', input_lengths, dev)
+        tl = _as_i32('tl', target_lengths, dev)
+        ws = torch.empty(max(int(lib.w2l_ctc_workspace_bytes(n, t, smax)), 4), dtype=torch.uint8, device=dev)
         grad = torch.empty(n, t, c, dtype=torch.float32, device=dev)
         check(lib.w2l_ctc_loss(ptr(lp), ptr(tg), ptr(il), ptr(tl), n, t, c, smax, int(blank), int(zero_infinity),
                                ptr(nll), ptr(loss), ptr(grad), ptr(ws), stream_ptr()), 'w2l_ctc_loss')
@@ -34,8 +130,41 @@
 
     @staticmethod
     def backward(ctx, g):
+        h = ctx.seam
+        if h is not None:
+            n, t, c = h.lp.shape
+            if (h.state == 'new' and getattr(h.node, 'w2l_seam', None) is h and g.numel() == 1 and g.dtype == torch.float32
+                    and g.device == h.lp.device and not torch.cuda.is_current_stream_capturing()):
+                h.state, h.up = 'armed', g.reshape(1)
+                return h.zero.expand(t, n, c), None, None, None, None, None
+            h.node = None
+            grad = h.gradient() * g
+            return grad.transpose(0, 1), None, None, None, None, None
         grad = ctx.grad * g
         return grad.transpose(0, 1), None, None, None, None, None
+
+
+def new_seam(lp, targets, input_lengths, target_lengths, smax, blank, zero_inf, own_ints=False):
+    dev = lp.device
+    n, t, c = lp.shape
+    h = LossSeam()
+    h.lp = lp
+    if own_ints:
+        h.tg = torch.empty(tuple(targets.shape), dtype=torch.int32, device=dev)
+        h.il = torch.empty(n, dtype=torch.int32, device=dev)
+        h.tl = torch.empty(n, dtype=torch.int32, device=dev)
+    else:
+        h.tg = _as_i32('tg', targets, dev)
+        h.il = _as_i32('il', input_lengths, dev)
+        h.tl = _as_i32('tl', target_lengths, dev)
+    h.ws = torch.empty(max(int(lib.w2l_ctc_workspace_bytes(n, t, smax)), 4), dtype=torch.uint8, device=dev)
+    h.nll_raw = torch.empty(n, dtype=torch.float32, device=dev)
+    h.smax, h.blank, h.zero_inf = smax, blank, zero_inf
+    z = _ZERO.get(dev.index)
+    if z is None:
+        z = _ZERO[dev.index] = torch.zeros(1, dtype=torch.float32, device=dev)
+    h.zero = z
+    return h
 
 
 class CTCLoss(nn.Module):
diff --git a/wav2letter_pytorch_amd/engine.py b/wav2letter_pytorch_amd/engine.py
--- a/wav2letter_pytorch_amd/engine.py
+++ b/wav2letter_pytorch_amd/engine.py
@@ -498,6 +498,7 @@
 FOLD_BN_FINALIZE = os.environ.get('W2L_FOLD_BN_FINALIZE', '0') == '1'
 FOLD_BN_FWD = os.environ.get('W2L_FOLD_BN_FWD', 'auto')
 FOLD_BN_FWD_MAX_ROWS = 12288
+FUSED_LOSS_SEAM = os.environ.get('W2L_FUSED_LOSS_SEAM', '1') != '0'
 FAST_BN_BWD = os.environ.get('W2L_FAST_BN_BWD', '1') == '1'
 STAT_SLOTS = int(os.environ.get('W2L_STAT_SLOTS', '8'))
 
@@ -629,6 +630,7 @@
         self.backward_done: Optional[Callable[[], None]] = None
         self.overlap_wgrad = True
         self._side = None
+        self._seam = None
         self._main_stream = None
         self._side_used = False
         self._held: list = []
@@ -1293,14 +1295,20 @@
         uc.keep.append(lens)
         return d
 
-    def backward(self, ctx, g_out: torch.Tensor):
+    def seam_ok(self, ctx) -> bool:
+        return bool(FUSED_LOSS_SEAM and self.head is not None and ctx['training'] and ctx['softmax_mode'] == 0
+                    and not self.precise and ctx['out'].is_cuda and self.n_labels <= 64)
+
+    def backward(self, ctx, g_out: Optional[torch.Tensor], seam=None):
         try:
+            self._seam = seam
             return self._backward(ctx, g_out)
         finally:
+            self._seam = None
             lib.w2l_conv_stats_mode(0)
             self._slot_pool = None
 
-    def _backward(self, ctx, g_out: torch.Tensor):
+    def _backward(self, ctx, g_out: Optional[torch.Tensor]):
         acts: List[Act] = ctx['acts']
         out = ctx['out']
         N = out.shape[0]
@@ -1376,10 +1384,12 @@
         dev = out.device
         st = stream_ptr
         pool_off = 0
-        g_out = g_out.contiguous().float()
+        seam = self._seam
         glog = torch.empty_like(out)
-        check(lib.w2l_log_softmax_bwd(ptr(g_out), ptr(out), N, Th, L, ctx['softmax_mode'], ptr(glog), st()),
-              'w2l_log_softmax_bwd')
+        if seam is None:
+            g_out = g_out.contiguous().float()
+            check(lib.w2l_log_softmax_bwd(ptr(g_out), ptr(out), N, Th, L, ctx['softmax_mode'], ptr(glog), st()),
+                  'w2l_log_softmax_bwd')
         head = self.head
         pk = pack_weights(head, precise)
         hh = roundup(Th, 64) - Th
@@ -1387,8 +1397,15 @@
         dy_lo = torch.empty_like(dy_hi) if precise else None
         colsum = small_pool[pool_off: pool_off + pk.coutp]
         pool_off += roundup(head.cout, 64)
-        check(lib.w2l_pad_cast(ptr(glog), N, Th, L, pk.coutp, hh, ptr(dy_hi), ptr(dy_lo), ptr(colsum), st()),
-              'w2l_pad_cast')
+        if seam is None:
+            check(lib.w2l_pad_cast(ptr(glog), N, Th, L, pk.coutp, hh, ptr(dy_hi), ptr(dy_lo), ptr(colsum), st()),
+                  'w2l_pad_cast')
+        else:
+            assert not precise and tuple(seam.lp.shape) == (N, Th, L) and seam.lp.data_ptr() == out.data_ptr()
+            seam.launch(pk.coutp, hh, dy_hi, glog)
+            fork = self._fork(dev) if self.grad_ready is None and self.flat_ready is None else None
+            with self._on_side(fork, [glog, small_pool]):
+                check(lib.w2l_colsum(ptr(glog), N * Th, L, pk.coutp, ptr(colsum), stream_ptr()), 'w2l_colsum')
         last = acts[-1]
         self._wgrad(head, pk, dy_hi, dy_lo, hh, Th, last, grads)
         if head.bias is not None:
diff --git a/wav2letter_pytorch_amd/layers.py b/wav2letter_pytorch_amd/layers.py
--- a/wav2letter_pytorch_amd/layers.py
+++ b/wav2letter_pytorch_amd/layers.py
@@ -8,6 +8,7 @@
 import torch
 import torch.nn as nn
 
+from . import ctc_loss
 from .engine import ACT_NONE, PAD_ZERO, ConvSpec, StackEngine, UnitSpec, _GradSource
 
 
@@ -168,6 +169,10 @@
         want_dx = bool(x.requires_grad)
         out, ectx = engine.forward(x, lens, training, softmax_mode, want_input_grad=want_dx)
         ctx.engine, ctx.ectx = engine, ectx
+        ctx.w2l_seam = None
+        ctx.w2l_seam_ok = engine.seam_ok(ectx)
+        ctx.w2l_seam_out = (out.data_ptr(), tuple(out.shape), tuple(out.stride()))
+        ctx.w2l_seam_buffers = ctc_loss.new_seam
         if holder.get('keep_ctx'):
             holder['ctx'] = ectx
         holder['lens_out'] = ectx['lens_out']
@@ -181,7 +186,8 @@
             rp.before_eager()
             rp.pending = None
         replay._last_backward[0] = None
-        grads = ctx.engine.backward(ctx.ectx, g)
+        seam, g = ctc_loss.claim(ctx, g)
+        grads = ctx.engine.backward(ctx.ectx, g, seam=seam)
         dx = ctx.ectx.get('input_grad')
         ctx.ectx = None
         return (dx, None, None, None, None, None, *grads)
diff --git a/wav2letter_pytorch_amd/replay.py b/wav2letter_pytorch_amd/replay.py
--- a/wav2letter_pytorch_amd/replay.py
+++ b/wav2letter_pytorch_amd/replay.py
@@ -7,7 +7,7 @@
 import numpy as np
 import torch
 
-from . import _lib
+from . import _lib, ctc_loss
 from ._lib import check, lib, ptr
 
 ENABLED = os.environ.get('W2L_REPLAY', '1') != '0'
@@ -66,6 +66,10 @@
         self.O_sig = self.X_sig = None
         self.x_static = self.x_ref = None
         self.g_static = None
+        self.seam = None
+        self.up_static = None
+        self.seam_call = None
+        self.B_fused = False
         self.out = None
         self.ectx = None
         self.lens_out = None
@@ -121,7 +125,7 @@
     def _mode_flags(self):
         from . import engine as E
         return (E.DETERMINISTIC_WGRAD, E.DEALT_WGRAD, E.DEFER_SPREAD, E.WGRAD_AFTER_DGRAD, E.FUSED_BN_REDUCE, E.FOLD_BN_FINALIZE,
-                E.FOLD_BN_FWD, E.FAST_BN_BWD, E.STAT_SLOTS, E.FP8_DGRAD, E.FP8_WGRAD, E.WGROUP_MAX, E.AUTOTUNE,
+                E.FOLD_BN_FWD, E.FAST_BN_BWD, E.FUSED_LOSS_SEAM, E.STAT_SLOTS, E.FP8_DGRAD, E.FP8_WGRAD, E.WGROUP_MAX, E.AUTOTUNE,
                 os.environ.get('W2L_WGRAD_GROUPS', 'auto'))
 
     def plan_forward(self, x, lens, training, softmax_mode, keep_ctx):
@@ -344,6 +348,10 @@
         else:
             out = _record_forward(rp, engine, rset, x, lens, softmax_mode)
         holder['lens_out'] = rset.lens_out
+        ctx.w2l_seam = None
+        ctx.w2l_seam_ok = rset.ectx is not None and engine.seam_ok(rset.ectx) and (mode == 'record' or rset.B_fused)
+        ctx.w2l_seam_out = (out.data_ptr(), tuple(out.shape), tuple(out.stride()))
+        ctx.w2l_seam_buffers = lambda *a: _seam_buffers(rset, mode, *a)
         return out
 
     @staticmethod
@@ -351,20 +359,24 @@
         engine, rset = ctx.engine, ctx.rset
         rp = replayer_for(engine)
         n = len(engine.parameters())
-        if any(p.grad is not None for p, _ in (rset.grads or [])) or (rset.grads is None and
+        seam, g = ctc_loss.claim(ctx, g)
+        other_form = ctx.mode == 'replay' and (seam is not None) != rset.B_fused
+        if other_form or any(p.grad is not None for p, _ in (rset.grads or [])) or (rset.grads is None and
                                                                       any(p.grad is not None for p in engine.parameters())):
             if rset.ectx is None:
+                if other_form:
+                    raise RuntimeError('replayed step: this backward pass needs the eager context of its record set, which is gone')
                 raise RuntimeError('replayed step: p.grad is already set (gradient accumulation) and the eager context of this '
                                    'record set is gone; call optimizer.zero_grad(set_to_none=True) before backward(), or set W2L_REPLAY=0')
             rp.before_eager()
-            grads = engine.backward(rset.ectx, g)
+            grads = engine.backward(rset.ectx, g, seam=seam)
             rp.pending = None
             _last_backward[0] = None
             return (None,) * 7 + tuple(grads)
         if ctx.mode == 'replay':
-            _replay_backward(rp, engine, rset, g)
+            _replay_backward(rp, engine, rset, g, seam)
         else:
-            _record_backward(rp, engine, rset, g)
+            _record_backward(rp, engine, rset, g, seam)
         return (None,) * (7 + n)
 
 
@@ -451,24 +463,82 @@
     return out
 
 
+SEAM_ARG = {'targets': 1, 'smax': 7, 'blank': 8, 'zero_inf': 9, 'ws': 11, 'upstream': 12}
+
+
+def _seam_buffers(rset, mode, lp, targets, input_lengths, target_lengths, smax, blank, zero_inf):
+    if mode == 'record':
+        h = ctc_loss.new_seam(lp, targets, input_lengths, target_lengths, smax, blank, zero_inf, own_ints=True)
+        h.src = [None, None, None]
+        rset.seam = h
+    else:
+        h = rset.seam
+        if h is None or not rset.B_fused or rset.seam_call is None or h.lp.data_ptr() != lp.data_ptr() or h.lp.shape != lp.shape:
+            return None
+        if tuple(h.tg.shape) != tuple(targets.shape) or h.smax != smax:
+            n, t, _ = lp.shape
+            h.tg = torch.empty(tuple(targets.shape), dtype=torch.int32, device=lp.device)
+            h.ws = torch.empty(max(int(lib.w2l_ctc_workspace_bytes(n, t, smax)), 4), dtype=torch.uint8, device=lp.device)
+            h.src[0] = None
+        h.smax, h.blank, h.zero_inf = smax, blank, zero_inf
+    for i, (dst, src) in enumerate(((h.tg, targets), (h.il, input_lengths), (h.tl, target_lengths))):
+        src = torch.as_tensor(src)
+        if src.numel() != dst.numel():
+            return None
+        sig = (src.data_ptr(), src._version, src)
+        if h.src[i] is None or h.src[i][0] != sig[0] or h.src[i][1] != sig[1] or h.src[i][2] is not src:
+            dst.copy_(src.reshape(dst.shape), non_blocking=True)
+            h.src[i] = sig
+    return h
+
+
+def _find_call(ph, name):
+    op = _lib._replay_ops()[name][0]
+    for it in ph.items:
+        if it[0] == 'c':
+            for j in range(it[2]):
+                if it[1][j].op == op:
+                    return it[1][j]
+    return None
+
+
+def _patch_seam_call(rset, h):
+    a = rset.seam_call.a
+    a[SEAM_ARG['targets']].p = h.tg.data_ptr()
+    a[SEAM_ARG['ws']].p = h.ws.data_ptr()
+    a[SEAM_ARG['smax']].i, a[SEAM_ARG['blank']].i, a[SEAM_ARG['zero_inf']].i = h.smax, h.blank, h.zero_inf
+
+
 def _assign_grads(rset):
     for p, gbuf in rset.grads:
         if gbuf is not None:
             p.grad = gbuf.detach()
 
 
-def _record_backward(rp, engine, rset, g):
+def _record_backward(rp, engine, rset, g, seam=None):
     from . import engine as E
     pool = rset.ensure_pool()
     tune0 = (len(E._tuned_shapes), len(E._wgroup_forms))
     with torch.cuda.use_mem_pool(pool):
-        rset.g_static = torch.empty(g.shape, dtype=torch.float32, device=g.device)
-        rset.g_static.copy_(g)
+        if seam is None:
+            rset.g_static = torch.empty(g.shape, dtype=torch.float32, device=g.device)
+            rset.g_static.copy_(g)
+        else:
+            rset.up_static = torch.empty(1, dtype=torch.float32, device=seam.lp.device)
+            rset.up_static.copy_(seam.up)
+            seam.up = rset.up_static
         with _lib.Recorder() as rec:
-            grads = engine.backward(rset.ectx, rset.g_static)
+            grads = engine.backward(rset.ectx, rset.g_static if seam is None else None, seam=seam)
     ph = rec.finish() if rset.F is not None else None
+    rset.B_fused = seam is not None
     params = engine.parameters()
     why = rec.poisoned
+    rset.seam_call = None
+    if ph is not None and seam is not None:
+        ph.keep.extend(seam.tensors())
+        rset.seam_call = _find_call(ph, 'w2l_ctc_grad_dy')
+        if rset.seam_call is None:
+            ph, why = None, 'the loss seam left no w2l_ctc_grad_dy in the record'
     if ph is not None and tune0 != (len(E._tuned_shapes), len(E._wgroup_forms)):
         ph, why = None, 'kernel plans were measured during the step'
     fixed = []
@@ -493,9 +563,15 @@
     _say(f'recorded set {rset.index}: F {rset.F.n_calls} calls, B {rset.B.n_calls} calls, {len(rset.deferred)} held-back gradients')
 
 
-def _replay_backward(rp, engine, rset, g):
-    rset.g_static.copy_(g, non_blocking=True)
+def _replay_backward(rp, engine, rset, g, seam=None):
+    if seam is None:
+        rset.g_static.copy_(g, non_blocking=True)
+    else:
+        _patch_seam_call(rset, seam)
+        rset.seam_call.a[SEAM_ARG['upstream']].p = seam.up.data_ptr()
     rset.B.replay()
+    if seam is not None:
+        rset.seam_call.a[SEAM_ARG['upstream']].p = rset.up_static.data_ptr()
     engine._side_used = False
     if rset.deferred:
         opt = engine.deferred
```
